# serycjon/WOFT

Hardware: AMD Instinct MI355X
Metric: tracked frames/sec at 1080p, 12 RAFT iters; flow EPE vs reference (higher is better)
Workload: dtype bf16x3 (split-bf16 MFMA operands emulating fp32, fp32 accumulate)

## Files before the change

### include/woft_hip.h

```cpp
#ifndef WOFT_HIP_H
#define WOFT_HIP_H

#include <stdint.h>

#ifdef __cplusplus
extern "C" {
#endif

#define WOFT_OK 0
#define WOFT_EINVAL (-1)
#define WOFT_ELAUNCH (-2)

int woft_abi_version(void);
int woft_sizeof(int which);
int woft_set_tuning(int key, int value);

enum woft_epilogue {
    WOFT_EPI_LINEAR = 0,
    WOFT_EPI_RELU = 1,
    WOFT_EPI_SIGMOID = 2,
    WOFT_EPI_TANH = 3,
    WOFT_EPI_RELU_RES_RELU = 4,
    WOFT_EPI_GRU_ZR = 5,
    WOFT_EPI_GRU_Q = 6,
    WOFT_EPI_CTX = 7,
    WOFT_EPI_WH_MEAN = 8,
    WOFT_EPI_FLOWHEAD = 9
};

typedef struct woft_conv_params {
    const float* in0;
    const float* in1;
    int32_t cs0, cs1;
    int32_t c_split;
    int32_t n_img, h, w;
    int32_t ho, wo;
    int32_t taps_y, taps_x;
    int32_t stride, pad_y, pad_x;
    int32_t cin_pad;
    int32_t flat;
    const float* wgt;
    const void* wgt_hi;
    const void* wgt_lo;
    int32_t precision;
    const float* bias;
    float alpha;
    int32_t cout;
    int32_t cout_pad;
    float* out;
    int64_t ldo;
    int32_t co_off;
    int32_t out_w, out_pitch;
    int32_t epi;
    int32_t split;
    const float* e0;
    const float* e1;
    int32_t lde0, lde1;
    float* out1;
    int32_t ldo1;
    float* stat_sum;
    float* stat_sq;
    int32_t tile_m, tile_n;
    int32_t halo;
    int32_t in_norm;
    const float* in_mean;
    const float* in_rstd;
    const float* bias_map;
    int32_t ld_bias_map;
    const int32_t* out_index;
    const float* wh0_lookup;
    int32_t wh0_ld;
    const float* wh0_mean;
    const void* wh0_w;
    const float* wh0_bias;
    const int32_t* wh0_index;
    const void* wgt_frag;
    const void* wgt_mx;
    int32_t roi_y0, roi_x0, roi_h, roi_w;
} woft_conv_params;

int woft_conv2d(const woft_conv_params* p, void* stream);
int woft_conv2d_pair(const woft_conv_params* a, const woft_conv_params* b, void* stream);
int woft_upload_u8(const void* src, void* pinned, void* dev, int64_t bytes, int32_t n_chunks, void* stream);
int woft_split_bf16(const float* x, int64_t n, void* hi, void* lo, void* stream);
int woft_conv3x3_narrow(const float* in, int32_t cs, int32_t n_img, int32_t h, int32_t w, int32_t cin_pad,
                        const float* wgt, const float* bias, int32_t cout, float* out, int64_t ldo, int32_t co_off,
                        void* stream);
int woft_flow_head_update(const float* in, int32_t cs, int32_t h, int32_t w, int32_t cin_pad, const float* wgt,
                          const float* bias, float* delta, int64_t ld_delta, float* coords1, float* flow4,
                          float* flow_cat, int32_t ld_cat, void* stream);
int woft_flow_head_gather(const float* part, int32_t n_planes, int32_t ld, int32_t h, int32_t w, const float* bias2,
                          float* delta, int64_t ld_delta, float* coords1, float* flow4, float* flow_cat, int32_t ld_cat,
                          void* stream);
int woft_split_bf16_lines(const float* x, int64_t n, void* out, void* stream);
int woft_corr_gemm_bf16(const void* a, const void* b, int64_t m, int64_t n, int64_t rows_a, int64_t rows_b, int32_t k,
                        float alpha, void* out, int64_t ldo, int32_t terms, int32_t out_bf16, void* stream);

int woft_inorm_finalize(const float* stat_sum, const float* stat_sq, int32_t n_part, int32_t ld,
                        int32_t channels, int32_t channels_pad, int64_t count, float eps,
                        float* mean, float* rstd, void* ws, void* stream);
int64_t woft_inorm_ws_bytes(void);
int woft_inorm_apply(const float* x, const float* mean, const float* rstd, const float* res,
                     const float* res_mean, const float* res_rstd, int32_t res_mode,
                     float* out, int64_t n_pix, int32_t channels, int32_t mode, void* stream);

int woft_preprocess_bgr_u8(const uint8_t* img, int32_t h, int32_t w, float* out,
                           int32_t hp, int32_t wp, int32_t pad_top, int32_t pad_left, void* stream);

int woft_avgpool2_nhwc(const float* in, int32_t h, int32_t w, int32_t c, float* out, void* stream);

int woft_feature_pyramid(const float* in, int32_t h, int32_t w, int32_t c, int32_t levels, float* const* pooled,
                         void* const* split, int32_t terms, void* stream);

typedef struct woft_lookup_params {
    const void* vol[4];
    int32_t ht[4], wt[4];
    int64_t plane[4];
    int32_t levels, radius;
    const float* coords;
    int64_t n_pix;
    float* out;
    int32_t ldo;
    int32_t vol_bf16;
    int32_t ablate;
} woft_lookup_params;
int woft_corr_lookup(const woft_lookup_params* p, void* stream);
typedef struct woft_lookup_otf_params {
    const void* f1;
    const void* f2[4];
    int32_t h[4], w[4];
    int32_t levels, radius, terms;
    int32_t hf, wf, k;
    float alpha;
    const float* coords;
    float* out;
    const int32_t* need;
    int32_t ldo;
    int32_t ablate;
    const float* fh_part;
    const float* fh_bias;
    float* fh_delta;
    float* fh_flow4;
    float* fh_flow_cat;
    int32_t fh_planes, fh_ld, fh_ld_delta, fh_ld_cat;
    int32_t roi_y0, roi_x0, roi_h, roi_w;
    int32_t smp_y0, smp_x0, smp_h, smp_w;
} woft_lookup_otf_params;
int woft_corr_lookup_otf(const woft_lookup_otf_params* p, void* stream);
#define WOFT_BAND_M0 3
#define WOFT_BAND_LD 16
#define WOFT_BAND_M(l) ((WOFT_BAND_M0 + (1 << (l)) - 1) >> (l))
#define WOFT_BAND_W(radius, l) (2 * ((radius) + 1 + WOFT_BAND_M(l)))
int woft_corr_band_geometry(int32_t radius, int32_t levels, int32_t* m, int32_t* w, int32_t* row_off);
typedef struct woft_lookup_band_params {
    woft_lookup_otf_params otf;
    float* band;
    int32_t* miss;
    int32_t* miss_count;
} woft_lookup_band_params;
int woft_corr_band_build(const woft_lookup_band_params* p, void* stream);
int woft_corr_lookup_band(const woft_lookup_band_params* p, void* stream);
int woft_tile_rows(const float* in, int32_t h, int32_t w, int32_t c, float* out, void* stream);

int woft_coords_update(float* coords1, const float* delta, int32_t ld_delta, int32_t wf, int64_t n_pix,
                       float* flow4, float* flow_cat, int32_t ld_cat, void* stream);
int woft_coords_init(float* coords1, int32_t hf, int32_t wf, float* flow4, float* flow_cat,
                     int32_t ld_cat, void* stream);
int woft_coords_init_flow(float* coords1, const float* flow_init, int32_t hf, int32_t wf, float* flow4, float* flow_cat,
                          int32_t ld_cat, void* stream);
int woft_forward_interpolate(const float* flow, int32_t hf, int32_t wf, float* out, void* stream);

int woft_sample_bilinear(const float* data, int32_t c, int32_t h, int32_t w, const float* x, const float* y, int64_t n,
                         float* out, void* stream);
int woft_flow_chain(const float* fab, const float* fbc, int32_t h, int32_t w, float* fac, void* stream);
int woft_flow_fb(const float* fab, const float* fba, int32_t h, int32_t w, float alpha, float beta, float* err, float* ok,
                 void* stream);

int woft_flow_chain_fold(const float* prev_flow, const float* prev_cost, const float* prev_vis, const float* step_flow,
                         const float* step_wlogit, const float* step_mlogit, int32_t h, int32_t w, float unit_cost,
                         float vis_thr, int32_t k, int32_t first, float* best_flow, float* best_cost, float* best_vis,
                         int32_t* best_sel, void* stream);

#define WOFT_CHAIN_HIST 130
int woft_chain_tc(const float* flow, const float* cost, const float* vis, const int32_t* sel, const uint8_t* tmask, int32_t gh,
                  int32_t gw, int32_t mh, int32_t mw, float vis_thr, float* dst, float* w, float* ok, int32_t* hist, void* stream);

int woft_features_pack(const float* f1, int64_t ld_f1, const float* net, int64_t ld_net, const float* inp, int64_t ld_inp,
                       int64_t P, int32_t fdim, int32_t hdim, int32_t cdim, float* record, void* stream);
int woft_features_unpack(const float* record, int64_t P, int32_t fdim, int32_t hdim, int32_t cdim, float* fmap, int64_t ld_fmap,
                         void* fmap_split, float* net, int64_t ld_net, float* xbuf, int64_t ld_xbuf, float* inp_c,
                         int64_t ld_inp_c, void* stream);

int woft_colsum(const float* f, int64_t n_pix, int32_t c, double* ws, int32_t n_part, double* total, void* stream);
int woft_wh_conv0(const float* lookup, int32_t ld_lookup, const float* mean, int64_t n_pix, int32_t nwin,
                  const float* wt, const float* bias, float* out, const int32_t* index, void* stream);
int woft_wh_pack(const float* lookup, int32_t ld_lookup, const float* f1, int32_t c, const double* f2_total,
                 float alpha, int64_t n_pix, int32_t nwin, float* mean, float* x8, void* stream);
int woft_wh_reduce(const float* act, int32_t c, int32_t nwin2, const float* w, float bias,
                   int64_t n_pix, float* out, void* stream);
int woft_warp_features(const float* f, int32_t h, int32_t w, int32_t c, int32_t cs, const float* coords, int64_t n_pix,
                       float* out, int32_t ld_out, void* stream);
int woft_wh_needed(const float* pts, const int32_t* count, int32_t n_max, int32_t top, int32_t left, int32_t hf, int32_t wf,
                   const int32_t* index, int32_t n_win, int32_t* bitmap, int32_t* dyn_index, int32_t* n_needed, void* stream);

int woft_convex_upsample(const float* coords1, const float* wlow, const float* mask, int32_t ld_mask,
                         int32_t hf, int32_t wf, int32_t crop_top, int32_t crop_left, int32_t h, int32_t w,
                         float* flow_up, float* dst, float* wout, int32_t do_sigmoid, void* stream);
int woft_convex_weights_at(const float* pts, const int32_t* count, int32_t n_max, const float* wlow, const float* mask,
                           int32_t ld_mask, int32_t hf, int32_t wf, int32_t crop_top, int32_t crop_left,
                           int32_t do_sigmoid, float* wsel, void* stream);
#define WOFT_WH_TRAIN_CHUNK 16
#define WOFT_WH_TRAIN_MAX_WIN (9 * 2048)
int woft_convex_weights_at_bwd(const float* pts, const int32_t* count, int32_t n_max, const float* g_wsel, const float* wlow,
                               const float* mask, int32_t ld_mask, int32_t hf, int32_t wf, int32_t crop_top,
                               int32_t crop_left, int32_t do_sigmoid, const int32_t* index, int32_t n_win, float* g_wlow,
                               void* stream);
int woft_wh_reduce_bwd(const float* act, const float* w6, const float* g_wlow, const int32_t* index, int32_t n_win,
                       float* g_act, double* ws, float* g_w6, float* g_b6, void* stream);
int woft_wh_train_conv(const float* x, int32_t cin, const float* wt, const float* bias, const float* gate, int32_t n_win,
                       float* y, void* stream);
int64_t woft_wh_wgrad_ws_bytes(int32_t n_win, int32_t cin);
int woft_wh_wgrad(const float* gy, const float* x, int32_t cin, int32_t cin_out, int32_t n_win, float* ws, float* gw,
                  float* gb, void* stream);
int woft_flow_to_tc(const float* flow, const float* weights, int32_t h, int32_t w, float* dst, float* wout,
                    int32_t do_sigmoid, void* stream);
int woft_upflow8(const float* coords1, const float* wlow, int32_t hf, int32_t wf,
                 int32_t crop_top, int32_t crop_left, int32_t h, int32_t w,
                 float* flow_up, float* dst, float* wout, int32_t do_sigmoid, void* stream);

int woft_warp_perspective_u8(const uint8_t* img, int32_t h, int32_t w, int32_t c, const double* hinv,
                             uint8_t* out, uint8_t* valid, int32_t nearest, void* stream);

int woft_warp_perspective_window_u8(const uint8_t* img, int32_t h, int32_t w, int32_t c, const double* hinv, int32_t y0,
                                    int32_t x0, int32_t hw, int32_t ww, uint8_t* out, uint8_t* valid, int32_t nearest,
                                    void* stream);
int woft_crop_u8(const uint8_t* img, int32_t h, int32_t w, int32_t c, int32_t y0, int32_t x0, int32_t hw, int32_t ww,
                 uint8_t* out, void* stream);
int64_t woft_mask_bbox_ws_bytes(void);
int woft_mask_bbox(const uint8_t* mask, int32_t h, int32_t w, const double* hinv, uint8_t* warped, void* ws, int32_t* bbox,
                   void* stream);

int woft_resize_linear_u8(const uint8_t* img, int32_t h, int32_t w, int32_t c, uint8_t* out, int32_t ho, int32_t wo,
                          float scale_y, float scale_x, void* stream);

int64_t woft_tc_select_ws_bytes(int64_t n);
int woft_tc_select(const float* dst, const float* w, const uint8_t* tmask, const uint8_t* pwmask, int32_t gh,
                   int32_t gw, int32_t mh, int32_t mw, int32_t check_dst, const float* sobol_u, int32_t n_draw,
                   void* ws, float* pa, float* pb, float* wout, int32_t cap, int32_t* count, void* stream);
int woft_tc_flags(const float* dst, const uint8_t* tmask, const uint8_t* pwmask, int32_t gh, int32_t gw, int32_t mh,
                  int32_t mw, int32_t check_dst, uint8_t* flags, void* stream);
int woft_tc_select_vis(const float* dst, const float* w, const uint8_t* tmask, const uint8_t* pwmask, int32_t gh,
                       int32_t gw, int32_t mh, int32_t mw, int32_t check_dst, const float* sobol_u, int32_t n_draw,
                       const float* vis, int32_t vis_mode, float vis_thr, void* ws, float* pa, float* pb, float* wout,
                       int32_t cap, int32_t* count, void* stream);
int woft_tc_flags_vis(const float* dst, const uint8_t* tmask, const uint8_t* pwmask, int32_t gh, int32_t gw, int32_t mh,
                      int32_t mw, int32_t check_dst, const float* vis, int32_t vis_mode, float vis_thr, uint8_t* flags,
                      void* stream);

#define WOFT_HFIT_SINGLE_MAX 2048
int64_t woft_hfit_ws_bytes(void);
int woft_hfit(const float* pa, const float* pb, const float* w, int32_t n_max, const int32_t* count,
              int32_t reweight, float huber_k, int32_t n_irls, void* ws, float* Hout, int32_t* status, void* stream);
#define WOFT_HFIT_BATCH_MAX 65535
int woft_hfit_batched(const float* pa, const float* pb, const float* w, int32_t batch, int32_t n_max,
                      const int32_t* counts, int32_t reweight, float huber_k, int32_t n_irls, float* Hout,
                      int32_t* status, void* stream);
int woft_hfit_batched_bwd(const float* pa, const float* pb, const float* w, int32_t batch, int32_t n_max,
                          const int32_t* counts, const float* gH, float* gpa, float* gpb, float* gw, int32_t* status,
                          void* stream);
int woft_hfit_step(const float* pa, const float* pb, const float* w, int32_t n, const float* rew, int32_t first,
                   void* ws, float* res, float* Hout, int32_t* status, void* stream);
int woft_inlier_frac(const float* pa, const float* pb, int32_t n_max, const int32_t* count, const float* H,
                     float thr, float* frac, void* stream);

int64_t woft_ransac_ws_bytes(int32_t n_max, int32_t max_iters);
int woft_ransac(const float* pa, const float* pb, int32_t n_max, const int32_t* count, int32_t max_iters, double thr,
                double conf, uint64_t seed, int32_t refine, void* ws, float* Hout, int32_t* status, int32_t* info,
                uint8_t* inlier_mask, void* stream);

int64_t woft_trs_ws_bytes(int32_t n_max, int32_t max_iters);
int woft_trs(const float* pa, const float* pb, int32_t n_max, const int32_t* count, int32_t max_iters, double thr,
             double conf, uint64_t seed, int32_t refine, void* ws, float* Hout, int32_t* status, int32_t* info,
             uint8_t* inlier_mask, void* stream);

#ifdef __cplusplus
}
#endif
#endif
```

### woft_amd/_lib.py

```python
import ctypes as C
import os
from pathlib import Path

import torch

LIB_PATH = Path(os.environ.get("WOFT_HIP_LIB") or Path(__file__).resolve().parent / "lib" / "libwoft_hip.so")

EPI_LINEAR, EPI_RELU, EPI_SIGMOID, EPI_TANH, EPI_RELU_RES_RELU, EPI_GRU_ZR, EPI_GRU_Q, EPI_CTX, EPI_WH_MEAN, EPI_FLOWHEAD = range(10)

vp, i32, i64, f32 = C.c_void_p, C.c_int32, C.c_int64, C.c_float


class ConvParams(C.Structure):
    _fields_ = [
        ("in0", vp), ("in1", vp), ("cs0", i32), ("cs1", i32), ("c_split", i32),
        ("n_img", i32), ("h", i32), ("w", i32), ("ho", i32), ("wo", i32),
        ("taps_y", i32), ("taps_x", i32), ("stride", i32), ("pad_y", i32), ("pad_x", i32),
        ("cin_pad", i32), ("flat", i32), ("wgt", vp), ("wgt_hi", vp), ("wgt_lo", vp), ("precision", i32),
        ("bias", vp), ("alpha", f32),
        ("cout", i32), ("cout_pad", i32), ("out", vp), ("ldo", i64), ("co_off", i32),
        ("out_w", i32), ("out_pitch", i32), ("epi", i32), ("split", i32),
        ("e0", vp), ("e1", vp), ("lde0", i32), ("lde1", i32), ("out1", vp), ("ldo1", i32),
        ("stat_sum", vp), ("stat_sq", vp), ("tile_m", i32), ("tile_n", i32), ("halo", i32),
        ("in_norm", i32), ("in_mean", vp), ("in_rstd", vp), ("bias_map", vp), ("ld_bias_map", i32),
        ("out_index", vp),
        ("wh0_lookup", vp), ("wh0_ld", i32), ("wh0_mean", vp), ("wh0_w", vp), ("wh0_bias", vp), ("wh0_index", vp),
        ("wgt_frag", vp), ("wgt_mx", vp),
        ("roi_y0", i32), ("roi_x0", i32), ("roi_h", i32), ("roi_w", i32),
    ]


class LookupParams(C.Structure):
    _fields_ = [
        ("vol", vp * 4), ("ht", i32 * 4), ("wt", i32 * 4), ("plane", i64 * 4),
        ("levels", i32), ("radius", i32), ("coords", vp), ("n_pix", i64), ("out", vp), ("ldo", i32),
        ("vol_bf16", i32), ("ablate", i32),
    ]


class LookupOtfParams(C.Structure):
    _fields_ = [
        ("f1", vp), ("f2", vp * 4), ("h", i32 * 4), ("w", i32 * 4),
        ("levels", i32), ("radius", i32), ("terms", i32), ("hf", i32), ("wf", i32), ("k", i32),
        ("alpha", f32), ("coords", vp), ("out", vp), ("need", vp), ("ldo", i32), ("ablate", i32),
        ("fh_part", vp), ("fh_bias", vp), ("fh_delta", vp), ("fh_flow4", vp), ("fh_flow_cat", vp),
        ("fh_planes", i32), ("fh_ld", i32), ("fh_ld_delta", i32), ("fh_ld_cat", i32),
        ("roi_y0", i32), ("roi_x0", i32), ("roi_h", i32), ("roi_w", i32),
        ("smp_y0", i32), ("smp_x0", i32), ("smp_h", i32), ("smp_w", i32),
    ]


class LookupBandParams(C.Structure):
    _fields_ = LookupOtfParams._fields_ + [("band", vp), ("miss", vp), ("miss_count", vp)]


_SIGS = {
    "woft_abi_version": (i32, []),
    "woft_sizeof": (i32, [i32]),
    "woft_set_tuning": (i32, [i32, i32]),
    "woft_conv2d": (i32, [C.POINTER(ConvParams), vp]),
    "woft_conv2d_pair": (i32, [C.POINTER(ConvParams), C.POINTER(ConvParams), vp]),
    "woft_upload_u8": (i32, [vp, vp, vp, i64, i32, vp]),
    "woft_split_bf16": (i32, [vp, i64, vp, vp, vp]),
    "woft_split_bf16_lines": (i32, [vp, i64, vp, vp]),
    "woft_flow_to_tc": (i32, [vp, vp, i32, i32, vp, vp, i32, vp]),
    "woft_corr_lookup_otf": (i32, [C.POINTER(LookupOtfParams), vp]),
    "woft_corr_band_geometry": (i32, [i32, i32, C.POINTER(i32), C.POINTER(i32), C.POINTER(i32)]),
    "woft_corr_band_build": (i32, [C.POINTER(LookupBandParams), vp]),
    "woft_corr_lookup_band": (i32, [C.POINTER(LookupBandParams), vp]),
    "woft_conv3x3_narrow": (i32, [vp, i32, i32, i32, i32, i32, vp, vp, i32, vp, i64, i32, vp]),
    "woft_flow_head_update": (i32, [vp, i32, i32, i32, i32, vp, vp, vp, i64, vp, vp, vp, i32, vp]),
    "woft_flow_head_gather": (i32, [vp, i32, i32, i32, i32, vp, vp, i64, vp, vp, vp, i32, vp]),
    "woft_corr_gemm_bf16": (i32, [vp, vp, i64, i64, i64, i64, i32, f32, vp, i64, i32, i32, vp]),
    "woft_inorm_finalize": (i32, [vp, vp, i32, i32, i32, i32, i64, f32, vp, vp, vp, vp]),
    "woft_inorm_ws_bytes": (i64, []),
    "woft_inorm_apply": (i32, [vp, vp, vp, vp, vp, vp, i32, vp, i64, i32, i32, vp]),
    "woft_preprocess_bgr_u8": (i32, [vp, i32, i32, vp, i32, i32, i32, i32, vp]),
    "woft_avgpool2_nhwc": (i32, [vp, i32, i32, i32, vp, vp]),
    "woft_feature_pyramid": (i32, [vp, i32, i32, i32, i32, vp, vp, i32, vp]),
    "woft_corr_lookup": (i32, [C.POINTER(LookupParams), vp]),
    "woft_tile_rows": (i32, [vp, i32, i32, i32, vp, vp]),
    "woft_coords_update": (i32, [vp, vp, i32, i32, i64, vp, vp, i32, vp]),
    "woft_coords_init": (i32, [vp, i32, i32, vp, vp, i32, vp]),
    "woft_coords_init_flow": (i32, [vp, vp, i32, i32, vp, vp, i32, vp]),
    "woft_forward_interpolate": (i32, [vp, i32, i32, vp, vp]),
    "woft_sample_bilinear": (i32, [vp, i32, i32, i32, vp, vp, i64, vp, vp]),
    "woft_flow_chain": (i32, [vp, vp, i32, i32, vp, vp]),
    "woft_flow_fb": (i32, [vp, vp, i32, i32, f32, f32, vp, vp, vp]),
    "woft_flow_chain_fold": (i32, [vp, vp, vp, vp, vp, vp, i32, i32, f32, f32, i32, i32, vp, vp, vp, vp, vp]),
    "woft_chain_tc": (i32, [vp, vp, vp, vp, vp, i32, i32, i32, i32, f32, vp, vp, vp, vp, vp]),
    "woft_features_pack": (i32, [vp, i64, vp, i64, vp, i64, i64, i32, i32, i32, vp, vp]),
    "woft_features_unpack": (i32, [vp, i64, i32, i32, i32, vp, i64, vp, vp, i64, vp, i64, vp, i64, vp]),
    "woft_colsum":(i32, [vp, i64, i32, vp, i32, vp, vp]),
    "woft_wh_pack": (i32, [vp, i32, vp, i32, vp, f32, i64, i32, vp, vp, vp]),
    "woft_wh_conv0": (i32, [vp, i32, vp, i64, i32, vp, vp, vp, vp, vp]),
    "woft_wh_reduce": (i32, [vp, i32, i32, vp, f32, i64, vp, vp]),
    "woft_warp_features": (i32, [vp, i32, i32, i32, i32, vp, i64, vp, i32, vp]),
    "woft_wh_needed": (i32, [vp, vp, i32, i32, i32, i32, i32, vp, i32, vp, vp, vp, vp]),
    "woft_convex_upsample": (i32, [vp, vp, vp, i32, i32, i32, i32, i32, i32, i32, vp, vp, vp, i32, vp]),
    "woft_convex_weights_at": (i32, [vp, vp, i32, vp, vp, i32, i32, i32, i32, i32, i32, vp, vp]),
    "woft_convex_weights_at_bwd": (i32, [vp, vp, i32, vp, vp, vp, i32, i32, i32, i32, i32, i32, vp, i32, vp, vp]),
    "woft_wh_reduce_bwd": (i32, [vp, vp, vp, vp, i32, vp, vp, vp, vp, vp]),
    "woft_wh_train_conv": (i32, [vp, i32, vp, vp, vp, i32, vp, vp]),
    "woft_wh_wgrad_ws_bytes": (i64, [i32, i32]),
    "woft_wh_wgrad": (i32, [vp, vp, i32, i32, i32, vp, vp, vp, vp]),
    "woft_upflow8": (i32, [vp, vp, i32, i32, i32, i32, i32, i32, vp, vp, vp, i32, vp]),
    "woft_warp_perspective_u8": (i32, [vp, i32, i32, i32, C.POINTER(C.c_double), vp, vp, i32, vp]),
    "woft_resize_linear_u8": (i32, [vp, i32, i32, i32, vp, i32, i32, f32, f32, vp]),
    "woft_warp_perspective_window_u8": (i32, [vp, i32, i32, i32, C.POINTER(C.c_double), i32, i32, i32, i32, vp, vp, i32, vp]),
    "woft_crop_u8": (i32, [vp, i32, i32, i32, i32, i32, i32, i32, vp, vp]),
    "woft_mask_bbox_ws_bytes": (i64, []),
    "woft_mask_bbox": (i32, [vp, i32, i32, C.POINTER(C.c_double), vp, vp, vp, vp]),
    "woft_tc_select_ws_bytes": (i64, [i64]),
    "woft_tc_select": (i32, [vp, vp, vp, vp, i32, i32, i32, i32, i32, vp, i32, vp, vp, vp, vp, i32, vp, vp]),
    "woft_tc_flags": (i32, [vp, vp, vp, i32, i32, i32, i32, i32, vp, vp]),
    "woft_tc_select_vis": (i32, [vp, vp, vp, vp, i32, i32, i32, i32, i32, vp, i32, vp, i32, f32, vp, vp, vp, vp, i32, vp, vp]),
    "woft_tc_flags_vis": (i32, [vp, vp, vp, i32, i32, i32, i32, i32, vp, i32, f32, vp, vp]),
    "woft_hfit_ws_bytes": (i64, []),
    "woft_hfit": (i32, [vp, vp, vp, i32, vp, i32, f32, i32, vp, vp, vp, vp]),
    "woft_hfit_batched": (i32, [vp, vp, vp, i32, i32, vp, i32, f32, i32, vp, vp, vp]),
    "woft_hfit_batched_bwd": (i32, [vp, vp, vp, i32, i32, vp, vp, vp, vp, vp, vp, vp]),
    "woft_hfit_step": (i32, [vp, vp, vp, i32, vp, i32, vp, vp, vp, vp, vp]),
    "woft_inlier_frac": (i32, [vp, vp, i32, vp, vp, f32, vp, vp]),
    "woft_ransac_ws_bytes": (i64, [i32, i32]),
    "woft_ransac": (i32, [vp, vp, i32, vp, i32, C.c_double, C.c_double, C.c_uint64, i32, vp, vp, vp, vp, vp, vp]),
    "woft_trs_ws_bytes": (i64, [i32, i32]),
    "woft_trs": (i32, [vp, vp, i32, vp, i32, C.c_double, C.c_double, C.c_uint64, i32, vp, vp, vp, vp, vp, vp]),
}

EXPORTS = tuple(_SIGS)
_lib = None


class WoftHipError(RuntimeError):
    pass


def load():
    global _lib
    if _lib is not None:
        return _lib
    if not LIB_PATH.exists():
        raise WoftHipError(f"{LIB_PATH} is missing: build it with `python -m woft_amd.build` "
                           "(hipcc --offload-arch=gfx950); woft_amd has no CPU fallback")
    lib = C.CDLL(str(LIB_PATH))
    for name, (res, args) in _SIGS.items():
        fn = getattr(lib, name)
        fn.restype, fn.argtypes = res, args
    if lib.woft_sizeof(0) != C.sizeof(ConvParams) or lib.woft_sizeof(1) != C.sizeof(LookupParams) \
            or lib.woft_sizeof(2) != C.sizeof(LookupOtfParams) or lib.woft_sizeof(3) != C.sizeof(LookupBandParams):
        raise WoftHipError("ctypes mirror of woft_conv_params / woft_lookup_params is out of sync with the library")
    _lib = lib
    return lib


def check(rc, what):
    if rc != 0:
        raise WoftHipError(f"{what} failed with code {rc}")


def ptr(t):
    return None if t is None else t.data_ptr()


_RAW_STREAM = getattr(torch._C, "_cuda_getCurrentRawStream", None) if os.environ.get("WOFT_RAW_STREAM", "1") != "0" else None
_CUR_DEV = torch.cuda.current_device


def stream_ptr():
    if _RAW_STREAM is None:
        return torch.cuda.current_stream().cuda_stream
    return _RAW_STREAM(_CUR_DEV())
```

### woft_amd/build.py

```python
import hashlib
import os
import subprocess
import sys
import time
from pathlib import Path

HERE = Path(__file__).resolve().parent
CSRC = HERE / "csrc"
LIBDIR = HERE / "lib"
LIB = LIBDIR / "libwoft_hip.so"
STAMP = LIBDIR / "libwoft_hip.stamp"
HIPCC = os.environ.get("HIPCC", "/opt/rocm/bin/hipcc")
FLAGS = ["--offload-arch=gfx950", "-O3", "-std=c++17", "-fPIC", "-fno-fast-math", "-ffp-contract=off",
         "-Wno-c++20-extensions"]


PARTS = {"conv.hip": [("p1", ["-DWOFT_ONLY_PREC=1"]), ("p2", ["-DWOFT_ONLY_PREC=2"]), ("p3", ["-DWOFT_ONLY_PREC=3"])],
         "conv_regb.hip": [(f"p{k}", [f"-DWOFT_ONLY_PREC={k}"]) for k in (1, 2, 3, 4)]}


def _sources():
    return sorted(CSRC.glob("*.hip"))


def _units():
    out = []
    for src in _sources():
        for tag, flags in PARTS.get(src.name, [("", [])]):
            out.append((src, LIBDIR / (src.stem + ("." + tag if tag else "") + ".o"), flags))
    return out


def _digest():
    h = hashlib.sha256()
    for p in sorted(list(CSRC.glob("*.hip")) + list(CSRC.glob("*.h")) + [HERE.parent / "include" / "woft_hip.h"]):
        h.update(p.name.encode())
        h.update(p.read_bytes())
    h.update(" ".join(FLAGS).encode())
    h.update(repr(sorted(PARTS.items())).encode())
    return h.hexdigest()


def build(force=False, verbose=True):
    LIBDIR.mkdir(exist_ok=True)
    dig = _digest()
    if not force and LIB.exists() and STAMP.exists() and STAMP.read_text().strip() == dig:
        return LIB
    objs = []
    units = _units()
    wanted = {u[1] for u in units}
    for old in LIBDIR.glob("*.o"):
        if old not in wanted:
            old.unlink()
    hdr = hashlib.sha256()
    for h in sorted(list(CSRC.glob("*.h")) + [HERE.parent / "include" / "woft_hip.h"]):
        hdr.update(h.name.encode())
        hdr.update(h.read_bytes())

    def unit_hash(src, extra):
        u = hashlib.sha256(hdr.digest())
        u.update(src.read_bytes())
        u.update(" ".join(FLAGS + extra).encode())
        return u.hexdigest()
    jobs = int(os.environ.get("WOFT_BUILD_JOBS", os.cpu_count() or 4))
    weight = {"conv.hip": 8, "conv_regb.hip": 6, "conv_1x1.hip": 20}
    units.sort(key=lambda u: -(u[0].stat().st_size * weight.get(u[0].name, 1)))
    pending, running = [], []
    for src, obj, extra in units:
        objs.append(obj)
        uh = unit_hash(src, extra)
        tag = Path(str(obj) + ".hash")
        if not force and obj.exists() and tag.exists() and tag.read_text().strip() == uh:
            continue
        pending.append((src, obj, extra, uh))
    while pending or running:
        while pending and len(running) < jobs:
            src, obj, extra, uh = pending.pop(0)
            tag = Path(str(obj) + ".hash")
            if tag.exists():
                tag.unlink()
            cmd = [HIPCC, *FLAGS, *extra, "-c", str(src), "-o", str(obj)]
            if verbose:
                print(" ".join(cmd), flush=True)
            running.append((src, subprocess.Popen(cmd), tag, uh))
        time.sleep(0.2)
        for ent in list(running):
            rc = ent[1].poll()
            if rc is None:
                continue
            running.remove(ent)
            if rc != 0:
                for other in running:
                    other[1].kill()
                raise RuntimeError(f"hipcc failed on {ent[0]}")
            ent[2].write_text(ent[3])
    cmd = [HIPCC, "--offload-arch=gfx950", "-shared", "-fPIC", "-o", str(LIB), *map(str, objs)]
    if verbose:
        print(" ".join(cmd), flush=True)
    subprocess.check_call(cmd)
    STAMP.write_text(dig)
    return LIB


if __name__ == "__main__":
    build(force="--force" in sys.argv)
    print(LIB)
```

### woft_amd/csrc/conv.hip

```cpp
#include <type_traits>

#include "conv_common.h"
#include "dma.h"
#include "halo_map.h"
#include "split_lines.h"

#if !defined(WOFT_ONLY_PREC)
#error "conv.hip is compiled in parts: -DWOFT_ONLY_PREC=1|2|3 (woft_amd/build.py)"
#endif
#define WOFT_CAT2_(a, b) a##b
#define WOFT_CAT2(a, b) WOFT_CAT2_(a, b)
#define WOFT_CAT4_(a, b, c, d) a##b##c##d
#define WOFT_CAT4(a, b, c, d) WOFT_CAT4_(a, b, c, d)
#if WOFT_ONLY_PREC == 1
constexpr int PART_TERMS = 3;
#elif WOFT_ONLY_PREC == 3
constexpr int PART_TERMS = 16;
#else
constexpr int PART_TERMS = 1;
#endif

#if WOFT_ONLY_PREC == 1
int g_tuning[4] = {0, 0, 0, 0};
#else
// ... 763 lines not shown
                            acc[i][j] = __builtin_amdgcn_mfma_f32_32x32x16_bf16(ah[i], bh[j], acc[i][j], 0, 0, 0);
                }
            }
        }
        if (STAGES == 2) dma_wait<0>();
        __syncthreads();
    }
    if (abl & 2) {
        float t = 0.f;
#pragma unroll
        for (int i = 0; i < TM; ++i)
#pragma unroll
            for (int j = 0; j < TN; ++j)
#pragma unroll
                for (int r = 0; r < 16; ++r) t += acc[i][j][r];
        if (t == 12345.678f) p.out[0] = t;
        return;
    }
    float* stage = (float*)smem + wave * woft::STAGE_FLOATS;
    constexpr int LD = woft::STAGE_LD;
    const int rr = lane >> 3, c4 = (lane & 7) * 4;
#pragma unroll
    for (int i = 0; i < TM; ++i)
#pragma unroll
        for (int j = 0; j < TN; ++j) {
#pragma unroll
            for (int r = 0; r < 16; ++r) stage[((r & 3) + 8 * (r >> 2) + 4 * hh) * LD + r32] = acc[i][j][r];
            __builtin_amdgcn_wave_barrier();
            const int n = n0 + wn * 64 + j * 32 + c4;
#pragma unroll
            for (int pass = 0; pass < 4; ++pass) {
                const int row = rr + 8 * pass;
                const int64_t m = m0 + wm * 64 + i * 32 + row;
                f32x4 v = *(const f32x4*)(stage + row * LD + c4);
                if (m >= M || n >= p.cout || (abl & 1)) continue;
#pragma unroll
                for (int e = 0; e < 4; ++e) v[e] *= p.alpha;
                if (OUT16) *(bf16x4*)((__bf16*)p.out + m * p.ldo + n) = __builtin_convertvector(v, bf16x4);
                else if (abl & 16) __builtin_nontemporal_store(v, (f32x4*)(p.out + m * p.ldo + n));
                else *(f32x4*)(p.out + m * p.ldo + n) = v;
            }
            __builtin_amdgcn_wave_barrier();
        }
}

#endif

#if WOFT_ONLY_PREC == 1
__global__ void split_bf16_kernel(const float* __restrict__ x, int64_t n4, __bf16* __restrict__ hi,
                                  __bf16* __restrict__ lo) {
    const int64_t i = (int64_t)blockIdx.x * blockDim.x + threadIdx.x;
    if (i >= n4) return;
    const f32x4 vv = *(const f32x4*)(x + i * 4);
    const bf16x4 h = __builtin_convertvector(vv, bf16x4);
    *(bf16x4*)(hi + i * 4) = h;
    if (lo != nullptr) *(bf16x4*)(lo + i * 4) = __builtin_convertvector(vv - __builtin_convertvector(h, f32x4), bf16x4);
}

#endif

template <int BM, int BN>
int launch_conv(const woft_conv_params& p, const woft_conv_params* second, hipStream_t s) {
    auto blocks = [](const woft_conv_params& q) { return ceil_div64((int64_t)q.n_img * q.ho * q.wo, BM) * (q.cout_pad / BN); };
    const woft_conv_params& pb = second ? *second : p;
    const int split = (int)blocks(p);
    dim3 grid((unsigned)(blocks(p) + (second ? blocks(pb) : 0)));
    if (p.precision == 0) {
#if WOFT_ONLY_PREC == 2
        if (second) return WOFT_EINVAL;
        woft_launch(0, conv_mfma_f32_kernel<BM, BN>, grid, dim3(256), 0, s, p);
        return woft_launch_status();
#else
        return WOFT_EINVAL;
#endif
    }
    if (p.precision != WOFT_ONLY_PREC) return WOFT_EINVAL;
    for (const woft_conv_params* q : {&p, &pb}) {
        const int64_t cs_max = (q->in1 != nullptr && q->cs1 > q->cs0) ? q->cs1 : q->cs0;
        if ((int64_t)q->n_img * q->h * q->w * cs_max >= (1ll << 31)) return WOFT_EINVAL;
        if ((int64_t)q->taps_y * q->taps_x * q->cin_pad >= (1 << 20)) return WOFT_EINVAL;
    }
    woft_launch(0, conv_mfma_bf16_kernel<BM, BN, PART_TERMS>, grid, dim3(256), 0, s, p, pb, split);
    return woft_launch_status();
}

}

int WOFT_CAT2(woft_conv_regb_launch_p, WOFT_ONLY_PREC)(const woft_conv_params& p, const woft_conv_params* second, void* stream);
int woft_conv_stem_launch(const woft_conv_params& p, void* stream);
int woft_conv_1x1_launch(const woft_conv_params& p, const woft_conv_params* second, void* stream);
int woft_conv_dispatch_p1(const woft_conv_params& p, const woft_conv_params* second, void* stream);
int woft_conv_dispatch_p2(const woft_conv_params& p, const woft_conv_params* second, void* stream);
int woft_conv_dispatch_p3(const woft_conv_params& p, const woft_conv_params* second, void* stream);

#if WOFT_ONLY_PREC == 1
static int conv_check(const woft_conv_params& p) {
    if (p.in0 == nullptr || p.out == nullptr) return WOFT_EINVAL;
    if (p.precision < 0 || p.precision > 4) return WOFT_EINVAL;
    if (p.precision == 4 && ((p.halo != 8 && p.halo != 12) || p.wgt_frag == nullptr || p.wgt_mx == nullptr ||
                             p.in_norm != 0 || p.taps_y * p.taps_x == 1))
        return WOFT_EINVAL;
    if (p.precision == 0 && p.wgt == nullptr) return WOFT_EINVAL;
    if (p.precision >= 1 && p.wgt_hi == nullptr) return WOFT_EINVAL;
    if (p.precision == 1 && p.wgt_lo == nullptr) return WOFT_EINVAL;
    if (p.cin_pad <= 0 || p.cin_pad % BK != 0) return WOFT_EINVAL;
    if (p.in1 != nullptr && (p.c_split % BK != 0 || p.c_split <= 0 || p.c_split >= p.cin_pad)) return WOFT_EINVAL;
    if (p.cs0 % 4 != 0 || (p.in1 != nullptr && p.cs1 % 4 != 0)) return WOFT_EINVAL;
    if (p.flat && (p.taps_x != 1 || p.in1 != nullptr || (p.cs0 != 4 && p.cs0 != 8 && p.cs0 != 16 && p.cs0 != 32)))
        return WOFT_EINVAL;
    if (!p.flat && (p.cs0 < (p.in1 != nullptr ? p.c_split : p.cin_pad) || (p.in1 != nullptr && p.cs1 < p.cin_pad - p.c_split)))
        return WOFT_EINVAL;
    if (p.n_img <= 0 || p.h <= 0 || p.w <= 0 || p.ho <= 0 || p.wo <= 0 || p.taps_y <= 0 || p.taps_x <= 0 ||
        p.stride <= 0 || p.cout <= 0)
        return WOFT_EINVAL;
    if ((p.tile_m != 64 && p.tile_m != 128) || (p.tile_n != 64 && p.tile_n != 128 && !(p.halo == 16 && p.tile_n == 256)))
        return WOFT_EINVAL;
    if (p.cout_pad % p.tile_n != 0 || p.cout > p.cout_pad) return WOFT_EINVAL;
    if (p.epi < 0 || p.epi > WOFT_EPI_FLOWHEAD) return WOFT_EINVAL;
    if (p.epi == WOFT_EPI_FLOWHEAD && (p.halo != 8 || p.precision == 0 || p.stat_sum != nullptr || p.bias_map != nullptr ||
                                       p.e0 == nullptr))
        return WOFT_EINVAL;
    if (p.epi == WOFT_EPI_WH_MEAN && (p.halo != 2 || p.cout_pad != p.tile_n || p.e0 == nullptr || p.e1 == nullptr ||
                                      p.stat_sum != nullptr))
        return WOFT_EINVAL;
    if ((p.epi == WOFT_EPI_RELU_RES_RELU || p.epi == WOFT_EPI_GRU_ZR || p.epi == WOFT_EPI_GRU_Q) && p.e0 == nullptr)
        return WOFT_EINVAL;
    if (p.epi == WOFT_EPI_GRU_Q && p.e1 == nullptr) return WOFT_EINVAL;
    if (p.epi == WOFT_EPI_GRU_ZR && p.out1 == nullptr) return WOFT_EINVAL;
    if (p.e0 != nullptr && p.lde0 % 4 != 0) return WOFT_EINVAL;
    if (p.e1 != nullptr && p.lde1 % 4 != 0) return WOFT_EINVAL;
    if (p.out1 != nullptr && (p.ldo1 % 4 != 0 || p.split % 4 != 0)) return WOFT_EINVAL;
    if ((p.stat_sum == nullptr) != (p.stat_sq == nullptr)) return WOFT_EINVAL;
    if (p.epi != WOFT_EPI_WH_MEAN) {
        if (p.out_pitch != 0 || p.ldo % 4 != 0 || p.co_off % 4 != 0 || p.epi == WOFT_EPI_CTX) return WOFT_EINVAL;
        const bool simple = p.epi == WOFT_EPI_LINEAR || p.epi == WOFT_EPI_RELU || p.epi == WOFT_EPI_SIGMOID || p.epi == WOFT_EPI_TANH;
        if (p.cout % 4 != 0 && (!simple || p.stat_sum != nullptr || p.bias_map != nullptr)) return WOFT_EINVAL;
    }
    if (p.in_norm < 0 || p.in_norm > 2) return WOFT_EINVAL;
    if ((p.roi_y0 | p.roi_x0 | p.roi_h | p.roi_w) != 0 &&
        ((p.halo != 8 && p.halo != 12 && p.halo != 16) || p.roi_h <= 0 || p.roi_w <= 0 || p.roi_y0 < 0 || p.roi_x0 < 0 ||
         p.roi_y0 > p.ho - p.roi_h || p.roi_x0 > p.wo - p.roi_w || p.stat_sum != nullptr || p.precision == 0))
        return WOFT_EINVAL;
    if (p.bias_map != nullptr && (p.cout % 4 != 0 || p.ld_bias_map < p.cout || p.ld_bias_map % 4 != 0 ||
                                  p.epi == WOFT_EPI_CTX || p.epi == WOFT_EPI_WH_MEAN || p.out_pitch != 0))
        return WOFT_EINVAL;
    if (p.in_norm != 0 && (p.halo == 0 || p.in1 != nullptr || p.in_mean == nullptr || p.in_rstd == nullptr)) return WOFT_EINVAL;
    if (p.wh0_lookup != nullptr &&
        (p.halo != 2 || p.precision == 0 || p.taps_y != 3 || p.taps_x != 3 || p.cin_pad != 128 || p.in1 != nullptr ||
         p.in_norm != 0 || p.ho != 9 || p.wo != 9 || p.wh0_ld < 324 || p.wh0_ld % 4 != 0 || p.wh0_mean == nullptr ||
         p.wh0_w == nullptr || p.wh0_bias == nullptr))
        return WOFT_EINVAL;
    return WOFT_OK;
}
#endif

int WOFT_CAT2(woft_conv_dispatch_p, WOFT_ONLY_PREC)(const woft_conv_params& p, const woft_conv_params* second, void* stream) {
    hipStream_t s = (hipStream_t)stream;
    if (second != nullptr && (second->precision != p.precision || second->halo != p.halo ||
                              (p.halo == 0 && second->tile_m != p.tile_m) ||
                              (second->tile_n != p.tile_n && p.halo != 16) || p.precision == 0 ||
                              (p.halo != 0 && p.halo != 8 && p.halo != 12 && p.halo != 16)))
        return WOFT_EINVAL;
    if (p.halo == 7)
        return second != nullptr ? WOFT_EINVAL : woft_conv_stem_launch(p, stream);
    if (p.halo == 16)
        return p.precision == 0 ? WOFT_EINVAL : woft_conv_1x1_launch(p, second, stream);
    for (const woft_conv_params* q : {&p, second}) {
        if (q == nullptr || q->halo == 0) continue;
        if (q->precision == 0 || q->flat || q->stride != 1) return WOFT_EINVAL;
        if (q->ho != q->h + 2 * q->pad_y - q->taps_y + 1 || q->wo != q->w + 2 * q->pad_x - q->taps_x + 1) return WOFT_EINVAL;
        const int64_t cs_max = (q->in1 != nullptr && q->cs1 > q->cs0) ? q->cs1 : q->cs0;
        if ((int64_t)q->n_img * q->h * q->w * cs_max >= (1ll << 31)) return WOFT_EINVAL;
        if ((int64_t)q->taps_y * q->taps_x * q->cin_pad >= (1 << 20)) return WOFT_EINVAL;
    }
    if (p.halo != 0) {
        if (p.halo == 8 || p.halo == 12)
            return WOFT_CAT2(woft_conv_regb_launch_p, WOFT_ONLY_PREC)(p, second, stream);
        if (p.halo == 1 && p.tile_n == 128) return launch_halo<8, 16, 128, 2, 2>(p, s);
        if (p.halo == 1 && p.tile_n == 64) return launch_halo<8, 16, 64, 2, 2>(p, s);
        if (p.halo == 2 && p.tile_n == 128 && p.ho == 9 && p.wo == 9) return launch_halo<9, 9, 128, 1, 2>(p, s);
        if (p.halo == 4 && p.tile_n == 128) return launch_halo<4, 16, 128, 2, 2>(p, s);
        if (p.halo == 4 && p.tile_n == 64) return launch_halo<4, 16, 64, 2, 2>(p, s);
        return WOFT_EINVAL;
    }
    if (p.tile_m == 128 && p.tile_n == 128) return launch_conv<128, 128>(p, second, s);
    if (p.tile_m == 128 && p.tile_n == 64) return launch_conv<128, 64>(p, second, s);
    if (p.tile_m == 64 && p.tile_n == 128) return launch_conv<64, 128>(p, second, s);
    return launch_conv<64, 64>(p, second, s);
}

#if WOFT_ONLY_PREC == 1
int woft_conv_regb_launch_p4(const woft_conv_params& p, const woft_conv_params* second, void* stream);

static int conv_dispatch_f16mx8(const woft_conv_params& p, const woft_conv_params* second, void* stream) {
    for (const woft_conv_params* q : {&p, second}) {
        if (q == nullptr) continue;
        if (q->precision != 4 || q->halo != p.halo || q->tile_n != p.tile_n || q->flat || q->stride != 1) return WOFT_EINVAL;
        if (q->ho != q->h + 2 * q->pad_y - q->taps_y + 1 || q->wo != q->w + 2 * q->pad_x - q->taps_x + 1) return WOFT_EINVAL;
        const int64_t cs_max = (q->in1 != nullptr && q->cs1 > q->cs0) ? q->cs1 : q->cs0;
        if ((int64_t)q->n_img * q->h * q->w * cs_max >= (1ll << 31)) return WOFT_EINVAL;
    }
    return woft_conv_regb_launch_p4(p, second, stream);
}

static int conv_dispatch(const woft_conv_params& p, const woft_conv_params* second, void* stream) {
    switch (p.precision) {
        case 4: return conv_dispatch_f16mx8(p, second, stream);
        case 1: return woft_conv_dispatch_p1(p, second, stream);
        case 3: return woft_conv_dispatch_p3(p, second, stream);
        default: return woft_conv_dispatch_p2(p, second, stream);
    }
}

extern "C" int woft_conv2d(const woft_conv_params* pp, void* stream) {
    if (pp == nullptr) return WOFT_EINVAL;
    const int rc = conv_check(*pp);
    return rc != WOFT_OK ? rc : conv_dispatch(*pp, nullptr, stream);
}

extern "C" int woft_conv2d_pair(const woft_conv_params* a, const woft_conv_params* b, void* stream) {
    if (a == nullptr || b == nullptr) return WOFT_EINVAL;
    int rc = conv_check(*a);
    if (rc == WOFT_OK) rc = conv_check(*b);
    if (rc != WOFT_OK) return rc;
    if (a->stat_sum != nullptr || b->stat_sum != nullptr) return WOFT_EINVAL;
    return conv_dispatch(*a, b, stream);
}
#endif

#if WOFT_ONLY_PREC == 3
extern "C" int woft_corr_gemm_bf16(const void* a, const void* b, int64_t m, int64_t n, int64_t rows_a, int64_t rows_b,
                                   int32_t k, float alpha, void* out, int64_t ldo, int32_t terms, int32_t out_bf16,
                                   void* stream) {
    if (!a || !b || !out || m <= 0 || n <= 0 || k <= 0 || ldo < n || n % 4 != 0 || ldo % 4 != 0) return WOFT_EINVAL;
    if (terms != 1 && terms != 3) return WOFT_EINVAL;
    if (k % (terms == 3 ? 32 : 64) != 0) return WOFT_EINVAL;
    if (rows_a % 128 != 0 || rows_b % 128 != 0 || rows_a < m || rows_b < n || m >= (1ll << 31)) return WOFT_EINVAL;
    woft_conv_params p = {};
    p.n_img = 1; p.ho = 1; p.wo = (int32_t)m;
    p.alpha = alpha;
    p.cout = (int32_t)n; p.cout_pad = (int32_t)rows_b;
    p.out = (float*)out; p.ldo = ldo;
    p.epi = WOFT_EPI_LINEAR;
    const int abl = g_tuning[2];
    hipStream_t s = (hipStream_t)stream;
    if (rows_a % 128 != 0 || rows_b % 128 != 0) return WOFT_EINVAL;
    dim3 grid((unsigned)(ceil_div64(m, 128) * (rows_b / 128)));
    if (terms == 3 && !out_bf16)
        hipLaunchKernelGGL((corr_gemm_bf16_kernel<3, 2, 2, 1>), grid, dim3(256), 0, s, (const __bf16*)a, (const __bf16*)b,
                           2 * k, p, abl);
    else if (terms == 3)
        hipLaunchKernelGGL((corr_gemm_bf16_kernel<3, 2, 2, 1, true>), grid, dim3(256), 0, s, (const __bf16*)a,
                           (const __bf16*)b, 2 * k, p, abl);
    else if (!out_bf16)
        hipLaunchKernelGGL((corr_gemm_bf16_kernel<1, 2, 2, 1>), grid, dim3(256), 0, s, (const __bf16*)a, (const __bf16*)b,
                           k, p, abl);
    else
        hipLaunchKernelGGL((corr_gemm_bf16_kernel<1, 2, 2, 1, true>), grid, dim3(256), 0, s, (const __bf16*)a,
                           (const __bf16*)b, k, p, abl);
    return woft_launch_status();
}

#endif

#if WOFT_ONLY_PREC == 1
int g_regb_dyn_lds = 0;

extern "C" int woft_set_tuning(int key, int value) {
    if (key < 0 || key >= 4) return WOFT_EINVAL;
    g_tuning[key] = value;
    if (key == 3) g_regb_dyn_lds = value;
    return WOFT_OK;
}

__global__ void split_bf16_lines_kernel(const float* __restrict__ x, int64_t n4, __bf16* __restrict__ out) {
    const int64_t i = (int64_t)blockIdx.x * blockDim.x + threadIdx.x;
    if (i >= n4) return;
    split_bf16_lines_store(out, i, *(const f32x4*)(x + i * 4));
}

extern "C" int woft_split_bf16_lines(const float* x, int64_t n, void* out, void* stream) {
    if (!x || !out || n <= 0 || n % 32 != 0) return WOFT_EINVAL;
    hipLaunchKernelGGL(split_bf16_lines_kernel, dim3((unsigned)ceil_div64(n / 4, 256)), dim3(256), 0, (hipStream_t)stream,
                       x, n / 4, (__bf16*)out);
    return woft_launch_status();
}

extern "C" int woft_split_bf16(const float* x, int64_t n, void* hi, void* lo, void* stream) {
    if (!x || !hi || n <= 0 || n % 4 != 0) return WOFT_EINVAL;
    hipLaunchKernelGGL(split_bf16_kernel, dim3((unsigned)ceil_div64(n / 4, 256)), dim3(256), 0, (hipStream_t)stream, x,
                       n / 4, (__bf16*)hi, (__bf16*)lo);
    return woft_launch_status();
}
#endif
```

### woft_amd/csrc/conv_1x1.hip

```cpp
#include "conv_common.h"

namespace {

using woft::BK;

template <int TERMS, int TN>
struct Geom1x1 {
    static constexpr int NP = (TERMS == 3) ? 2 : 1;
    static constexpr int BM = 64, TM = 2;
    static constexpr int WCOLS = 32 * TN, BN = 4 * WCOLS;
    static constexpr int A_PLANE = BM * LDB, A_ELEMS = NP * A_PLANE;
    static constexpr int ST = 2;
    static constexpr int STAGE_ELEMS = 2 * 4 * ST * woft::STAGE_FLOATS;
    static constexpr int SMEM_ELEMS = (2 * A_ELEMS > STAGE_ELEMS) ? 2 * A_ELEMS : STAGE_ELEMS;
};

template <int TERMS, int TN, bool FLAT, int DEPTH, int NB>
__device__ __forceinline__ void tile_1x1(const woft_conv_params& p, const int m_tile, const int n_tile, __bf16* smem) {
    using G = Geom1x1<TERMS, TN>;
    constexpr int NP = G::NP, TM = G::TM, A_PLANE = G::A_PLANE, A_ELEMS = G::A_ELEMS, WCOLS = G::WCOLS, BN = G::BN;
    static_assert(DEPTH % 2 == 0 && (2 * DEPTH) % NB == 0 && NB >= 2, "static ring slots");
    constexpr int STEP_ELEMS = NP * 2 * 64 * 8;

    const int tid = threadIdx.x;
    const int lane = tid & 63;
    const int wave = __builtin_amdgcn_readfirstlane(tid >> 6);
    const int r32 = lane & 31, hh = lane >> 5;
    const int row = tid >> 2, v = tid & 3;

    int64_t M = (int64_t)p.n_img * p.ho * p.wo;
    int64_t m0 = (int64_t)m_tile * G::BM;
    if ((p.roi_y0 | p.roi_x0 | p.roi_h | p.roi_w) != 0) {
        const int runs = (p.roi_w + G::BM - 1) / G::BM;
        const int line = m_tile / runs, run = m_tile - line * runs;
        const int img = line / p.roi_h, ry = line - img * p.roi_h;
        m0 = ((int64_t)img * p.ho + p.roi_y0 + ry) * p.wo + p.roi_x0 + run * G::BM;
        const int left = p.roi_w - run * G::BM;
        M = m0 + (left < G::BM ? left : G::BM);
    }
    const int n0 = n_tile * BN;
    const int nchunk = FLAT ? p.taps_y : p.cin_pad / BK;

    const int abl = (p.out_w <= -12350 && p.out_w > -12358) ? -12350 - p.out_w : 0;
    const bool rok = m0 + row < M;
    const uint32_t pix = rok ? (uint32_t)(m0 + row) : 0u;
    int oy = 0, img_row0 = 0;
    uint32_t run0 = 0;
    bool okx[2] = {true, true};
    if constexpr (FLAT) {
        const int hw = p.ho * p.wo;
        const int img = (int)(pix / (uint32_t)hw), rem = (int)(pix - (uint32_t)img * (uint32_t)hw);
        oy = rem / p.wo;
        const int ox = rem - oy * p.wo;
        img_row0 = img * p.h;
#pragma unroll
        for (int e = 0; e < 2; ++e) {
            const int ixp = ox - p.pad_x + (8 * v + 4 * e) / p.cs0;
            okx[e] = rok && ixp >= 0 && ixp < p.w;
        }
        run0 = (uint32_t)((ox - p.pad_x) * p.cs0 + 8 * v);
    }
    f32x4 rh[DEPTH][2];
    auto load_a = [&](int chunk, auto slot_tag) {
        constexpr int slot = decltype(slot_tag)::value;
        if ((abl & 1) && chunk >= DEPTH) return;
        const int ck = chunk < nchunk ? chunk : nchunk - 1;
        if constexpr (FLAT) {
            int iy = oy + ck - p.pad_y;
            iy = iy < 0 ? 0 : (iy >= p.h ? p.h - 1 : iy);
            const uint32_t rowoff = (uint32_t)(img_row0 + iy) * (uint32_t)(p.w * p.cs0);
#pragma unroll
            for (int e = 0; e < 2; ++e) rh[slot][e] = *(const f32x4*)(p.in0 + (okx[e] ? rowoff + run0 + 4 * e : 0u));
        } else {
            const int c0 = ck * BK;
            const bool second = (p.in1 != nullptr) && (c0 >= p.c_split);
            const float* base = second ? p.in1 : p.in0;
            const uint32_t cs = (uint32_t)(second ? p.cs1 : p.cs0);
            const uint32_t coff = (uint32_t)(second ? c0 - p.c_split : c0);
            rh[slot][0] = *(const f32x4*)(base + (pix * cs + coff + 8 * v));
            rh[slot][1] = *(const f32x4*)(base + (pix * cs + coff + 8 * v + 4));
        }
    };
    auto store_a = [&](int chunk, __bf16* As, auto slot_tag) {
        constexpr int slot = decltype(slot_tag)::value;
        const f32x4 zero = {0.f, 0.f, 0.f, 0.f};
        bool oky = true;
        if constexpr (FLAT) {
            const int iy = oy + chunk - p.pad_y;
            oky = iy >= 0 && iy < p.h;
        }
        bf16x4 hi[2], lo[2];
#pragma unroll
        for (int e = 0; e < 2; ++e) {
            const f32x4 val = (FLAT ? (okx[e] && oky) : rok) ? rh[slot][e] : zero;
            hi[e] = cvt16<TERMS>(val);
            if (NP == 2) lo[e] = __builtin_convertvector(val - widen_bf16x4(hi[e]), bf16x4);
        }
        *(bf16x8*)(As + row * LDB + 8 * v) = __builtin_shufflevector(hi[0], hi[1], 0, 1, 2, 3, 4, 5, 6, 7);
        if (NP == 2) *(bf16x8*)(As + A_PLANE + row * LDB + 8 * v) = __builtin_shufflevector(lo[0], lo[1], 0, 1, 2, 3, 4, 5, 6, 7);
    };

    const __bf16* wstream[TN];
#pragma unroll
    for (int j = 0; j < TN; ++j) wstream[j] = (const __bf16*)p.wgt_frag + (int64_t)(n0 / 32 + wave * TN + j) * nchunk * STEP_ELEMS + lane * 8;
    bf16x8 bq[NB][TN][NP];
    auto fetch_b = [&](int step, auto slot_tag) {
        constexpr int slot = decltype(slot_tag)::value;
        if ((abl & 2) && step >= NB - 1) return;
        const int s = step < 2 * nchunk ? step : 2 * nchunk - 1;
        const int off = (s >> 1) * STEP_ELEMS + (s & 1) * 512;
#pragma unroll
        for (int j = 0; j < TN; ++j)
#pragma unroll
            for (int pl = 0; pl < NP; ++pl) bq[slot][j][pl] = *(const bf16x8*)(wstream[j] + off + pl * 1024);
    };

    f32x16 acc[TM][TN];
#pragma unroll
    for (int i = 0; i < TM; ++i)
#pragma unroll
        for (int j = 0; j < TN; ++j)
#pragma unroll
            for (int r = 0; r < 16; ++r) acc[i][j][r] = 0.f;
    const int a_off = r32 * LDB + hh * 8;

    [&]<int... D>(std::integer_sequence<int, D...>) {
        (load_a(D, std::integral_constant<int, D>{}), ...);
    }(std::make_integer_sequence<int, DEPTH>{});
    [&]<int... S>(std::integer_sequence<int, S...>) {
        (fetch_b(S, std::integral_constant<int, S>{}), ...);
    }(std::make_integer_sequence<int, NB - 1>{});
    store_a(0, smem, std::integral_constant<int, 0>{});
    __syncthreads();

    auto run_chunk = [&](int c, auto d_tag) {
        constexpr int D = decltype(d_tag)::value;
        const __bf16* As = smem + (D & 1) * A_ELEMS;
        bf16x8 aq[2][TM][NP];
        auto read_a = [&](auto s2_tag) {
            constexpr int s2 = decltype(s2_tag)::value;
#pragma unroll
            for (int i = 0; i < TM; ++i)
#pragma unroll
                for (int pl = 0; pl < NP; ++pl) aq[s2][i][pl] = *(const bf16x8*)(As + a_off + i * 32 * LDB + pl * A_PLANE + s2 * 16);
        };
        read_a(std::integral_constant<int, 0>{});
        read_a(std::integral_constant<int, 1>{});
        [&]<int... S2>(std::integer_sequence<int, S2...>) {
            ([&] {
                constexpr int s2 = S2, slot = (2 * D + s2) % NB;
                fetch_b(2 * c + s2 + NB - 1, std::integral_constant<int, (2 * D + s2 + NB - 1) % NB>{});
                __builtin_amdgcn_sched_barrier(0);
                if (NP == 2) {
#pragma unroll
                    for (int j = 0; j < TN; ++j)
#pragma unroll
                        for (int i = 0; i < TM; ++i) acc[i][j] = mma16<TERMS>(aq[s2][i][NP - 1], bq[slot][j][0], acc[i][j]);
#pragma unroll
                    for (int j = 0; j < TN; ++j)
#pragma unroll
                        for (int i = 0; i < TM; ++i) acc[i][j] = mma16<TERMS>(aq[s2][i][0], bq[slot][j][NP - 1], acc[i][j]);
                }
#pragma unroll
                for (int j = 0; j < TN; ++j)
#pragma unroll
                    for (int i = 0; i < TM; ++i) acc[i][j] = mma16<TERMS>(aq[s2][i][0], bq[slot][j][0], acc[i][j]);
                if constexpr (s2 == 0) {
                    store_a(c + 1, smem + ((D + 1) & 1) * A_ELEMS, std::integral_constant<int, (D + 1) % DEPTH>{});
                    load_a(c + DEPTH, std::integral_constant<int, D>{});
                }
                __builtin_amdgcn_sched_barrier(0);
            }(), ...);
        }(std::make_integer_sequence<int, 2>{});
        __syncthreads();
    };
    for (int c0 = 0; c0 < nchunk; c0 += DEPTH) {
        [&]<int... D>(std::integer_sequence<int, D...>) {
            ((c0 + D < nchunk ? run_chunk(c0 + D, std::integral_constant<int, D>{}) : (void)0), ...);
        }(std::make_integer_sequence<int, DEPTH>{});
    }
    if (abl & 4) {
        float t = 0.f;
#pragma unroll
        for (int i = 0; i < TM; ++i)
#pragma unroll
            for (int j = 0; j < TN; ++j)
#pragma unroll
                for (int r = 0; r < 16; ++r) t += acc[i][j][r];
        if (t == 12345.678f) p.out[0] = t;
        return;
    }
    woft::conv_epilogue_t<TM, TN, G::BM, WCOLS, G::ST>(p, acc, (float*)smem + wave * G::ST * woft::STAGE_FLOATS,
                                                        woft::LinearRows{m0, M}, n0, 0, wave, lane, m_tile);
}

__host__ __device__ __forceinline__ int m_tiles_1x1(const woft_conv_params& p) {
    if ((p.roi_y0 | p.roi_x0 | p.roi_h | p.roi_w) != 0) return p.n_img * p.roi_h * ((p.roi_w + 63) / 64);
    return (int)(((int64_t)p.n_img * p.ho * p.wo + 63) / 64);
}


template <int TERMS>
__global__ __launch_bounds__(256, 2) void conv1x1_kernel(const woft_conv_params pa, const woft_conv_params pb, const int split) {
    __shared__ __attribute__((aligned(16))) __bf16 smem[Geom1x1<TERMS, 2>::SMEM_ELEMS];
    static_assert(Geom1x1<TERMS, 2>::SMEM_ELEMS >= Geom1x1<TERMS, 1>::SMEM_ELEMS, "one LDS array for every mode");
    const bool second_layer = (int)blockIdx.x >= split;
    const woft_conv_params p = second_layer ? pb : pa;
    const int bid = second_layer ? (int)blockIdx.x - split : (int)blockIdx.x;
    int m_tile, n_tile;
    woft::tile_of_block(bid, m_tiles_1x1(p), p.cout_pad / (p.flat ? 128 : 256), m_tile, n_tile);
    if (!p.flat) tile_1x1<TERMS, 2, false, 4, 4>(p, m_tile, n_tile, smem);
    else tile_1x1<TERMS, 1, true, 4, 4>(p, m_tile, n_tile, smem);
}

}

int woft_conv_1x1_launch(const woft_conv_params& a, const woft_conv_params* second, void* stream) {
    for (const woft_conv_params* q : {&a, second}) {
        if (q == nullptr) continue;
        const woft_conv_params& p = *q;
        if (p.precision < 1 || p.precision > 3 || p.precision != a.precision) return WOFT_EINVAL;
        if (p.stride != 1 || p.ho != p.h || p.wo != p.w || p.taps_x != 1) return WOFT_EINVAL;
        if (p.flat) {
            if (p.cin_pad != 32 || p.tile_n != 128 || 2 * p.pad_y + 1 != p.taps_y) return WOFT_EINVAL;
        } else if (p.taps_y != 1 || p.pad_y != 0 || p.pad_x != 0 || p.tile_n != 256) {
            return WOFT_EINVAL;
        }
        if (p.wgt_frag == nullptr || p.stat_sum != nullptr || p.in_norm != 0 || p.wh0_lookup != nullptr) return WOFT_EINVAL;
        if (p.epi == WOFT_EPI_FLOWHEAD || p.epi == WOFT_EPI_WH_MEAN || p.epi == WOFT_EPI_CTX) return WOFT_EINVAL;
        if (p.cout_pad % p.tile_n != 0) return WOFT_EINVAL;
        const int64_t cs_max = (p.in1 != nullptr && p.cs1 > p.cs0) ? p.cs1 : p.cs0;
        if ((int64_t)p.n_img * p.h * p.w * cs_max >= (1ll << 31)) return WOFT_EINVAL;
    }
    auto blocks = [](const woft_conv_params& q) {
        return (int64_t)m_tiles_1x1(q) * (q.cout_pad / (q.flat ? 128 : 256));
    };
    const woft_conv_params& pb = second ? *second : a;
    const int split = (int)blocks(a);
    dim3 grid((unsigned)(blocks(a) + (second ? blocks(pb) : 0)));
    hipStream_t s = (hipStream_t)stream;
    switch (a.precision) {
        case 1: woft_launch(0, conv1x1_kernel<3>, grid, dim3(256), 0, s, a, pb, split); break;
        case 2: woft_launch(0, conv1x1_kernel<1>, grid, dim3(256), 0, s, a, pb, split); break;
        default: woft_launch(0, conv1x1_kernel<16>, grid, dim3(256), 0, s, a, pb, split); break;
    }
    return woft_launch_status();
}
```

### woft_amd/csrc/lookup_band.hip

```cpp
#include "common.h"
#include "lookup_blocks.h"

namespace {

template <int R>
__global__ __launch_bounds__(256) void corr_lookup_band_kernel(const woft_lookup_band_params bp) {
    const woft_lookup_otf_params& p = bp.otf;
    constexpr int NPX = 64, NT = 256, MAXL = 4;
    constexpr int NW = 2 * R + 1, N2 = NW * NW, WS = NW + 1;
    constexpr int RS = WOFT_BAND_LD + 4;
    constexpr int PLD = WS * RS;
    constexpr int NLD = NPX * WS * 4 / NT;
    static_assert(NLD * NT == NPX * WS * 4, "pieces divide among the threads");
    __shared__ __attribute__((aligned(16))) float Wl[NPX * PLD];
    __shared__ int s_ox[MAXL][NPX], s_oy[MAXL][NPX];
    __shared__ float s_fx[MAXL][NPX], s_fy[MAXL][NPX];

    const int tid = threadIdx.x;
    const BlockRect br = block_rect(p);
    const int tiles_x = br.nx, ntiles = br.nx * br.ny;
    int tile;
    {
        const int q = ntiles / 8, rr = ntiles % 8, xcd = blockIdx.x % 8, idx = blockIdx.x / 8;
        tile = (xcd < rr ? xcd * (q + 1) : rr * (q + 1) + (xcd - rr) * q) + idx;
    }
    const int px0 = (br.bx0 + tile % tiles_x) * 8, py0 = (br.by0 + tile / tiles_x) * 8;
    const bool sampled = (p.smp_y0 | p.smp_x0 | p.smp_h | p.smp_w) == 0 ||
                         (py0 < p.smp_y0 + p.smp_h && py0 + 8 > p.smp_y0 && px0 < p.smp_x0 + p.smp_w && px0 + 8 > p.smp_x0);
    const int y = py0 + ((tid & 63) >> 3), x = px0 + (tid & 7);
    const bool cvalid = tid < NPX && y < p.hf && x < p.wf;
    const int64_t i = (int64_t)y * p.wf + x;
    if (p.need != nullptr) {
        const int any = cvalid ? p.need[i] : 0;
        if (!__syncthreads_or(any)) {
            if (cvalid) bp.miss[i] = 0;
            return;
        }
    }
    float cx = 0.f, cy = 0.f;
    if (cvalid) {
        cx = p.coords[i * 2];
        cy = p.coords[i * 2 + 1];
        if (p.fh_part != nullptr) {
            typedef float f32x2 __attribute__((ext_vector_type(2)));
            float dx = p.fh_bias ? p.fh_bias[0] : 0.f, dy = p.fh_bias ? p.fh_bias[1] : 0.f;
            const int64_t plane = (int64_t)p.hf * p.wf * p.fh_ld;
#pragma unroll
            for (int ky = 0; ky < 3; ++ky)
#pragma unroll
                for (int kx = 0; kx < 3; ++kx) {
                    const int yy = y + ky - 1, xx = x + kx - 1;
                    f32x2 v = {0.f, 0.f};
                    if (yy >= 0 && yy < p.hf && xx >= 0 && xx < p.wf) {
                        const float* src = p.fh_part + ((int64_t)yy * p.wf + xx) * p.fh_ld + (ky * 3 + kx) * 2;
                        v = *(const f32x2*)src;
                        for (int t = 1; t < p.fh_planes; ++t) v += *(const f32x2*)(src + t * plane);
                    }
                    dx += v[0];
                    dy += v[1];
                }
            p.fh_delta[i * p.fh_ld_delta] = dx;
            p.fh_delta[i * p.fh_ld_delta + 1] = dy;
            cx += dx;
            cy += dy;
            ((float*)p.coords)[i * 2] = cx;
            ((float*)p.coords)[i * 2 + 1] = cy;
            const float fx = cx - (float)x, fy = cy - (float)y;
            if (p.fh_flow4 != nullptr) *(f32x4*)(p.fh_flow4 + i * 4) = f32x4{fx, fy, 0.f, 0.f};
            if (p.fh_flow_cat != nullptr) {
                p.fh_flow_cat[i * p.fh_ld_cat] = fx;
                p.fh_flow_cat[i * p.fh_ld_cat + 1] = fy;
            }
        }
    }
    if (!sampled) {
        if (cvalid) bp.miss[i] = 0;
        return;
    }
    int ok = 1;
    if (cvalid) {
#pragma unroll
        for (int l = 0; l < MAXL; ++l) {
            if (l < p.levels) {
                const float sc = 1.0f / (float)(1 << l);
                const float xs = cx * sc, ys = cy * sc;
                float flx = floorf(xs), fly = floorf(ys);
                s_fx[l][tid] = xs - flx;
                s_fy[l][tid] = ys - fly;
                flx = fminf(fmaxf(flx, -1.0e6f), 1.0e6f);
                fly = fminf(fmaxf(fly, -1.0e6f), 1.0e6f);
                const int m = WOFT_BAND_M(l);
                const int ox = (int)flx - (x >> l) + m, oy = (int)fly - (y >> l) + m;
                ok &= (ox >= 0 && ox <= 2 * m && oy >= 0 && oy <= 2 * m) ? 1 : 0;
                s_ox[l][tid] = ox;
                s_oy[l][tid] = oy;
            }
        }
    }
    const int hit = __syncthreads_and(ok);
    if (cvalid) bp.miss[i] = hit ? 0 : 1;
    if (!hit) {
        if (tid == 0) atomicAdd(bp.miss_count, 1);
        return;
    }
    const int rows = band_row_off(R, p.levels);
    f32x4 pc[NLD];
    auto load_level = [&](int l) __attribute__((always_inline)) {
        const int roff = band_row_off(R, l);
#pragma unroll
        for (int k = 0; k < NLD; ++k) {
            const int it = tid + k * NT;
            const int pix = it / (4 * WS), rem = it - pix * (4 * WS);
            const int gy = py0 + (pix >> 3), gx = px0 + (pix & 7);
            pc[k] = f32x4{0.f, 0.f, 0.f, 0.f};
            if (gy < p.hf && gx < p.wf)
                pc[k] = *(const f32x4*)(bp.band + (((int64_t)gy * p.wf + gx) * rows + roff + s_ox[l][pix]) * WOFT_BAND_LD + rem * 4);
        }
    };
    load_level(0);
    for (int l = 0; l < p.levels; ++l) {
#pragma unroll
        for (int k = 0; k < NLD; ++k) {
            const int it = tid + k * NT;
            const int pix = it / (4 * WS), rem = it - pix * (4 * WS);
            *(f32x4*)(Wl + pix * PLD + (rem >> 2) * RS + (rem & 3) * 4) = pc[k];
        }
        __syncthreads();
        if (l + 1 < p.levels) load_level(l + 1);
        for (int it = tid; it < NPX * NW; it += NT) {
            const int pix = it / NW, c = it - pix * NW;
            const int gy = py0 + (pix >> 3), gx = px0 + (pix & 7);
            if (gy >= p.hf || gx >= p.wf) continue;
            const float fx = s_fx[l][pix], fy = s_fy[l][pix];
            const float* cq = Wl + pix * PLD + c * RS + s_oy[l][pix];
            float h[WS];
#pragma unroll
            for (int j = 0; j < WS; ++j) h[j] = cq[j] * (1.f - fx) + cq[RS + j] * fx;
            float* o = p.out + ((int64_t)gy * p.wf + gx) * p.ldo + l * N2 + c * NW;
#pragma unroll
            for (int j = 0; j < NW; ++j) o[j] = h[j] * (1.f - fy) + h[j + 1] * fy;
        }
        __syncthreads();
    }
}

}

extern "C" int woft_corr_lookup_band(const woft_lookup_band_params* bp, void* stream) {
    if (!bp || !bp->band || !bp->miss || !bp->miss_count) return WOFT_EINVAL;
    const woft_lookup_otf_params& p = bp->otf;
    if (p.levels < 1 || p.levels > 4 || !p.f1 || !p.coords || !p.out || p.hf <= 0 || p.wf <= 0 || p.ablate != 0) return WOFT_EINVAL;
    if (p.terms != 1 && p.terms != 3) return WOFT_EINVAL;
    if (!((p.k == 256 && p.radius == 4) || (p.k == 128 && p.radius == 3))) return WOFT_EINVAL;
    for (int l = 0; l < p.levels; ++l)
        if (p.h[l] <= 0 || p.w[l] <= 0) return WOFT_EINVAL;
    const int nout = p.levels * (2 * p.radius + 1) * (2 * p.radius + 1);
    if (p.ldo < nout) return WOFT_EINVAL;
    if (p.fh_part != nullptr && (p.fh_delta == nullptr || p.fh_planes < 1 || p.fh_ld < 20 || p.fh_ld % 4 != 0 || p.fh_ld_delta < 2 ||
                                 (p.fh_flow_cat != nullptr && p.fh_ld_cat < 2) || p.need != nullptr))
        return WOFT_EINVAL;
    auto rect_bad = [&](int y0, int x0, int h, int w) {
        return (y0 | x0 | h | w) != 0 && (h <= 0 || w <= 0 || y0 < 0 || x0 < 0 || y0 > p.hf - h || x0 > p.wf - w);
    };
    if (rect_bad(p.roi_y0, p.roi_x0, p.roi_h, p.roi_w) || rect_bad(p.smp_y0, p.smp_x0, p.smp_h, p.smp_w)) return WOFT_EINVAL;
    const BlockRect br = block_rect(p);
    dim3 grid((unsigned)(br.nx * br.ny));
    hipStream_t s = (hipStream_t)stream;
    if (p.radius == 4) woft_launch(0, corr_lookup_band_kernel<4>, grid, dim3(256), 0, s, *bp);
    else woft_launch(0, corr_lookup_band_kernel<3>, grid, dim3(256), 0, s, *bp);
    return woft_launch_status();
}
```

### woft_amd/engine.py

```python
import math
import os
from typing import NamedTuple

import torch

from . import _lib, conv_select, flow_region, ops, wh_train
from .conv_select import KERNELS, Kernel
from .ops import Act, new_act

EPI = _lib
DEFER_NORM = os.environ.get("WOFT_DEFER_NORM", "1") != "0"
FUSE_FLOWHEAD = os.environ.get("WOFT_FUSE_FLOWHEAD", "1") != "0"
PAIR_BRANCHES = os.environ.get("WOFT_PAIR", "1") != "0"
PYRAMID_ONE_LAUNCH = os.environ.get("WOFT_PYRAMID", "1") != "0"
FOLD_GATHER = os.environ.get("WOFT_FOLD_GATHER", "1") != "0"
CORR_BAND = os.environ.get("WOFT_CORR_BAND", "1") != "0"
BAND_MIN_LOOKUPS = 6


def _ru(x, m):
    return (x + m - 1) // m * m


class Step(NamedTuple):
    kind: str
    arg: object
    tag: str = None


class _Folded(NamedTuple):
    prog_iter_first: list
    prog_iter: list
    prog_iter_last: list
    gather: list
    lookup: object


class FlowKey(NamedTuple):
    iters: int
    crop: tuple
    h: int
    w: int
    flow_up: int
    dst: int
    wout: int
    mout: int
    do_sigmoid: bool
    mask_sigmoid: bool
    defer_wh: bool
    skip_wh: bool
    has_init: bool
    target_restored: bool
    wh_region: int
    flow_region: tuple


class _FlowGraph(torch.cuda.CUDAGraph):
    post = None


def _timed(sink, launch, *args, extra=None):
    if sink is None:
        return launch(*args)
    s, e = torch.cuda.Event(enable_timing=True), torch.cuda.Event(enable_timing=True)
    s.record()
    launch(*args)
    e.record()
    sink.append((s, e) if extra is None else (s, e, extra()))


def _head_layers(sd, prefix, cin):
    idx = sorted(int(k.split(".")[2]) for k in sd if k.startswith(prefix) and k.endswith(".weight"))
    shapes = [tuple(sd[f"{prefix}{i}.weight"].shape) for i in idx]
    ok = not (len(idx) < 2 or shapes[-1][0] != 1 or shapes[-1][2:] != (1, 1) or shapes[0][1] != cin
              or any(a[0] != b[1] for a, b in zip(shapes, shapes[1:])) or any(sh[2] != sh[3] or sh[2] % 2 == 0 for sh in shapes))
    return idx, shapes, ok


class _Spec:

    def __init__(self, small):
        self.small = small
        if small:
            self.fdim, self.hdim, self.cdim, self.radius = 128, 96, 64, 3
            self.fnorm, self.cnorm = "instance", "none"
        else:
            self.fdim, self.hdim, self.cdim, self.radius = 256, 128, 128, 4
            self.fnorm, self.cnorm = "instance", "batch"
        self.levels = 4
        self.nwin = 2 * self.radius + 1
        self.corr_c = self.levels * self.nwin ** 2
        self.corr_cs = _ru(self.corr_c, 32)
        self.xdim = _ru(self.cdim + (82 if small else 128), 32)
        self.flow_off = self.cdim + (80 if small else 126)


class _Enc:

    def __init__(self, sd, p, norm, spec, out_split=None):
        self.norm = norm

        def get(name, stride=1, flat_cs=0, bn=None):
            w, b = sd[name + ".weight"], sd[name + ".bias"]
            if norm == "batch" and bn is not None:
                w, b = ops.fold_bn(w, b, sd[bn + ".weight"], sd[bn + ".bias"], sd[bn + ".running_mean"],
                                   sd[bn + ".running_var"])
            return ops.pack_conv(w, b, stride=stride, flat_cs=flat_cs)

        self.conv1 = get(p + ".conv1", 2, 4, p + ".norm1")
        self.blocks = []
        for li, stride in ((1, 1), (2, 2), (3, 2)):
            for bi in range(2):
                q = f"{p}.layer{li}.{bi}"
                s = stride if bi == 0 else 1
                if spec.small:
                    convs = [get(q + ".conv1", 1, bn=q + ".norm1"), get(q + ".conv2", s, bn=q + ".norm2"),
                             get(q + ".conv3", 1, bn=q + ".norm3")]
                else:
                    convs = [get(q + ".conv1", s, bn=q + ".norm1"), get(q + ".conv2", 1, bn=q + ".norm2")]
                blk = dict(stride=s, convs=convs)
                if s != 1:
                    blk["down"] = get(q + ".downsample.0", s, bn=q + ".downsample.1")
                self.blocks.append(blk)
        w2, b2 = sd[p + ".conv2.weight"], sd[p + ".conv2.bias"]
        if out_split:
            self.conv2_net = ops.pack_conv(w2[:out_split], b2[:out_split])
            self.conv2_inp = ops.pack_conv(w2[out_split:], b2[out_split:])
        else:
            self.conv2 = ops.pack_conv(w2, b2)


class RaftEngine:
    def __init__(self, state_dict, small=False, weighted=True, precision="fp32", corr="volume", volume_storage=None,
                 mask_head=False, corr_band="auto"):
        if precision not in ops.PRECISION:
            raise ValueError(f"precision must be one of {sorted(ops.PRECISION)}")
        if corr not in ("volume", "otf"):
            raise ValueError("corr must be 'volume' or 'otf'")
        self.precision = precision
        self.prec_corr = self.prec_wh = "bf16x3" if precision in ("fp16", "f16mx8") else precision
        self.corr = corr
        if corr_band not in ("auto", True, False):
            raise ValueError("corr_band must be 'auto', True or False")
        self.corr_band = corr_band
        self.volume_storage = volume_storage or ("bf16" if precision == "bf16" else "fp32")
        if self.volume_storage not in ("fp32", "bf16") or (self.volume_storage == "bf16" and precision == "fp32"):
            raise ValueError("volume_storage: 'fp32', or 'bf16' with the split-bf16 precisions (their GEMM packs it)")
        _lib.load()
        if not torch.cuda.is_available():
            raise _lib.WoftHipError("woft_amd needs a HIP device: there is no CPU fallback")
        sd = {k: v.detach().float().cpu() for k, v in state_dict.items()}
        self.weighted, self.small, self.mask_head = weighted, small, bool(mask_head)
        self.spec = sp = _Spec(small)
        self.radius, self.levels = sp.radius, sp.levels
        if self.mask_head and not weighted:
            raise ValueError("mask_head: the MaskHead belongs to WeightedRAFT (weighted_raft.py:75-76), not to plain RAFT")
        self.convc2 = self.mk1 = self.mk2 = None
        self.wh_std = self.wh_flat0 = False
        self.wh0 = self.wh2 = self.wh4 = self.wh0_frag = self.wh_layers = self.wh6_c = self.wh6_w = self.wh6_b = None
        self.mh_shapes = self.mh_layers = self.mh_c = self.mh_wlast = self.mh_b = None
        self._pack_encoders(sd)
        self._pack_update_block(sd)
        if weighted:
            self._pack_weight_head(sd)
        if self.mask_head:
            self._pack_mask_head(sd)
        self._plans = {}

    def _pack_encoders(self, sd):
        self.fnet = _Enc(sd, "fnet", self.spec.fnorm, self.spec)
        self.cnet = _Enc(sd, "cnet", self.spec.cnorm, self.spec, out_split=self.spec.hdim)

    def _pack_update_block(self, sd):
        sp, small, precision = self.spec, self.small, self.precision
        u = "update_block."
        g = lambda n, **kw: ops.pack_conv(sd[u + n + ".weight"], sd[u + n + ".bias"], **kw)
        self.convc1 = g("encoder.convc1")
        self.convf1 = g("encoder.convf1", flat_cs=4)
        self.convf2 = g("encoder.convf2")
        self.convm = g("encoder.conv")
        self.fh1 = g("flow_head.conv1")
        self.fh2 = g("flow_head.conv2")
        self.fh2_frag = (ops.pack_flowhead_frags(sd[u + "flow_head.conv2.weight"], 2 if precision in ("bf16x3", "f16mx8") else 1,
                                                 f16=precision == "fp16")
                         if precision != "fp32" and FUSE_FLOWHEAD else None)
        if not small:
            self.convc2 = g("encoder.convc2")
            self.mk1 = g("mask.0")
            self.mk2 = g("mask.2", scale=0.25)
        hd_, cd_, mot = sp.hdim, sp.cdim, (82 if small else 128)
        dyn = [(0, hd_, 0), (hd_ + cd_, hd_ + cd_ + mot, hd_)]
        ctx = [(hd_, hd_ + cd_, 0)]
        self.zr_dyn, self.zr_inp, self.q_dyn, self.q_inp = [], [], [], []
        for sfx, pd in (("", None),) if small else (("1", (0, 2)), ("2", (2, 0))):
            zr_w, zr_b = (torch.cat([sd[f"{u}gru.convz{sfx}{s}"], sd[f"{u}gru.convr{sfx}{s}"]], 0) for s in (".weight", ".bias"))
            q_w, q_b = sd[f"{u}gru.convq{sfx}.weight"], sd[f"{u}gru.convq{sfx}.bias"]
            self.zr_dyn.append(ops.pack_conv(zr_w, None, padding=pd, cin_layout=dyn))
            self.zr_inp.append(ops.pack_conv(zr_w, zr_b, padding=pd, cin_layout=ctx))
            self.q_dyn.append(ops.pack_conv(q_w, None, padding=pd, cin_layout=dyn))
            self.q_inp.append(ops.pack_conv(q_w, q_b, padding=pd, cin_layout=ctx))

    def _pack_weight_head(self, sd):
        sp, precision = self.spec, self.precision
        w = "weight_head.net."
        idx, shapes, ok = _head_layers(sd, w, sp.levels + 1)
        if not ok:
            raise ValueError(f"weight head layers {shapes}: not a WeightHead (weighted_raft.py:318-345)")
        self.wh_std = shapes == [(128, 5, 3, 3), (128, 128, 3, 3), (128, 128, 3, 3), (1, 128, 1, 1)]
        last = idx[-1]
        if self.wh_std:
            self.wh0, self.wh2, self.wh4, self.wh0_frag = self._wh_std_packed(sd)
        else:
            k0 = shapes[0][2]
            self.wh_flat0 = k0 * 8 <= 32
            self.wh_layers = [ops.pack_conv(sd[f"{w}{idx[0]}.weight"], sd[f"{w}{idx[0]}.bias"], flat_cs=8 if self.wh_flat0 else 0)]
            self.wh_layers += [ops.pack_conv(sd[f"{w}{i}.weight"], sd[f"{w}{i}.bias"]) for i in idx[1:-1]]
        self.wh6_c = shapes[-1][1]
        self.wh6_w = torch.zeros(_ru(self.wh6_c, 4))
        self.wh6_w[:self.wh6_c] = sd[f"{w}{last}.weight"].reshape(-1)
        self.wh6_w = self.wh6_w.contiguous().cuda()
        self.wh6_b = float(sd[f"{w}{last}.bias"].item())

    def _wh_std_packed(self, sd):
        w = "weight_head.net."
        wh0 = ops.pack_conv(sd[w + "0.weight"], sd[w + "0.bias"], flat_cs=8)
        wh2 = ops.pack_conv(sd[w + "2.weight"], sd[w + "2.bias"])
        wh4 = ops.pack_conv(sd[w + "4.weight"], sd[w + "4.bias"])
        wh0_frag = (ops.pack_wh0_frags(sd[w + "0.weight"], 2 if self.prec_wh == "bf16x3" else 1)
                    if self.precision != "fp32" and self.spec.nwin == 9 else None)
        return wh0, wh2, wh4, wh0_frag

    def repack_weight_head(self, sd):
        assert self.weighted and self.wh_std
        sd = {k: v.detach().float().cpu() for k, v in sd.items() if k.startswith("weight_head.net.")}
        wh0, wh2, wh4, frag = self._wh_std_packed(sd)
        for old, new in ((self.wh0, wh0), (self.wh2, wh2), (self.wh4, wh4)):
            ops.repack_conv_(old, new)
        if self.wh0_frag is not None:
            self.wh0_frag.copy_(frag)
        self.wh6_w[:self.wh6_c].copy_(sd["weight_head.net.6.weight"].reshape(-1))
        self.wh6_b = float(sd["weight_head.net.6.bias"].item())
        for plan in self._plans.values():
            plan.refresh_weight_head()

    def _pack_mask_head(self, sd):
        sp = self.spec
        m = "mask_head.net."
        idx, shapes, ok = _head_layers(sd, m, 2 * sp.fdim)
        if not ok:
            raise ValueError(f"mask head layers {shapes}: not a MaskHead on {2 * sp.fdim} channels (weighted_raft.py:387-409)")
        self.mh_shapes = shapes
        self.mh_layers = [ops.pack_conv(sd[f"{m}{i}.weight"], sd[f"{m}{i}.bias"]) for i in idx[:-1]]
        self.mh_c = shapes[-1][1]
        self.mh_wlast = sd[f"{m}{idx[-1]}.weight"].reshape(-1).clone()
        self.mh_b = float(sd[f"{m}{idx[-1]}.bias"].item())

    def plan(self, hp, wp, slot=0):
        key = (hp, wp) if slot == 0 else (hp, wp, slot)
        if key not in self._plans:
            self._plans[key] = _Plan(self, hp, wp)
        return self._plans[key]

    def drop_plan(self, key):
        return self._plans.pop(key, None)


class _Plan:

    def __init__(self, eng, hp, wp):
        assert hp % 8 == 0 and wp % 8 == 0
        self.eng, self.hp, self.wp = eng, hp, wp
        self.prec, self.prec_corr, self.prec_wh = eng.precision, eng.prec_corr, eng.prec_wh
        self.otf = eng.corr == "otf"
        self.hf, self.wf, self.P = hp // 8, wp // 8, (hp // 8) * (wp // 8)
        self._source_changed()
        self._target_changed()
        self.lookup_events = None
        self.wh_events = None
        self.conv_events = None
        self._graphs = {}
        self._band = None
        self._band_params = {}
        self.mk = self.mask = self.prog_iter_last = self.folded = self.fh_part = None
        self.x8 = self.x32 = self.wmean = self.wlow = self.cs_ws = self.cs_tot = self.wh6_b = self._wh6_pad = None
        self.a1 = self.a2 = self.wh0_t = self.wh_last = None
        self.wh0_direct = self.wh0_fused = self.wh_fused = False
        self.prog_mask, self.prog_wh, self.prog_mh = [], [], []
        self.mh_warped = self.mh_last = self.mh_w = self.mh_low = None
        self.flow_region, self._flow_regions = None, {}
        self.wh_region, self._wh_regions = None, {}
        self._wh_dyn = {}
        self._wh_train = None
        self._plan_features()
        self._plan_update_block()
        if eng.weighted:
            self._plan_weight_head()
        if eng.mask_head:
            self._plan_mask_head()

    @staticmethod
    def _z(*s, dtype=torch.float32):
        return torch.zeros(*s, dtype=dtype, device="cuda")

    def _plan_features(self):
        eng, sp, hp, wp, hf, wf, P, z = self.eng, self.eng.spec, self.hp, self.wp, self.hf, self.wf, self.P, self._z
        self.img = [new_act(1, hp, wp, 3, cs=4), new_act(1, hp, wp, 3, cs=4)]
        self.f1rows = z(_ru(P, 128), sp.fdim)
        self.f1 = Act(self.f1rows[:P], 1, hf, wf, sp.fdim)
        x3 = self.prec_corr == "bf16x3"
        bf = lambda rows: (z(rows.shape[0], rows.shape[1] * (2 if x3 else 1), dtype=torch.bfloat16)
                           if self.prec != "fp32" else None)
        self.f1s = bf(self.f1rows)
        if self.otf and self.prec == "fp32":
            self.f1s = self.f1rows
        self.dims, self.f2rows, self.f2act, self.vol, self.f2s = [], [], [], [], []
        h, w = hf, wf
        for _ in range(sp.levels):
            self.dims.append((h, w))
            self.f2act.append(new_act(1, h, w, sp.fdim, zero=True))
            if self.otf:
                self.f2s.append(bf(self.f2act[-1].t) if self.prec != "fp32" else self.f2act[-1].t)
            else:
                n = ops.tiled_dims(h, w)[2]
                rows = z(_ru(n, 128), sp.fdim)
                self.f2rows.append(rows)
                self.f2s.append(bf(rows))
                self.vol.append(z(P, n, dtype=torch.bfloat16 if eng.volume_storage == "bf16" else torch.float32))
            h, w = h // 2, w // 2
        self.net0 = new_act(1, hf, wf, sp.hdim, zero=True)
        self.xbuf = new_act(1, hf, wf, sp.xdim, zero=True)
        self.flow_cat = self.xbuf.t[:, sp.flow_off:]
        self._enc_scratch = {}
        n_stat = 2 * math.ceil((hp // 2) * (wp // 2) / 64) * 128
        self.stats = (z(n_stat), z(n_stat))
        self.fin_ws = ops.inorm_ws("cuda")
        self._norm_slots = {}
        self.prog_f_src = self._encoder_program(eng.fnet, self.img[0], [(eng.fnet.conv2, self.f1, 0, EPI.EPI_LINEAR)])
        self.prog_f_dst = self._encoder_program(eng.fnet, self.img[1],
                                                [(eng.fnet.conv2, self.f2act[0], 0, EPI.EPI_LINEAR)])
        self.prog_c_src = self._encoder_program(eng.cnet, self.img[0],
                                                [(eng.cnet.conv2_net, self.net0, 0, EPI.EPI_TANH),
                                                 (eng.cnet.conv2_inp, self.xbuf, 0, EPI.EPI_RELU)])
        self.prog_volume = self._volume_program()

    def _plan_update_block(self):
        eng, sp, hf, wf, P, z, cp = self.eng, self.eng.spec, self.hf, self.wf, self.P, self._z, self._cp
        self.coords = z(P, 2)
        self.corr = new_act(1, hf, wf, sp.corr_c, cs=sp.corr_cs, zero=True)
        self.c1 = new_act(1, hf, wf, 96 if sp.small else 256, zero=True)
        self.cf = new_act(1, hf, wf, 128 if sp.small else 256, zero=True)
        self.fl1 = new_act(1, hf, wf, 64 if sp.small else 128, zero=True)
        self.flow4 = new_act(1, hf, wf, 2, cs=4, zero=True)
        self.inp_c = new_act(1, hf, wf, sp.cdim, zero=True)
        self.gate_bias = [(new_act(1, hf, wf, 2 * sp.hdim, zero=True), new_act(1, hf, wf, sp.hdim, zero=True))
                          for _ in eng.zr_inp]
        self.prog_gate_bias = []
        for k in range(len(eng.zr_inp)):
            self.prog_gate_bias += [Step("conv", cp(self.inp_c, eng.zr_inp[k], self.gate_bias[k][0])),
                                    Step("conv", cp(self.inp_c, eng.q_inp[k], self.gate_bias[k][1]))]
        self.zbuf = new_act(1, hf, wf, sp.hdim, zero=True)
        self.rh = new_act(1, hf, wf, sp.hdim, zero=True)
        self.hA = new_act(1, hf, wf, sp.hdim, zero=True)
        self.hB = new_act(1, hf, wf, sp.hdim, zero=True)
        self.fh = new_act(1, hf, wf, 128 if sp.small else 256, zero=True)
        self.delta = new_act(1, hf, wf, 2, cs=4, zero=True)
        self.flow_init = z(2, hf, wf)
        if self.otf:
            terms = 3 if self.prec_corr == "bf16x3" else (0 if self.prec == "fp32" else 1)
            self.lookup = ops.make_lookup_otf_params(self.f1s, self.f2s, self.dims, hf, wf, sp.fdim, self.coords,
                                                     self.corr.t, sp.radius, terms)
        else:
            self.lookup = ops.make_lookup_params(self.vol, self.dims, self.coords, self.corr.t, sp.radius)
        self.prog_iter_first = self._iter_program(first=True)
        self.prog_iter = self._iter_program(first=False)
        if not sp.small:
            self.mk = new_act(1, hf, wf, 256, zero=True)
            self.mask = new_act(1, hf, wf, 576, zero=True)
            self.prog_mask = [cp(self.hB, eng.mk1, self.mk, epi=EPI.EPI_RELU),
                              cp(self.mk, eng.mk2, self.mask)]
            k = next((i for i, st in enumerate(self.prog_iter) if st.tag == "fh1"), None)
            if PAIR_BRANCHES and k is not None and ops.pair_ok(self.prog_iter[k].arg, self.prog_mask[0]):
                self.prog_iter_last = (self.prog_iter[:k] + [Step("conv2", (self.prog_iter[k].arg, self.prog_mask[0]), "fh1+mk1")]
                                       + self.prog_iter[k + 1:])
        self.folded = self._fold_gather_programs()

    def _plan_weight_head(self):
        eng, sp, P, z, n = self.eng, self.eng.spec, self.P, self._z, self.eng.spec.nwin
        self.x8 = new_act(P, n, n, 5, cs=8, zero=True)
        self.wmean = z(P)
        self.wlow = z(P)
        self.cs_ws = z(256, sp.fdim, dtype=torch.float64)
        self.cs_tot = z(sp.fdim, dtype=torch.float64)
        self.wh6_b = torch.tensor([eng.wh6_b], dtype=torch.float32, device="cuda")
        cpw = lambda *a, **kw: self._cp(*a, precision=self.prec_wh, **kw)
        if eng.wh_std:
            self.a2 = new_act(P, n, n, 128)
            self.wh0_direct = n in (7, 9)
            self.wh0_fused = (eng.wh0_frag is not None and os.environ.get("WOFT_WH0_FUSED", "1") != "0"
                              and ops.select_conv(self.a2, eng.wh2, precision=self.prec_wh).kernel is Kernel.WINDOW_9X9)
            self.a1 = self.a2 if self.wh0_fused else new_act(P, n, n, 128)
            self.wh0_t = eng.wh0.wgt[:128].t().contiguous()
            self.prog_wh, self.wh_fused = self._wh_program(P, None)
            return
        x = self.x8
        if not eng.wh_flat0:
            self.x32 = x = new_act(P, n, n, 5, cs=32, zero=True)
        for pc in eng.wh_layers:
            out = new_act(P, n, n, pc.cout, cs=_ru(_ru(pc.cout, 4), 32), zero=True)
            self.prog_wh.append(cpw(x, pc, out, epi=EPI.EPI_RELU))
            x = out
        self.wh_last = x

    def _plan_mask_head(self):
        eng, sp, hf, wf = self.eng, self.eng.spec, self.hf, self.wf
        self.mh_warped = new_act(1, hf, wf, sp.fdim, zero=True)
        x = None
        for k, pc in enumerate(eng.mh_layers):
            out = new_act(1, hf, wf, pc.cout, cs=_ru(_ru(pc.cout, 4), 32), zero=True)
            src = dict(x2=self.mh_warped, c_split=sp.fdim) if k == 0 else {}
            self.prog_mh.append(self._cp(self.f1 if k == 0 else x, pc, out, epi=EPI.EPI_RELU, precision=self.prec_wh, **src))
            x = out
        self.mh_last = x
        self.mh_w = torch.zeros(x.cs, dtype=torch.float32)
        self.mh_w[:eng.mh_c] = eng.mh_wlast
        self.mh_w = self.mh_w.to("cuda")
        self.mh_low = self._z(self.P)

    def _fold_gather_programs(self):
        progs = [p for p in (self.prog_iter_first, self.prog_iter, self.prog_iter_last) if p is not None]
        if not (FOLD_GATHER and self.otf and all(p and p[-1].kind == "fh_gather" and p[0].kind == "lookup" for p in progs)):
            return None
        n_planes, bias2 = self.prog_iter[-1].arg
        lk = ops.copy_params(self.lookup)
        lk.fh_part, lk.fh_bias, lk.fh_delta = _lib.ptr(self.fh_part), _lib.ptr(bias2), _lib.ptr(self.delta.t)
        lk.fh_flow4, lk.fh_flow_cat = _lib.ptr(self.flow4.t), self.flow_cat.data_ptr()
# ... 121 lines not shown

    def _cp(self, *a, **kw):
        kw.setdefault("precision", self.prec)
        return ops.conv_params(*a, **kw)

    def _scratch(self, name, n, h, w, c):
        cs = _ru(c, 32)
        key = (name, h, w, cs)
        if key not in self._enc_scratch:
            self._enc_scratch[key] = new_act(n, h, w, c, cs=cs, zero=True)
        return self._enc_scratch[key]

    def _encoder_program(self, e, img, outputs):
        prog = []
        inorm = e.norm == "instance"
        tag = "i" if inorm else "c"

        def slot(name):
            key = f"{tag}_{name}"
            if key not in self._norm_slots:
                self._norm_slots[key] = (torch.zeros(256, device="cuda"), torch.zeros(256, device="cuda"))
            return self._norm_slots[key]

        def materialise(x):
            if not isinstance(x, list):
                return x
            if x[4] is None:
                _, raw_x, mode, ms, _ = x
                x[4] = self._scratch(f"{tag}_mat_{len(prog)}", 1, raw_x.h, raw_x.w, raw_x.c)
                prog.append(Step("apply", (raw_x, x[4], mode - 1, None, ms, None, 0)))
            return x[4]

        def layer(x, pc, name, relu, res=None, defer=False):
            xin, in_norm, in_stats = x, 0, None
            if isinstance(x, list):
                _, raw_x, mode, ms, mat = x
                if mat is None and ops.select_conv(raw_x, pc, in_norm=mode, precision=self.prec).in_norm:
                    xin, in_norm, in_stats = raw_x, mode, ms
                else:
                    xin = materialise(x)
            ho, wo = pc.out_hw(xin.h, xin.w)
            out = self._scratch(f"{tag}_{name}", 1, ho, wo, pc.cout)
            kw = dict(in_norm=in_norm, in_stats=in_stats) if in_norm else {}
            if not inorm:
                epi = EPI.EPI_RELU_RES_RELU if res is not None else (EPI.EPI_RELU if relu else EPI.EPI_LINEAR)
                prog.append(Step("conv", self._cp(xin, pc, out, epi=epi, e0=materialise(res) if res is not None else None, **kw)))
                return out
            raw = self._scratch(f"{tag}_raw_{name}", 1, ho, wo, pc.cout)
            p = self._cp(xin, pc, raw, stats=self.stats, **kw)
            rows = 2 * p._m_tiles
            ms = slot(name)
            prog.append(Step("conv", p))
            prog.append(Step("fin", (rows, pc.cout_pad, pc.cout, raw.cs, p._m, ms)))
            if defer and res is None:
                return ["raw", raw, 2 if relu else 1, ms, None]
            if res is None:
                prog.append(Step("apply", (raw, out, 1 if relu else 0, None, ms, None, 0)))
            elif isinstance(res, list) and res[4] is None:
                prog.append(Step("apply", (raw, out, 2, res[1], ms, res[3], res[2])))
            else:
                prog.append(Step("apply", (raw, out, 2, materialise(res), ms, None, 0)))
            return out

        x = layer(img, e.conv1, "c1", True, defer=inorm and DEFER_NORM)
        for i, blk in enumerate(e.blocks):
            res = x if blk["stride"] == 1 else layer(x, blk["down"], f"b{i}_d", False, defer=inorm and DEFER_NORM)
            y = x
            for k, pc in enumerate(blk["convs"][:-1]):
                y = layer(y, pc, f"b{i}_{k}", True, defer=inorm)
            x = layer(y, blk["convs"][-1], f"b{i}_o", True, res=res)
        x = materialise(x)
        for pc, out, co_off, epi in outputs:
            prog.append(Step("conv", self._cp(x, pc, out, co_off=co_off, epi=epi)))
        return prog

    def _volume_program(self):
        sp = self.eng.spec
        prog = []
        alpha = 1.0 / math.sqrt(float(sp.fdim))
        x3 = self.prec_corr == "bf16x3"
        if self.otf and self.prec != "fp32" and PYRAMID_ONE_LAUNCH and sp.fdim % 32 == 0 and self.f2act[0].cs == sp.fdim and sp.levels <= 4:
            return [Step("pyramid", ops.PyramidArgs(self.f2act[:sp.levels], self.f2s[:sp.levels], 3 if x3 else 1))]
        for l in range(sp.levels):
            if l > 0:
                prog.append(Step("pool", (self.f2act[l - 1], self.f2act[l])))
            if self.otf:
                if self.prec != "fp32":
                    prog.append(Step("split", (self.f2act[l].t, self.f2s[l])))
                continue
            prog.append(Step("tile", (self.f2act[l], self.f2rows[l])))
            if self.prec == "fp32":
                prog.append(Step("conv", ops.corr_volume(self.f1, self.f2rows[l], self.vol[l].shape[1], self.vol[l], alpha)))
            else:
                prog.append(Step("split", (self.f2rows[l], self.f2s[l])))
                prog.append(Step("cgemm", (self.f1s, self.f2s[l], self.P, self.vol[l].shape[1], alpha, self.vol[l],
                                       3 if x3 else 1)))
        return prog

    def _iter_program(self, first):
        e, cp, sp = self.eng, self._cp, self.eng.spec
        hd = sp.hdim
        h_in = self.net0 if first else self.hB
        prog = [Step("lookup", self.lookup)]
        if sp.small:
            prog += [Step("conv", cp(self.corr, e.convc1, self.cf, co_off=0, epi=EPI.EPI_RELU)),
                     Step("conv", cp(self.flow4, e.convf1, self.fl1, epi=EPI.EPI_RELU)),
                     Step("conv", cp(self.fl1, e.convf2, self.cf, co_off=96, epi=EPI.EPI_RELU)),
                     Step("conv", cp(self.cf, e.convm, self.xbuf, co_off=sp.cdim, epi=EPI.EPI_RELU))]
        else:
            flo = [Step("conv", cp(self.flow4, e.convf1, self.fl1, epi=EPI.EPI_RELU), "convf1"),
                   Step("conv", cp(self.fl1, e.convf2, self.cf, co_off=192, epi=EPI.EPI_RELU), "convf2")]
            cor = [Step("conv", cp(self.corr, e.convc1, self.c1, epi=EPI.EPI_RELU), "convc1"),
                   Step("conv", cp(self.c1, e.convc2, self.cf, co_off=0, epi=EPI.EPI_RELU), "convc2")]
            if PAIR_BRANCHES:
                for c_, f_ in zip(cor, flo):
                    if ops.pair_ok(c_.arg, f_.arg):
                        prog.append(Step("conv2", (c_.arg, f_.arg), c_.tag + "+" + f_.tag))
                    else:
                        prog += [c_, f_]
            else:
                prog += cor + flo
            prog.append(Step("conv", cp(self.cf, e.convm, self.xbuf, co_off=sp.cdim, epi=EPI.EPI_RELU), "convm"))
        steps = len(e.zr_dyn)
        states = [h_in, self.hA, self.hB] if steps == 2 else [h_in, self.hB]
        if steps == 1 and not first:
            states = [self.hB, self.hA]
        for k in range(steps):
            hi, ho = states[k], states[k + 1]
            gz, gq = self.gate_bias[k]
            pzr = cp(hi, e.zr_dyn[k], self.zbuf, x2=self.xbuf, x2_off=sp.cdim, c_split=hd,
                     epi=EPI.EPI_GRU_ZR, split=hd, e0=hi, out1=self.rh, bias_map=gz)
            pq = cp(self.rh, e.q_dyn[k], ho, x2=self.xbuf, x2_off=sp.cdim, c_split=hd,
                    epi=EPI.EPI_GRU_Q, e0=hi, e1=self.zbuf, bias_map=gq)
            prog += [Step("conv", pzr, f"gru_zr{k}"), Step("conv", pq, f"gru_q{k}")]
        if steps == 1 and not first:
            prog.append(Step("copy", (self.hA.t, self.hB.t)))
        fused = None
        if e.fh2_frag is not None and e.fh2.cout == 2:
            if self.fh_part is None:
                self.fh_part = torch.zeros(4 * self.P, 20, dtype=torch.float32, device="cuda")
            fused = ops.flowhead_params(self.hB, e.fh1, self.fh_part, e.fh2_frag, precision=self.prec)
        if fused is not None:
            prog += [Step("conv", fused, "fh1"), Step("fh_gather", (fused._n_planes, e.fh2.bias[:2].contiguous()))]
            return prog
        prog.append(Step("conv", cp(self.hB, e.fh1, self.fh, epi=EPI.EPI_RELU), "fh1"))
        if ops.narrow_ok(self.fh, e.fh2):
            prog.append(Step("fh_update", (self.fh, e.fh2, self.delta)))
        else:
            prog += [Step("conv", cp(self.fh, e.fh2, self.delta)), Step("coords", None)]
        return prog

    def run(self, prog):
        ev = self.conv_events
        for kind, a, tag in prog:
            if kind == "conv":
                ops.run_conv(a) if ev is None else _timed(ev.get(tag), ops.run_conv, a)
            elif kind == "conv2":
                ops.run_conv_pair(*a) if ev is None else _timed(ev.get(tag), ops.run_conv_pair, *a)
            elif kind == "fin":
                rows, ld, c, c_pad, count, ms = a
                ops.inorm_finalize(self.stats, rows, ld, c, count, ms[0], ms[1], channels_pad=c_pad, ws=self.fin_ws)
            elif kind == "apply":
                raw, out, mode, res, ms, res_ms, res_mode = a
                ops.inorm_apply(raw, ms[0], ms[1], out, mode, res=res, res_stats=res_ms, res_mode=res_mode)
            elif kind == "pyramid":
                ops.feature_pyramid(a)
            elif kind == "pool":
                ops.avgpool2(a[0], a[1])
            elif kind == "split":
                self._split(a[0], a[1])
            elif kind == "tile":
                ops.tile_rows(a[0], a[1])
            elif kind == "cgemm":
                ops.corr_gemm_bf16(*a)
            elif kind == "lookup":
                self._lookup(a)
            elif kind == "copy":
                a[1].copy_(a[0])
            elif kind == "fh_gather":
                ops.flow_head_gather(self.fh_part, a[0], self.hf, self.wf, a[1], self.delta, self.coords, self.flow4.t,
                                     self.flow_cat, self.xbuf.cs)
            elif kind == "fh_update":
                ops.flow_head_update(a[0], a[1], a[2], self.coords, self.flow4.t, self.flow_cat, self.xbuf.cs)
            elif kind == "coords":
                ops.coords_update(self.coords, self.delta.t, self.delta.cs, self.wf, self.flow4.t, self.flow_cat, self.xbuf.cs)
            else:
                raise ValueError(kind)

    def _lookup(self, params):
        if self.band_valid:
            _timed(self.lookup_events, self._lookup_band, params)
            return
        _timed(self.lookup_events, ops.run_lookup_otf if self.otf else ops.run_lookup, params)

    def band_applies(self, lookups, has_init=False):
        e, sp = self.eng, self.eng.spec
        if not CORR_BAND or e.corr_band is False or not self.otf or self.prec == "fp32" or has_init:
            return False
        if (sp.radius, sp.fdim) not in ops.BAND_INSTANCES or sp.levels > 4:
            return False
        return e.corr_band is True or lookups >= BAND_MIN_LOOKUPS

    def _band_buffers(self):
        if self._band is None:
            sp = self.eng.spec
            rows = ops.band_geometry(sp.radius, sp.levels)[3]
            i32 = lambda n: torch.zeros(n, dtype=torch.int32, device="cuda")
            self._band = (torch.zeros(self.P * rows * ops.BAND_LD, dtype=torch.float32, device="cuda"), i32(self.P), i32(1))
        return self._band

    def _band_build(self):
        band, miss, count = self._band_buffers()
        count.zero_()
        ops.run_band_build(self._band_variant(self.lookup))
        self.band_valid = True

    def _band_variant(self, params):
        key = id(params)
        if key not in self._band_params:
            band, miss, count = self._band_buffers()
            fb = ops.copy_params(params)
            fb.fh_part, fb.need = None, _lib.ptr(miss)
            fb._keep = (getattr(params, "_keep", None), miss)
            self._band_params[key] = (params, ops.make_lookup_band_params(params, band, miss, count), fb)
        _, bp, fb = self._band_params[key]
        bp.need = params.need
        bp._fallback = fb
        return bp

    def _lookup_band(self, params):
        bp = self._band_variant(params)
        ops.run_lookup_band(bp)
        ops.run_lookup_otf(bp._fallback)

    @property
    def band_miss_blocks(self):
        return 0 if self._band is None else int(self._band[2].item())

    def _split(self, rows, out):
        if self.prec_corr == "bf16x3":
            ops.split_bf16_lines(rows, out)
        else:
            ops.split_bf16(rows, out, None)

    def _source_changed(self, owner=None):
        self.source_owner = owner
        self._operands_changed()

    def _target_changed(self, owner=None):
        self.target_owner, self.target_valid = owner, False
        self._operands_changed()

    def _operands_changed(self):
        self.band_valid = False

    @property
    def source_tag(self):
        return None if self.source_owner is None else self.source_owner[0]

    def load_image(self, slot, img_u8, pad_top, pad_left, owner=None):
        if slot == 0:
            self._source_changed()
        else:
            self._target_changed(owner)
        ops.preprocess(img_u8, self.img[slot], self.hp, self.wp, pad_top, pad_left)

    def encode_source(self, reuse_target=False, owner=None):
        reused = bool(reuse_target) and self.otf and self.target_valid
        self._source_changed(owner)
        if reused:
            self.f1rows[:self.P].copy_(self.f2act[0].t.view(self.P, -1))
            if self.prec != "fp32":
                self.f1s[:self.P].copy_(self.f2s[0])
        else:
            self.run(self.prog_f_src)
        self.run(self.prog_c_src)
        if self.prec != "fp32" and not reused:
            self._split(self.f1rows, self.f1s)
        self.inp_c.t.copy_(self.xbuf.t[:, :self.eng.spec.cdim])
        self.run(self.prog_gate_bias)
        return reused

    @property
    def record_dims(self):
        sp = self.eng.spec
        return sp.fdim, sp.hdim, sp.cdim

    def new_record(self):
        return torch.empty(ops.features_record_floats(self.P, *self.record_dims), dtype=torch.float32, device="cuda")

    def encode_record(self, record):
        self._source_changed()
        self._target_changed()
        self.run(self.prog_f_src)
        self.run(self.prog_c_src)
        ops.features_pack(self.f1rows, self.net0.t, self.xbuf.t, self.P, self.record_dims, record)

    def restore_source(self, record):
        x3 = self.prec != "fp32" and self.prec_corr == "bf16x3"
        self._source_changed()
        ops.features_unpack(record, self.P, self.record_dims, self.f1rows, self.f1s if x3 else None, self.net0.t, self.xbuf.t,
                            self.inp_c.t)
        if self.prec != "fp32" and not x3:
            self._split(self.f1rows, self.f1s)
        self.run(self.prog_gate_bias)

    def restore_target(self, record):
        self._target_changed()
        ops.features_unpack(record, self.P, self.record_dims, self.f2act[0].t)

    def set_flow_init(self, flow_init):
        if tuple(flow_init.shape) != (2, self.hf, self.wf):
            raise ValueError(f"flow_init must have shape (2, {self.hf}, {self.wf}) for a {self.hp} x {self.wp} padded input, "
                             f"got {tuple(flow_init.shape)}")
        self.flow_init.copy_(flow_init, non_blocking=True)

    def flow_low(self):
        return self.flow4.t[:, :2].t().reshape(2, self.hf, self.wf).contiguous()

    def flow(self, iters, crop, h, w, flow_up=None, dst=None, wout=None, do_sigmoid=False, trace=None, defer_wh=False,
             mout=None, mask_sigmoid=False, flow_init=None, skip_wh=False, target_restored=False, graph=False):
        if iters < 1:
            raise ValueError("iters must be >= 1")
        if self._wh_train is not None:
            self._wh_train["gen"] += 1
        if flow_init is not None and flow_init is not True:
            self.set_flow_init(flow_init)
        region = self.flow_region if (trace is None and flow_init is None) else None
        if region is not None and region["key"][1] != iters:
            region = None
        launch = lambda: self._flow(iters, crop, h, w, flow_up, dst, wout, do_sigmoid, trace, defer_wh, mout, mask_sigmoid,
                                    flow_init is not None, skip_wh, target_restored, region)
        if not graph or trace is not None or any(ev is not None for ev in (self.lookup_events, self.wh_events, self.conv_events)):
            return launch()
        key = FlowKey(iters, crop, h, w, _lib.ptr(flow_up), _lib.ptr(dst), _lib.ptr(wout), _lib.ptr(mout), bool(do_sigmoid),
                      bool(mask_sigmoid), bool(defer_wh), bool(skip_wh), flow_init is not None, bool(target_restored),
                      _lib.ptr(self.wh_region[0]) if self.wh_region is not None else None, region["key"] if region is not None else None)
        g = self._graphs.get(key)
        if g is not None:
            g.replay()
            self.band_valid, self.target_valid = g.post
            return
        launch()
        if key in self._graphs:
            g = _FlowGraph()
            with torch.cuda.graph(g):
                launch()
            g.post = (self.band_valid, self.target_valid)
        self._graphs[key] = g

    def _flow(self, iters, crop, h, w, flow_up, dst, wout, do_sigmoid, trace, defer_wh, mout, mask_sigmoid, has_init, skip_wh,
              target_restored, region):
        e, sp = self.eng, self.eng.spec
        self._target_changed(self.target_owner)
        if not target_restored:
            self.run(self.prog_f_dst)
        self.run(self.prog_volume)
        self.target_valid = True
        if self.band_applies(iters + (1 if e.weighted and not skip_wh else 0), has_init):
            self._band_build()
        if not has_init:
            ops.coords_init(self.coords, self.hf, self.wf, self.flow4.t, self.flow_cat, self.xbuf.cs)
        else:
            ops.coords_init_flow(self.coords, self.flow_init, self.hf, self.wf, self.flow4.t, self.flow_cat, self.xbuf.cs)
            if trace is not None:
                trace(self, -1)
        folded = self.folded is not None and trace is None
        for it in range(iters):
            prog = self._iteration(it, iters, folded)
            self.run(prog if region is None else region["iters"].get(it, prog))
            if trace is not None:
                trace(self, it)
        if folded:
            self.run(self.folded.gather)
        for p in self.prog_mask[1 if iters > 1 and self.prog_iter_last is not None else 0:]:
            ops.run_conv(p)
        if defer_wh or skip_wh:
            assert not defer_wh or (e.weighted and not sp.small and self.wh_region is not None and not e.mask_head)
            self._upsample(None, crop, h, w, flow_up=flow_up, dst=dst, wout=None, do_sigmoid=do_sigmoid)
            return
        if e.weighted:
            index, prog = self.wh_region if self.wh_region is not None else (None, self.prog_wh)
            self._weight_head(prog, index)
        wout = wout if e.weighted else None
        self._upsample(self.wlow, crop, h, w, flow_up=flow_up, dst=dst, wout=wout, do_sigmoid=do_sigmoid)
        if e.mask_head:
            self._mask_head()
            if mout is not None:
                self._upsample(self.mh_low, crop, h, w, wout=mout, do_sigmoid=mask_sigmoid)

    def _upsample(self, wlow, crop, h, w, **outputs):
        if self.eng.spec.small:
            ops.upflow8(self.coords, wlow, self.hf, self.wf, crop, h, w, **outputs)
        else:
            ops.convex_upsample(self.coords, wlow, self.mask.t, self.hf, self.wf, crop, h, w, **outputs)

    def _mask_head(self):
        e = self.eng
        ops.warp_features(self.f2act[0], self.coords, self.mh_warped)
        for p in self.prog_mh:
            ops.run_conv(p)
        ops.wh_reduce(self.mh_last, 1, self.mh_w, e.mh_b, self.P, self.mh_low)

    def finish_weights(self, pts, count, n_max, pad, crop, h, w, flow_up=None, dst=None, wout=None, do_sigmoid=False,
                       w_points=None):
        index, _ = self.wh_region[:2]
        key = index.data_ptr()
        if key not in self._wh_dyn:
            dyn = torch.full_like(index, -1)
            prog, fused = self._wh_program(int(index.numel()), dyn)
            assert fused
            self._wh_dyn[key] = (dyn, prog, torch.zeros(self.P, dtype=torch.int32, device=index.device),
                                 torch.zeros(1, dtype=torch.int32, device=index.device))
        dyn, prog, bitmap, n_needed = self._wh_dyn[key]
        ops.wh_needed(pts, count, n_max, pad[0], pad[1], self.hf, self.wf, index, bitmap, dyn, n_needed)
        self._weight_head(prog, dyn, n_needed, need=bitmap)
        if w_points is not None:
            ops.convex_weights_at(pts, count, n_max, self.wlow, self.mask.t, self.hf, self.wf, crop, w_points,
                                  do_sigmoid=do_sigmoid)
            return
        self._upsample(self.wlow, crop, h, w, flow_up=flow_up, dst=dst, wout=wout, do_sigmoid=do_sigmoid)

    def refresh_weight_head(self):
        e = self.eng
        self.wh0_t.copy_(e.wh0.wgt[:128].t())
        self.wh6_b.fill_(e.wh6_b)
        if self._wh6_pad is not None:
            self._wh6_pad[:e.wh6_c].copy_(e.wh6_w[:e.wh6_c])
        self._graphs.clear()

    def _wh6_padded(self, cs):
        if self._wh6_pad is None or self._wh6_pad.numel() != cs:
            self._wh6_pad = torch.zeros(cs, dtype=torch.float32, device="cuda")
            self._wh6_pad[:self.eng.wh6_c] = self.eng.wh6_w[:self.eng.wh6_c]
        return self._wh6_pad

    def _head_input(self, need, x8):
        sp = self.eng.spec
        if self.otf:
            self.lookup.need = _lib.ptr(need)
        self._lookup(self.lookup)
        if self.otf:
            self.lookup.need = None
        ops.colsum(self.f2act[0].t, self.P, sp.fdim, self.cs_ws, self.cs_tot)
        ops.wh_pack(self.corr, self.f1, self.cs_tot, 1.0 / (math.sqrt(float(sp.fdim)) * self.P), sp.nwin, self.wmean, x8)

    def _weight_head(self, prog_wh, index, n_needed=None, need=None):
        e, n = self.eng, self.eng.spec.nwin
        self._head_input(need, None if self.wh0_direct else self.x8)
        if self.x32 is not None:
            self.x32.t[:, :8].copy_(self.x8.t)
        n_win = int(index.numel()) if index is not None else self.P
        if index is not None:
            self.wlow.zero_()
        if self.wh0_direct and not self.wh0_fused:
            ops.wh_conv0(self.corr, self.wmean, n_win, n, self.wh0_t, e.wh0.bias, self.a1, index)
        _timed(self.wh_events, ops.run_conv, prog_wh[0], extra=lambda: n_win if n_needed is None else n_needed.clone())
        for p in prog_wh[1:]:
            ops.run_conv(p)
        if not self.wh_fused:
            last = self.a1 if e.wh_std else self.wh_last
            ops.wh_reduce(last, n * n, self._wh6_padded(last.cs), e.wh6_b, self.P, self.wlow)

    def _wh_train_buffers(self, n_max):
        cap = 9 * n_max
        t = self._wh_train
        if t is None or t["cap"] < cap:
            z, P = self._z, self.P
            i32 = lambda *s: torch.zeros(*s, dtype=torch.int32, device="cuda")
            t = dict(cap=cap, x8=z(cap, 81, 8), act=[z(cap, 81, 128) for _ in range(3)], g=[z(cap, 81, 128) for _ in range(2)],
                     out=z(cap), wlow=z(P), g_wlow=z(P), bitmap=i32(P), dyn=i32(P),
                     all=torch.arange(P, dtype=torch.int32, device="cuda"),
                     ws=z(ops.wh_wgrad_ws_floats(cap, 128)), ws64=z(-(-cap // ops.WH_TRAIN_CHUNK) * 129, dtype=torch.float64),
                     gen=0 if t is None else t["gen"])
            self._wh_train = t
        return t

    def wh_train_forward(self, params, pts, count, n_max, pad, crop, do_sigmoid=False):
        sp, n = self.eng.spec, self.eng.spec.nwin
        assert self.eng.weighted and self.eng.wh_std and not sp.small and n == 9 and 0 < n_max <= ops.HFIT_SINGLE_MAX
        t = self._wh_train_buffers(n_max)
        t["gen"] += 1
        w0, b0, w2, b2, w4, b4, w6, b6 = (p.detach() for p in params)
        wsel = torch.zeros(n_max, dtype=torch.float32, device="cuda")
        ops.wh_needed(pts, count, n_max, pad[0], pad[1], self.hf, self.wf, t["all"], t["bitmap"], t["dyn"])
        index = t["dyn"][t["dyn"] >= 0].contiguous()
        n_win = int(index.numel())
        if n_win == 0:
            return wsel, None
        self._head_input(t["bitmap"], None)
        li = index.long()
        x8 = t["x8"][:n_win]
        x8[:, :, :4] = self.corr.t[li, :4 * n * n].view(n_win, n * n, 4)
        x8[:, :, 4] = self.wmean[li][:, None]
        wh_train.head_forward(x8, n_win, (w0, b0, w2, b2, w4, b4, w6), t["act"], t["out"])
        t["wlow"].zero_()
        t["wlow"][li] = t["out"][:n_win] + b6.reshape(())
        ops.convex_weights_at(pts, count, n_max, t["wlow"], self.mask.t, self.hf, self.wf, crop, wsel, do_sigmoid=do_sigmoid)
        return wsel, dict(gen=t["gen"], index=index, n_win=n_win, pts=pts, count=count, n_max=n_max, crop=crop,
                          do_sigmoid=bool(do_sigmoid), w2=w2.clone(), w4=w4.clone(), w6=w6.reshape(-1).clone())

    def wh_train_backward(self, state, g_wsel):
        z = lambda *s: torch.zeros(*s, dtype=torch.float32, device="cuda")
        gw0, gb0, gw2, gb2, gw4, gb4, gw6, gb6 = z(128, 5, 3, 3), z(128), z(128, 128, 3, 3), z(128), z(128, 128, 3, 3), z(128), \
            z(1, 128, 1, 1), z(1)
        grads = (gw0, gb0, gw2, gb2, gw4, gb4, gw6, gb6)
# ... 13 lines not shown
```

### woft_amd/flow_provider.py

```python
import logging
import os
from collections import OrderedDict
from pathlib import Path
from timeit import default_timer as timer

import numpy as np
import torch

from . import _lib, ops, wh_train
from .engine import RaftEngine

logger = logging.getLogger(__name__)


def _pad_geometry(h, w, mode):
    if mode == "nopad":
        assert h % 8 == 0
        assert w % 8 == 0
        return h, w, 0, 0, h, w, h, w
    if mode == "crop":
        ch, cw = (h // 8) * 8, (w // 8) * 8
        return ch, cw, 0, 0, ch, cw, ch, cw
    if mode == "RAFT":
        ph = (((h // 8) + 1) * 8 - h) % 8
        pw = (((w // 8) + 1) * 8 - w) % 8
        return h + ph, w + pw, ph // 2, pw // 2, h, w, h, w
    if mode == "Michal":
        raise NotImplementedError("padding_mode 'Michal' (raft.py:250-271) fails in the reference itself for "
                                  "raft_type 'orig'/'weighted'; it is not provided on the HIP path")
    raise ValueError(f"invalid padding_mode '{mode}'")


def _mask_head_shapes(structure, fdim):
    try:
        layers = [tuple(d) if isinstance(d, (list, tuple)) else (d, 3) for d in structure]
        shapes, cur = [], 2 * fdim
        for c, k in layers:
            c, k = int(c), int(k)
            if c < 1 or k < 1 or k % 2 == 0:
                raise ValueError
            shapes.append((c, cur, k, k))
            cur = c
    except (TypeError, ValueError):
        raise ValueError(f"class_params.mask_head_structure {structure!r}: not a list of (channels, odd kernel) tuples "
                         "or channel counts (weighted_raft.py:387-409)") from None
    return shapes + [(1, cur, 1, 1)]


class FrameFeatures:

    def __init__(self, provider, record, geometry, size):
        self.provider, self.record = provider, record
        self.geometry, self.size = tuple(int(v) for v in geometry), tuple(int(v) for v in size)

    @property
    def shape(self):
        return self.size + (3,)

    @property
    def nbytes(self):
        return self.record.numel() * self.record.element_size()

    def __repr__(self):
        return f"FrameFeatures({self.size[0]} x {self.size[1]}, padded geometry {self.geometry}, {self.nbytes} bytes)"


class _Recent:

    def __init__(self):
        self.order, self.protected = OrderedDict(), None

    def touch(self, key, keep, protect=False):
        if protect:
            self.protected = key
        self.order[key] = None
        self.order.move_to_end(key)
        others = [k for k in self.order if k != self.protected]
        dropped = others[:max(0, len(others) - keep)]
        for k in dropped:
            del self.order[k]
        return dropped


class _LastFlow:

    def __init__(self, low_plan=None):
        self.low_plan = low_plan
        self.wh = None
        self.flow_map = None
        self.deferred = None


class RAFTWrapper:
    def __init__(self, config):
        self.C = config
        cp = config.class_params
        if self.C.raft_type not in ("orig", "weighted", "weighted_masked"):
            raise ValueError(f"Unknown RAFT type {self.C.raft_type}")
        self.masked = self.C.raft_type == "weighted_masked"
        if self.masked and not cp.mask_estimation:
            raise ValueError("raft_type 'weighted_masked' needs class_params.mask_estimation = True (and mask_head_structure): "
                             "without the MaskHead the network has no mask output")
        if self.C.raft_type == "weighted" and cp.mask_estimation:
            raise ValueError("class_params.mask_estimation is set with raft_type 'weighted', which returns no mask: use raft_type "
                             "'weighted_masked'")
        self._cache_mask_warned = False
        logger.info(f"Loading weights from: {self.C.model}")

        def read(src):
            sd = src if isinstance(src, dict) else torch.load(src, map_location="cpu")
            return {(k[len("module."):] if k.startswith("module.") else k): v for k, v in sd.items()}
        state_dict = read(self.C.model)
        if self.C.backbone_model:
            in_backbone = lambda k: ("fnet" in k) or ("cnet" in k) or ("update_block" in k)
            state_dict = {k: v for k, v in state_dict.items() if not in_backbone(k)}
            state_dict.update({k: v for k, v in read(self.C.backbone_model).items() if in_backbone(k)})
        weighted = self.C.raft_type in ("weighted", "weighted_masked")
        small = bool(cp.small)
        if self.masked:
            if not cp.mask_head_structure:
                raise ValueError("raft_type 'weighted_masked' needs class_params.mask_head_structure (weighted_raft.py:387-409)")
            want = _mask_head_shapes(cp.mask_head_structure, 128 if small else 256)
            idx = sorted(int(k.split(".")[2]) for k in state_dict if k.startswith("mask_head.net.") and k.endswith(".weight"))
            got = [tuple(state_dict[f"mask_head.net.{i}.weight"].shape) for i in idx]
            if got != want or idx != list(range(0, 2 * len(want), 2)):
                raise ValueError(f"class_params.mask_head_structure {cp.mask_head_structure!r} expects mask_head.net layers {want}; "
                                 f"the checkpoint has {got} (at net.{idx})")
        for src, val in (("env WOFT_PRECISION", os.environ.get("WOFT_PRECISION")),
                         ("flow config key 'precision'", self.C.precision),
                         ("class_params.mixed_precision", "fp16" if cp.mixed_precision else None),
                         ("built-in default (no key in the flow config): fp32-emulating bf16x3 -- finer than the TF32 convolutions "
                          "the reference's torch 1.8.1 runs by default on Ampere; 'fp32' = exact products", "bf16x3")):
            if val:
                self.precision, self.precision_source = str(val), src
                break
        note = (f"RAFT arithmetic: precision = '{self.precision}' (from: {self.precision_source}). "
                + ("This is the reference's arithmetic (exact IEEE fp32 products)." if self.precision == "fp32" else
                   "NOT the reference's IEEE-fp32 products: set precision = 'fp32' in the flow config (or WOFT_PRECISION=fp32) "
                   "for the reference's arithmetic (about 4x slower)."))
        logger.log(logging.WARNING if self.precision_source.startswith("built-in default") else logging.INFO, note)
        self.precision_note = note
        self.corr = os.environ.get("WOFT_CORR") or getattr(self.C, "corr", None) or "otf"
        v = getattr(self.C, "corr_band", None)
        self.corr_band = "auto" if (v is None or isinstance(v, type(self.C))) else (v if v == "auto" else bool(v))
        self.engine = RaftEngine(state_dict, small=small, weighted=weighted, precision=self.precision, corr=self.corr,
                                 volume_storage=getattr(self.C, "volume_storage", None), mask_head=self.masked,
                                 corr_band=self.corr_band)
        self._wh_loaded = {k: v for k, v in state_dict.items() if k.startswith("weight_head.net.")}
        self._wh_params = None
        v = getattr(self.C, "flow_region", None)
        self.flow_region_on = (os.environ.get("WOFT_FLOW_REGION", "1") != "0") if (v is None or isinstance(v, type(self.C))) else bool(v)
        self.use_graph = (os.environ.get("WOFT_GRAPH") or str(int(bool(getattr(self.C, "graph", False))))) == "1"
        self._pinned, self._pins = None, 0
        self._wmask, self._wregion, self._all_pixels = None, {}, {}
        self._fmask, self._fregion = None, {}
        self.weights_deferred, self._last = False, _LastFlow()
        self.defer_min_ratio = 6
        self._out = {}
        self._cache_errors = set()
        self.source_features_reused = False
        self._plan_bound = None
        self._recent_plans, self._recent_outs, self._recent_pixels = _Recent(), _Recent(), _Recent()

    def bound_plans(self, n_other):
        self._plan_bound = None if n_other is None else max(1, int(n_other))

    def _touch_plan(self, plan_key, out_key, n_pix, pinned_here):
        n = self._plan_bound
        if n is None:
            return
        for key in self._recent_plans.touch(plan_key, n, protect=pinned_here):
            self.engine.drop_plan(key)
        for key in self._recent_outs.touch(out_key, n, protect=pinned_here):
            self._out.pop(key, None)
        for key in self._recent_pixels.touch(n_pix, n, protect=pinned_here):
            self._all_pixels.pop(key, None)

    def finish_weights(self, pts, count, n_max, out=None):
        plan, crop, oh, ow, o, do_sigmoid = self._last.deferred
        self._last.deferred = None
        plan.finish_weights(pts, count, n_max, crop, crop, oh, ow, flow_up=o["flow"], dst=o["dst"], wout=o["w"],
                            do_sigmoid=do_sigmoid, w_points=out)
        return o["w"] if out is None else out

    @property
    def _wh_flow(self):
        return self._last.wh

    def _wh_trainable(self):
        eng = self.engine
        why = (f"raft_type '{self.C.raft_type}' (only 'weighted' is covered)" if self.C.raft_type != "weighted" else
               "the small model (its head reads 7x7 windows of another lookup)" if eng.small else
               "a weight_head_structure other than [(128, 3), (128, 3), (128, 3)]" if not eng.wh_std else
               "a weights_postprocessing_fn between the head and the weights" if self.C.weights_postprocessing_fn else None)
        if why:
            raise NotImplementedError(f"training of the weight head is not provided for {why}")

    def weight_head_parameters(self):
        self._wh_trainable()
        if self._wh_params is None:
            self._wh_params = wh_train.make_parameters(self._wh_loaded)
        return self._wh_params

    def weights_at(self, pts, count=None, do_sigmoid=False):
        self._wh_trainable()
        if self._last.wh is None:
            raise RuntimeError("weights_at(): no computed flow to evaluate the head on (none yet, or the last one came from the "
                               "flow cache)")
        if not (isinstance(pts, torch.Tensor) and pts.is_cuda and pts.dtype == torch.float32 and pts.dim() == 2
                and pts.shape[1] == 2 and pts.shape[0] >= 1):
            raise TypeError("weights_at(): pts must be a (n_max, 2) float32 device tensor of (x, y) pixels")
        if pts.shape[0] > ops.HFIT_SINGLE_MAX:
            raise ValueError(f"weights_at(): at most {ops.HFIT_SINGLE_MAX} points per call, got {pts.shape[0]}")
        if count is not None and not (isinstance(count, torch.Tensor) and count.is_cuda and count.dtype == torch.int32
                                      and count.numel() == 1):
            raise TypeError("weights_at(): count must be a device int32 scalar")
        plan, crop = self._last.wh
        params = self.weight_head_parameters().values()
        return wh_train.weights_at(plan, params, pts.detach().contiguous(), count, int(pts.shape[0]), crop, do_sigmoid)

    def sync_weight_head(self):
        self.engine.repack_weight_head({k: v.detach() for k, v in self.weight_head_parameters().items()})

    def pin_source(self, src_img):
        self._pinned = src_img
        self._pins += 1
        self._wmask, self._wregion = None, {}
        self._fmask, self._fregion = None, {}

    def pin_flow_region(self, mask):
        self._fmask = None if mask is None else np.ascontiguousarray(np.asarray(mask) > 0)
        self._fregion = {}

    def _flow_region(self, key, hp, wp, top, left, oh, ow):
        if self._fmask is None:
            return None
        if key not in self._fregion:
            ys, xs = np.nonzero(self._fmask[:oh, :ow])
            rect = None
            if ys.size:
                y0, y1, x0, x1 = (ys.min() + top) >> 3, (ys.max() + top) >> 3, (xs.min() + left) >> 3, (xs.max() + left) >> 3
                rect = (int(y0), int(x0), int(y1 - y0 + 1), int(x1 - x0 + 1))
            self._fregion[key] = rect
        return self._fregion[key]

    def pin_weight_region(self, mask):
        self._wmask = None if mask is None else np.ascontiguousarray(np.asarray(mask) > 0)
        self._wregion = {}

    def _weight_region(self, key, hp, wp, top, left, oh, ow):
        if self._wmask is None:
            return None
        if key not in self._wregion:
            m = self._wmask[:oh, :ow]
            coarse = np.zeros((hp // 8, wp // 8), bool)
            ys, xs = np.nonzero(m)
            coarse[(ys + top) >> 3, (xs + left) >> 3] = True
            pad = np.pad(coarse, 1)
            dil = np.zeros_like(coarse)
            for dy in range(3):
                for dx in range(3):
                    dil |= pad[dy:dy + coarse.shape[0], dx:dx + coarse.shape[1]]
            idx = np.flatnonzero(dil).astype(np.int32)
            self._wregion[key] = torch.from_numpy(idx).cuda() if idx.size and idx.size < dil.size else None
        return self._wregion[key]

    def postprocess_weights(self, flat_weights, fn):
        s = self.last_flow_shape
        weights = fn(flat_weights.reshape(s["batch"], 1, s["H"], s["W"]))
        return weights.reshape(s["batch"], s["H"] * s["W"])

    def _outputs(self, h, w):
        key = (h, w)
        if key not in self._out:
            z = lambda *s: torch.empty(*s, dtype=torch.float32, device="cuda")
            self._out[key] = dict(flow=z(2, h, w), dst=z(2, h * w), w=z(1, h * w),
                                  src=torch.stack([torch.arange(h * w, device="cuda") % w,
                                                   torch.div(torch.arange(h * w, device="cuda"), w, rounding_mode="floor")]))
            if self.masked:
                self._out[key]["m"] = z(1, h * w)
        return self._out[key]

    def _cached_flow(self, src_img, identifier, mode, numpy_out, do_sigmoid, borrow=False):
        dataset_name, seq_name, frame_i = identifier
        self._last = _LastFlow(self._last.low_plan)
        path = Path(self.C.flow_cache_dir) / dataset_name / seq_name / f"{frame_i}-{frame_i + 1}.npz"
        data = np.load(path, allow_pickle=False)
        flow = np.ascontiguousarray(data["half_flow"].astype(np.float32))
        wts = data["half_weights"].astype(np.float32)
        wts = np.ascontiguousarray(wts) if wts.size > 1 else None
        h, w = flow.shape[1:]
        post = self.C.weights_postprocessing_fn if wts is not None else None
        o = self._outputs(h, w)
        o["flow"].copy_(torch.from_numpy(flow), non_blocking=True)
        wl = None
        if wts is not None:
            wl = torch.from_numpy(wts).cuda(non_blocking=True)
        lib = _lib.load()
        _lib.check(lib.woft_flow_to_tc(_lib.ptr(o["flow"]), _lib.ptr(wl), h, w, _lib.ptr(o["dst"]),
                                       _lib.ptr(o["w"]) if wl is not None else None, int(bool(do_sigmoid) and not post),
# ... 194 lines not shown
```

### woft_amd/ops.py

```python
import ctypes as C
import math
import os
from dataclasses import dataclass

import numpy as np
import torch

from . import _lib, conv_select
from ._lib import ConvParams, LookupBandParams, LookupOtfParams, LookupParams, check, ptr, stream_ptr
from .conv_select import KERNELS, PRECISION, Kernel, pair_ok

DEV = "cuda"


def _round_up(x, m):
    return (x + m - 1) // m * m


@dataclass
class Act:
    t: torch.Tensor
    n: int
    h: int
    w: int
# ... 274 lines not shown
    assert part.shape[0] >= n_planes * x.n_pix and part.shape[1] >= 20 and x.n == 1
    p.e0, p.lde0 = ptr(frags), 0
    p._keep = p._keep + (part, frags)
    p._n_planes = n_planes
    return p


def flow_head_gather(part, n_planes, h, w, bias2, delta, coords, flow4=None, flow_cat=None, ld_cat=0):
    check(_lib.load().woft_flow_head_gather(ptr(part), n_planes, part.shape[1], h, w, ptr(bias2), ptr(delta.t), delta.cs,
                                            ptr(coords), ptr(flow4), ptr(flow_cat), ld_cat, stream_ptr()),
          "woft_flow_head_gather")


def run_conv_pair(a, b):
    check(_lib.load().woft_conv2d_pair(C.byref(a), C.byref(b), stream_ptr()), "woft_conv2d_pair")


def run_conv(p):
    check(_lib.load().woft_conv2d(C.byref(p), stream_ptr()), "woft_conv2d")


def conv2d(x, pc, c_out_stride=None, **kw):
    ho, wo = pc.out_hw(x.h, x.w)
    out = kw.pop("out", None) or new_act(x.n, ho, wo, pc.cout, cs=c_out_stride or _round_up(pc.cout, 4), zero=True)
    p = conv_params(x, pc, out, ho=ho, wo=wo, **kw)
    run_conv(p)
    return out


def inorm_ws(device="cuda"):
    return torch.zeros(int(_lib.load().woft_inorm_ws_bytes()), dtype=torch.uint8, device=device)


def inorm_finalize(stats, n_part, ld, channels, count, mean, rstd, eps=1e-5, channels_pad=None, ws=None):
    check(_lib.load().woft_inorm_finalize(ptr(stats[0]), ptr(stats[1]), n_part, ld, channels, channels_pad or channels,
                                          count, eps, ptr(mean), ptr(rstd), ptr(ws), stream_ptr()), "woft_inorm_finalize")


def inorm_apply(x, mean, rstd, out, mode, res=None, res_stats=None, res_mode=0):
    assert out.cs == x.cs and (res is None or res.cs == x.cs)
    rm, rr = res_stats if res_stats is not None else (None, None)
    check(_lib.load().woft_inorm_apply(ptr(x.t), ptr(mean), ptr(rstd), ptr(res.t) if res is not None else None,
                                       ptr(rm), ptr(rr), res_mode, ptr(out.t), x.n_pix, x.cs, mode, stream_ptr()),
          "woft_inorm_apply")


class PyramidArgs:
    def __init__(self, maps, splits, terms):
        import ctypes
        self.maps, self.splits, self.terms = maps, splits, terms
        self.levels = len(maps)
        assert 1 <= self.levels <= 4 and len(splits) == self.levels and all(m.cs == maps[0].cs == m.c for m in maps)
        for l in range(1, self.levels):
            assert (maps[l].h, maps[l].w) == (maps[l - 1].h // 2, maps[l - 1].w // 2)
        self.pooled = (ctypes.c_void_p * 3)(*[maps[l].t.data_ptr() if l < self.levels else None for l in range(1, 4)])
        self.split = (ctypes.c_void_p * 4)(*[splits[l].data_ptr() if l < self.levels else None for l in range(4)])


def feature_pyramid(a):
    m = a.maps[0]
    check(_lib.load().woft_feature_pyramid(ptr(m.t), m.h, m.w, m.cs, a.levels, a.pooled, a.split, a.terms, stream_ptr()),
          "woft_feature_pyramid")


def preprocess(img_u8, out, hp, wp, pad_top, pad_left):
    h, w = img_u8.shape[:2]
    check(_lib.load().woft_preprocess_bgr_u8(ptr(img_u8), h, w, ptr(out.t), hp, wp, pad_top, pad_left, stream_ptr()),
          "woft_preprocess_bgr_u8")


def avgpool2(x, out):
    check(_lib.load().woft_avgpool2_nhwc(ptr(x.t), x.h, x.w, x.cs, ptr(out.t), stream_ptr()), "woft_avgpool2_nhwc")


def split_bf16(x, hi, lo=None):
    check(_lib.load().woft_split_bf16(ptr(x), x.numel(), ptr(hi), ptr(lo), stream_ptr()), "woft_split_bf16")


def conv3x3_narrow(x, pc, out, co_off=0):
    assert (pc.taps_y, pc.taps_x, pc.stride, pc.pad_y, pc.pad_x, pc.flat) == (3, 3, 1, 1, 1, 0) and pc.cout <= 2
    assert out.n == x.n and out.h == x.h and out.w == x.w
    check(_lib.load().woft_conv3x3_narrow(ptr(x.t), x.cs, x.n, x.h, x.w, pc.cin_pad, ptr(pc.wgt), ptr(pc.bias), pc.cout,
                                          ptr(out.t), out.cs, co_off, stream_ptr()), "woft_conv3x3_narrow")


def flow_head_update(x, pc, delta, coords, flow4=None, flow_cat=None, ld_cat=0):
    assert narrow_ok(x, pc) and pc.cout == 2 and x.n == 1 and coords.shape[0] == x.h * x.w
    check(_lib.load().woft_flow_head_update(ptr(x.t), x.cs, x.h, x.w, pc.cin_pad, ptr(pc.wgt), ptr(pc.bias), ptr(delta.t),
                                            delta.cs, ptr(coords), ptr(flow4), ptr(flow_cat), ld_cat, stream_ptr()),
          "woft_flow_head_update")


def narrow_ok(x, pc):
    return ((pc.taps_y, pc.taps_x, pc.stride, pc.pad_y, pc.pad_x, pc.flat) == (3, 3, 1, 1, 1, 0) and pc.cout <= 2
            and pc.cin_pad in (128, 256) and x.cs >= pc.cin_pad)


def make_lookup_otf_params(f1s, f2s, dims, hf, wf, k, coords, out, radius, terms):
    p = LookupOtfParams()
    p.f1 = ptr(f1s)
    for l, (t, (h, w)) in enumerate(zip(f2s, dims)):
        p.f2[l], p.h[l], p.w[l] = ptr(t), h, w
    p.levels, p.radius, p.terms = len(f2s), radius, terms
    p.hf, p.wf, p.k = hf, wf, k
    p.alpha = 1.0 / math.sqrt(float(k))
    p.coords, p.out, p.ldo = ptr(coords), ptr(out), out.shape[1]
    p._keep = (f1s, f2s, coords, out)
    return p


def run_lookup_otf(p):
    check(_lib.load().woft_corr_lookup_otf(C.byref(p), stream_ptr()), "woft_corr_lookup_otf")


BAND_M0, BAND_LD = 3, 16
BAND_INSTANCES = ((4, 256), (3, 128))


def band_m(l):
    return (BAND_M0 + (1 << l) - 1) >> l


def band_geometry(radius, levels):
    m = [band_m(l) for l in range(levels)]
    w = [2 * (radius + 1 + ml) for ml in m]
    off = [sum(w[:l]) for l in range(levels)]
    return m, w, off, sum(w)


def band_hit(cx, cy, x, y, levels):
    for l in range(levels):
        s = 1.0 / (1 << l)
        if abs(math.floor(cx * s) - (x >> l)) > band_m(l) or abs(math.floor(cy * s) - (y >> l)) > band_m(l):
            return False
    return True


def make_lookup_band_params(otf, band, miss, miss_count):
    p = LookupBandParams()
    C.memmove(C.byref(p), C.byref(otf), C.sizeof(LookupOtfParams))
    p.band, p.miss, p.miss_count = ptr(band), ptr(miss), ptr(miss_count)
    p._keep = (getattr(otf, "_keep", None), band, miss, miss_count)
    return p


def run_band_build(p):
    check(_lib.load().woft_corr_band_build(C.byref(p), stream_ptr()), "woft_corr_band_build")


def run_lookup_band(p):
    check(_lib.load().woft_corr_lookup_band(C.byref(p), stream_ptr()), "woft_corr_lookup_band")


def split_bf16_lines(x, out):
    check(_lib.load().woft_split_bf16_lines(ptr(x), x.numel(), ptr(out), stream_ptr()), "woft_split_bf16_lines")


def features_record_floats(n_pix, fdim, hdim, cdim):
    return n_pix * (fdim + hdim + cdim)


def features_pack(f1rows, net, xbuf, n_pix, dims, record):
    fdim, hdim, cdim = dims
    assert record.dtype == torch.float32 and record.is_contiguous() and record.numel() == features_record_floats(n_pix, *dims)
    assert f1rows.shape[0] >= n_pix and net.shape[0] >= n_pix and xbuf.shape[0] >= n_pix
    check(_lib.load().woft_features_pack(ptr(f1rows), f1rows.stride(0), ptr(net), net.stride(0), ptr(xbuf), xbuf.stride(0),
                                         n_pix, fdim, hdim, cdim, ptr(record), stream_ptr()), "woft_features_pack")


def features_unpack(record, n_pix, dims, fmap, fmap_split=None, net=None, xbuf=None, inp_c=None):
    fdim, hdim, cdim = dims
    assert record.dtype == torch.float32 and record.is_contiguous() and record.numel() == features_record_floats(n_pix, *dims)
    assert fmap.shape[0] >= n_pix and all(t is None or t.shape[0] >= n_pix for t in (fmap_split, net, xbuf, inp_c))
    ld = lambda t: 0 if t is None else t.stride(0)
    check(_lib.load().woft_features_unpack(ptr(record), n_pix, fdim, hdim, cdim, ptr(fmap), ld(fmap), ptr(fmap_split), ptr(net),
                                           ld(net), ptr(xbuf), ld(xbuf), ptr(inp_c), ld(inp_c), stream_ptr()),
          "woft_features_unpack")


def corr_gemm_bf16(a, b, m, n, alpha, out, terms):
    k = a.shape[1] // 2 if terms == 3 else a.shape[1]
    assert out.dtype in (torch.float32, torch.bfloat16)
    check(_lib.load().woft_corr_gemm_bf16(ptr(a), ptr(b), m, n, a.shape[0], b.shape[0], k, float(alpha), ptr(out),
                                          out.shape[1], terms, int(out.dtype == torch.bfloat16), stream_ptr()),
          "woft_corr_gemm_bf16")


def corr_volume(f1, f2_rows, n_q, out, alpha, precision=0, f2_hi=None, f2_lo=None):
    p = ConvParams()
    p.in0, p.cs0, p.in1, p.cs1, p.c_split = ptr(f1.t), f1.cs, None, 0, f1.cs
    p.n_img, p.h, p.w, p.ho, p.wo = 1, f1.h, f1.w, f1.h, f1.w
    p.taps_y = p.taps_x = p.stride = 1
    p.pad_y = p.pad_x = 0
    p.cin_pad, p.flat = f1.cs, 0
    p.wgt, p.bias, p.alpha = ptr(f2_rows), None, alpha
    p.wgt_hi, p.wgt_lo, p.precision = ptr(f2_hi), ptr(f2_lo), PRECISION.get(precision, precision)
    p.cout, p.cout_pad = n_q, f2_rows.shape[0]
    p.out, p.ldo, p.co_off = ptr(out), out.shape[1], 0
    p.out_w, p.out_pitch = 0, 0
    p.epi = _lib.EPI_LINEAR
    p.tile_m, p.tile_n = (128, 128) if f2_rows.shape[0] % 128 == 0 else (128, 64)
    p.halo = Kernel.GATHER
    p._keep = (f1, f2_rows, out, f2_hi, f2_lo)
    return p


def tiled_dims(h, w, tw=4):
    ht, wt = (h + 3) // 4, (w + tw - 1) // tw
    return ht, wt, ht * wt * 4 * tw


def tile_rows(x, out):
    check(_lib.load().woft_tile_rows(ptr(x.t), x.h, x.w, x.cs, ptr(out), stream_ptr()), "woft_tile_rows")


def tile_planes(planes, tw=4):
    P, h, w = planes.shape
    ht, wt, n = tiled_dims(h, w, tw)
    pad = torch.zeros(P, ht * 4, wt * tw, dtype=planes.dtype, device=planes.device)
    pad[:, :h, :w] = planes
    return pad.reshape(P, ht, 4, wt, tw).permute(0, 1, 3, 2, 4).reshape(P, n).contiguous()


def untile_planes(vol, h, w, tw=4):
    ht, wt, n = tiled_dims(h, w, tw)
    P = vol.shape[0]
    return vol[:, :n].reshape(P, ht, wt, 4, tw).permute(0, 1, 3, 2, 4).reshape(P, ht * 4, wt * tw)[:, :h, :w]


def make_lookup_params(vols, dims, coords, out, radius):
    p = LookupParams()
    assert len({v.dtype for v in vols}) == 1 and vols[0].dtype in (torch.float32, torch.bfloat16)
    p.vol_bf16 = int(vols[0].dtype == torch.bfloat16)
    for l, v in enumerate(vols):
        p.vol[l] = ptr(v)
        p.ht[l], p.wt[l], n = tiled_dims(*dims[l])
        assert v.shape[1] >= n
        p.plane[l] = v.shape[1]
    p.levels, p.radius = len(vols), radius
    p.coords, p.n_pix, p.out, p.ldo = ptr(coords), coords.shape[0], ptr(out), out.shape[1]
    p._keep = (vols, coords, out)
    return p


def run_lookup(p):
    check(_lib.load().woft_corr_lookup(C.byref(p), stream_ptr()), "woft_corr_lookup")


def coords_init(coords, hf, wf, flow4=None, flow_cat=None, ld_cat=0):
    check(_lib.load().woft_coords_init(ptr(coords), hf, wf, ptr(flow4), ptr(flow_cat), ld_cat, stream_ptr()),
          "woft_coords_init")


def coords_init_flow(coords, flow_init, hf, wf, flow4=None, flow_cat=None, ld_cat=0):
    assert flow_init.dtype == torch.float32 and flow_init.is_contiguous() and tuple(flow_init.shape) == (2, hf, wf)
    check(_lib.load().woft_coords_init_flow(ptr(coords), ptr(flow_init), hf, wf, ptr(flow4), ptr(flow_cat), ld_cat,
                                            stream_ptr()), "woft_coords_init_flow")


def forward_interpolate(flow, out=None):
    assert flow.dtype == torch.float32 and flow.is_contiguous() and flow.dim() == 3 and flow.shape[0] == 2
    if out is None:
        out = torch.empty_like(flow)
    assert out.dtype == torch.float32 and out.is_contiguous() and out.shape == flow.shape
    check(_lib.load().woft_forward_interpolate(ptr(flow), flow.shape[1], flow.shape[2], ptr(out), stream_ptr()),
          "woft_forward_interpolate")
    return out


def _f32c(t, *shape):
    return t.dtype == torch.float32 and t.is_contiguous() and t.is_cuda and (not shape or tuple(t.shape) == shape)


def sample_bilinear(data, x, y, out=None):
    assert data.dim() == 3 and _f32c(data) and x.dim() == 1 and _f32c(x) and _f32c(y, *x.shape)
    c, h, w = data.shape
    n = x.shape[0]
    if out is None:
        out = torch.empty((c, n), dtype=torch.float32, device=data.device)
    assert _f32c(out, c, n)
    check(_lib.load().woft_sample_bilinear(ptr(data), c, h, w, ptr(x), ptr(y), n, ptr(out), stream_ptr()), "woft_sample_bilinear")
    return out


def flow_chain(flow_ab, flow_bc, out=None):
    assert flow_ab.dim() == 3 and flow_ab.shape[0] == 2 and _f32c(flow_ab) and _f32c(flow_bc, *flow_ab.shape)
    if out is None:
        out = torch.empty_like(flow_ab)
    assert _f32c(out, *flow_ab.shape) and out.data_ptr() != flow_bc.data_ptr()
    check(_lib.load().woft_flow_chain(ptr(flow_ab), ptr(flow_bc), flow_ab.shape[1], flow_ab.shape[2], ptr(out), stream_ptr()),
          "woft_flow_chain")
    return out


def flow_fb(flow_ab, flow_ba, alpha=0.01, beta=0.5, err=None, ok=None, want_err=True, want_ok=True):
    assert flow_ab.dim() == 3 and flow_ab.shape[0] == 2 and _f32c(flow_ab) and _f32c(flow_ba, *flow_ab.shape)
    h, w = flow_ab.shape[1:]
    if err is None and want_err:
        err = torch.empty((h, w), dtype=torch.float32, device=flow_ab.device)
    if ok is None and want_ok:
        ok = torch.empty((h, w), dtype=torch.float32, device=flow_ab.device)
    assert (err is None or (_f32c(err) and err.numel() == h * w)) and (ok is None or (_f32c(ok) and ok.numel() == h * w))
    check(_lib.load().woft_flow_fb(ptr(flow_ab), ptr(flow_ba), h, w, float(alpha), float(beta), ptr(err), ptr(ok), stream_ptr()),
          "woft_flow_fb")
    return err, ok

# ... 368 lines not shown
```

Measured before the change: 122.8.

## Fuse band correlation sampling into the convc1 1x1 GEMM kernel

Adds a fused kernel that computes the band correlation samples for each 8x8 pixel tile straight into LDS and feeds them as the A operand of the convc1 1x1 GEMM. The separate write and re-read of the lookup output is skipped. The convf1 1x1 conv runs in the same launch as extra blocks. The band lookup kernel gains a defer_samples flag so it only does miss detection, and misses still go through the fallback path. This removes a global round trip and a launch per iteration, at the cost of a much more complex kernel that is specialized to radius 4, fdim 256, 4 levels and cin 352, with higher LDS pressure.

```diff
diff --git a/include/woft_hip.h b/include/woft_hip.h
--- a/include/woft_hip.h
+++ b/include/woft_hip.h
@@ -157,9 +157,11 @@
     float* band;
     int32_t* miss;
     int32_t* miss_count;
+    int32_t defer_samples;
 } woft_lookup_band_params;
 int woft_corr_band_build(const woft_lookup_band_params* p, void* stream);
 int woft_corr_lookup_band(const woft_lookup_band_params* p, void* stream);
+int woft_conv1x1_band(const woft_conv_params* c1, const woft_conv_params* f1, const woft_lookup_band_params* bp, void* stream);
 int woft_tile_rows(const float* in, int32_t h, int32_t w, int32_t c, float* out, void* stream);
 
 int woft_coords_update(float* coords1, const float* delta, int32_t ld_delta, int32_t wf, int64_t n_pix,
diff --git a/woft_amd/_lib.py b/woft_amd/_lib.py
--- a/woft_amd/_lib.py
+++ b/woft_amd/_lib.py
@@ -51,7 +51,7 @@
 
 
 class LookupBandParams(C.Structure):
-    _fields_ = LookupOtfParams._fields_ + [("band", vp), ("miss", vp), ("miss_count", vp)]
+    _fields_ = LookupOtfParams._fields_ + [("band", vp), ("miss", vp), ("miss_count", vp), ("defer_samples", i32)]
 
 
 _SIGS = {
@@ -68,6 +68,7 @@
     "woft_corr_band_geometry": (i32, [i32, i32, C.POINTER(i32), C.POINTER(i32), C.POINTER(i32)]),
     "woft_corr_band_build": (i32, [C.POINTER(LookupBandParams), vp]),
     "woft_corr_lookup_band": (i32, [C.POINTER(LookupBandParams), vp]),
+    "woft_conv1x1_band": (i32, [C.POINTER(ConvParams), C.POINTER(ConvParams), C.POINTER(LookupBandParams), vp]),
     "woft_conv3x3_narrow": (i32, [vp, i32, i32, i32, i32, i32, vp, vp, i32, vp, i64, i32, vp]),
     "woft_flow_head_update": (i32, [vp, i32, i32, i32, i32, vp, vp, vp, i64, vp, vp, vp, i32, vp]),
     "woft_flow_head_gather": (i32, [vp, i32, i32, i32, i32, vp, vp, i64, vp, vp, vp, i32, vp]),
diff --git a/woft_amd/build.py b/woft_amd/build.py
--- a/woft_amd/build.py
+++ b/woft_amd/build.py
@@ -63,7 +63,7 @@
         u.update(" ".join(FLAGS + extra).encode())
         return u.hexdigest()
     jobs = int(os.environ.get("WOFT_BUILD_JOBS", os.cpu_count() or 4))
-    weight = {"conv.hip": 8, "conv_regb.hip": 6, "conv_1x1.hip": 20}
+    weight = {"conv.hip": 8, "conv_regb.hip": 6, "conv_1x1.hip": 20, "conv_1x1_band.hip": 20}
     units.sort(key=lambda u: -(u[0].stat().st_size * weight.get(u[0].name, 1)))
     pending, running = [], []
     for src, obj, extra in units:
diff --git a/woft_amd/csrc/conv.hip b/woft_amd/csrc/conv.hip
--- a/woft_amd/csrc/conv.hip
+++ b/woft_amd/csrc/conv.hip
@@ -939,6 +939,7 @@
         return WOFT_EINVAL;
     return WOFT_OK;
 }
+int woft_conv_check(const woft_conv_params& p) { return conv_check(p); }
 #endif
 
 int WOFT_CAT2(woft_conv_dispatch_p, WOFT_ONLY_PREC)(const woft_conv_params& p, const woft_conv_params* second, void* stream) {
diff --git a/woft_amd/csrc/conv_1x1.hip b/woft_amd/csrc/conv_1x1.hip
--- a/woft_amd/csrc/conv_1x1.hip
+++ b/woft_amd/csrc/conv_1x1.hip
@@ -1,203 +1,6 @@
-#include "conv_common.h"
+#include "conv_1x1_tile.h"
 
 namespace {
-
-using woft::BK;
-
-template <int TERMS, int TN>
-struct Geom1x1 {
-    static constexpr int NP = (TERMS == 3) ? 2 : 1;
-    static constexpr int BM = 64, TM = 2;
-    static constexpr int WCOLS = 32 * TN, BN = 4 * WCOLS;
-    static constexpr int A_PLANE = BM * LDB, A_ELEMS = NP * A_PLANE;
-    static constexpr int ST = 2;
-    static constexpr int STAGE_ELEMS = 2 * 4 * ST * woft::STAGE_FLOATS;
-    static constexpr int SMEM_ELEMS = (2 * A_ELEMS > STAGE_ELEMS) ? 2 * A_ELEMS : STAGE_ELEMS;
-};
-
-template <int TERMS, int TN, bool FLAT, int DEPTH, int NB>
-__device__ __forceinline__ void tile_1x1(const woft_conv_params& p, const int m_tile, const int n_tile, __bf16* smem) {
-    using G = Geom1x1<TERMS, TN>;
-    constexpr int NP = G::NP, TM = G::TM, A_PLANE = G::A_PLANE, A_ELEMS = G::A_ELEMS, WCOLS = G::WCOLS, BN = G::BN;
-    static_assert(DEPTH % 2 == 0 && (2 * DEPTH) % NB == 0 && NB >= 2, "static ring slots");
-    constexpr int STEP_ELEMS = NP * 2 * 64 * 8;
-
-    const int tid = threadIdx.x;
-    const int lane = tid & 63;
-    const int wave = __builtin_amdgcn_readfirstlane(tid >> 6);
-    const int r32 = lane & 31, hh = lane >> 5;
-    const int row = tid >> 2, v = tid & 3;
-
-    int64_t M = (int64_t)p.n_img * p.ho * p.wo;
-    int64_t m0 = (int64_t)m_tile * G::BM;
-    if ((p.roi_y0 | p.roi_x0 | p.roi_h | p.roi_w) != 0) {
-        const int runs = (p.roi_w + G::BM - 1) / G::BM;
-        const int line = m_tile / runs, run = m_tile - line * runs;
-        const int img = line / p.roi_h, ry = line - img * p.roi_h;
-        m0 = ((int64_t)img * p.ho + p.roi_y0 + ry) * p.wo + p.roi_x0 + run * G::BM;
-        const int left = p.roi_w - run * G::BM;
-        M = m0 + (left < G::BM ? left : G::BM);
-    }
-    const int n0 = n_tile * BN;
-    const int nchunk = FLAT ? p.taps_y : p.cin_pad / BK;
-
-    const int abl = (p.out_w <= -12350 && p.out_w > -12358) ? -12350 - p.out_w : 0;
-    const bool rok = m0 + row < M;
-    const uint32_t pix = rok ? (uint32_t)(m0 + row) : 0u;
-    int oy = 0, img_row0 = 0;
-    uint32_t run0 = 0;
-    bool okx[2] = {true, true};
-    if constexpr (FLAT) {
-        const int hw = p.ho * p.wo;
-        const int img = (int)(pix / (uint32_t)hw), rem = (int)(pix - (uint32_t)img * (uint32_t)hw);
-        oy = rem / p.wo;
-        const int ox = rem - oy * p.wo;
-        img_row0 = img * p.h;
-#pragma unroll
-        for (int e = 0; e < 2; ++e) {
-            const int ixp = ox - p.pad_x + (8 * v + 4 * e) / p.cs0;
-            okx[e] = rok && ixp >= 0 && ixp < p.w;
-        }
-        run0 = (uint32_t)((ox - p.pad_x) * p.cs0 + 8 * v);
-    }
-    f32x4 rh[DEPTH][2];
-    auto load_a = [&](int chunk, auto slot_tag) {
-        constexpr int slot = decltype(slot_tag)::value;
-        if ((abl & 1) && chunk >= DEPTH) return;
-        const int ck = chunk < nchunk ? chunk : nchunk - 1;
-        if constexpr (FLAT) {
-            int iy = oy + ck - p.pad_y;
-            iy = iy < 0 ? 0 : (iy >= p.h ? p.h - 1 : iy);
-            const uint32_t rowoff = (uint32_t)(img_row0 + iy) * (uint32_t)(p.w * p.cs0);
-#pragma unroll
-            for (int e = 0; e < 2; ++e) rh[slot][e] = *(const f32x4*)(p.in0 + (okx[e] ? rowoff + run0 + 4 * e : 0u));
-        } else {
-            const int c0 = ck * BK;
-            const bool second = (p.in1 != nullptr) && (c0 >= p.c_split);
-            const float* base = second ? p.in1 : p.in0;
-            const uint32_t cs = (uint32_t)(second ? p.cs1 : p.cs0);
-            const uint32_t coff = (uint32_t)(second ? c0 - p.c_split : c0);
-            rh[slot][0] = *(const f32x4*)(base + (pix * cs + coff + 8 * v));
-            rh[slot][1] = *(const f32x4*)(base + (pix * cs + coff + 8 * v + 4));
-        }
-    };
-    auto store_a = [&](int chunk, __bf16* As, auto slot_tag) {
-        constexpr int slot = decltype(slot_tag)::value;
-        const f32x4 zero = {0.f, 0.f, 0.f, 0.f};
-        bool oky = true;
-        if constexpr (FLAT) {
-            const int iy = oy + chunk - p.pad_y;
-            oky = iy >= 0 && iy < p.h;
-        }
-        bf16x4 hi[2], lo[2];
-#pragma unroll
-        for (int e = 0; e < 2; ++e) {
-            const f32x4 val = (FLAT ? (okx[e] && oky) : rok) ? rh[slot][e] : zero;
-            hi[e] = cvt16<TERMS>(val);
-            if (NP == 2) lo[e] = __builtin_convertvector(val - widen_bf16x4(hi[e]), bf16x4);
-        }
-        *(bf16x8*)(As + row * LDB + 8 * v) = __builtin_shufflevector(hi[0], hi[1], 0, 1, 2, 3, 4, 5, 6, 7);
-        if (NP == 2) *(bf16x8*)(As + A_PLANE + row * LDB + 8 * v) = __builtin_shufflevector(lo[0], lo[1], 0, 1, 2, 3, 4, 5, 6, 7);
-    };
-
-    const __bf16* wstream[TN];
-#pragma unroll
-    for (int j = 0; j < TN; ++j) wstream[j] = (const __bf16*)p.wgt_frag + (int64_t)(n0 / 32 + wave * TN + j) * nchunk * STEP_ELEMS + lane * 8;
-    bf16x8 bq[NB][TN][NP];
-    auto fetch_b = [&](int step, auto slot_tag) {
-        constexpr int slot = decltype(slot_tag)::value;
-        if ((abl & 2) && step >= NB - 1) return;
-        const int s = step < 2 * nchunk ? step : 2 * nchunk - 1;
-        const int off = (s >> 1) * STEP_ELEMS + (s & 1) * 512;
-#pragma unroll
-        for (int j = 0; j < TN; ++j)
-#pragma unroll
-            for (int pl = 0; pl < NP; ++pl) bq[slot][j][pl] = *(const bf16x8*)(wstream[j] + off + pl * 1024);
-    };
-
-    f32x16 acc[TM][TN];
-#pragma unroll
-    for (int i = 0; i < TM; ++i)
-#pragma unroll
-        for (int j = 0; j < TN; ++j)
-#pragma unroll
-            for (int r = 0; r < 16; ++r) acc[i][j][r] = 0.f;
-    const int a_off = r32 * LDB + hh * 8;
-
-    [&]<int... D>(std::integer_sequence<int, D...>) {
-        (load_a(D, std::integral_constant<int, D>{}), ...);
-    }(std::make_integer_sequence<int, DEPTH>{});
-    [&]<int... S>(std::integer_sequence<int, S...>) {
-        (fetch_b(S, std::integral_constant<int, S>{}), ...);
-    }(std::make_integer_sequence<int, NB - 1>{});
-    store_a(0, smem, std::integral_constant<int, 0>{});
-    __syncthreads();
-
-    auto run_chunk = [&](int c, auto d_tag) {
-        constexpr int D = decltype(d_tag)::value;
-        const __bf16* As = smem + (D & 1) * A_ELEMS;
-        bf16x8 aq[2][TM][NP];
-        auto read_a = [&](auto s2_tag) {
-            constexpr int s2 = decltype(s2_tag)::value;
-#pragma unroll
-            for (int i = 0; i < TM; ++i)
-#pragma unroll
-                for (int pl = 0; pl < NP; ++pl) aq[s2][i][pl] = *(const bf16x8*)(As + a_off + i * 32 * LDB + pl * A_PLANE + s2 * 16);
-        };
-        read_a(std::integral_constant<int, 0>{});
-        read_a(std::integral_constant<int, 1>{});
-        [&]<int... S2>(std::integer_sequence<int, S2...>) {
-            ([&] {
-                constexpr int s2 = S2, slot = (2 * D + s2) % NB;
-                fetch_b(2 * c + s2 + NB - 1, std::integral_constant<int, (2 * D + s2 + NB - 1) % NB>{});
-                __builtin_amdgcn_sched_barrier(0);
-                if (NP == 2) {
-#pragma unroll
-                    for (int j = 0; j < TN; ++j)
-#pragma unroll
-                        for (int i = 0; i < TM; ++i) acc[i][j] = mma16<TERMS>(aq[s2][i][NP - 1], bq[slot][j][0], acc[i][j]);
-#pragma unroll
-                    for (int j = 0; j < TN; ++j)
-#pragma unroll
-                        for (int i = 0; i < TM; ++i) acc[i][j] = mma16<TERMS>(aq[s2][i][0], bq[slot][j][NP - 1], acc[i][j]);
-                }
-#pragma unroll
-                for (int j = 0; j < TN; ++j)
-#pragma unroll
-                    for (int i = 0; i < TM; ++i) acc[i][j] = mma16<TERMS>(aq[s2][i][0], bq[slot][j][0], acc[i][j]);
-                if constexpr (s2 == 0) {
-                    store_a(c + 1, smem + ((D + 1) & 1) * A_ELEMS, std::integral_constant<int, (D + 1) % DEPTH>{});
-                    load_a(c + DEPTH, std::integral_constant<int, D>{});
-                }
-                __builtin_amdgcn_sched_barrier(0);
-            }(), ...);
-        }(std::make_integer_sequence<int, 2>{});
-        __syncthreads();
-    };
-    for (int c0 = 0; c0 < nchunk; c0 += DEPTH) {
-        [&]<int... D>(std::integer_sequence<int, D...>) {
-            ((c0 + D < nchunk ? run_chunk(c0 + D, std::integral_constant<int, D>{}) : (void)0), ...);
-        }(std::make_integer_sequence<int, DEPTH>{});
-    }
-    if (abl & 4) {
-        float t = 0.f;
-#pragma unroll
-        for (int i = 0; i < TM; ++i)
-#pragma unroll
-            for (int j = 0; j < TN; ++j)
-#pragma unroll
-                for (int r = 0; r < 16; ++r) t += acc[i][j][r];
-        if (t == 12345.678f) p.out[0] = t;
-        return;
-    }
-    woft::conv_epilogue_t<TM, TN, G::BM, WCOLS, G::ST>(p, acc, (float*)smem + wave * G::ST * woft::STAGE_FLOATS,
-                                                        woft::LinearRows{m0, M}, n0, 0, wave, lane, m_tile);
-}
-
-__host__ __device__ __forceinline__ int m_tiles_1x1(const woft_conv_params& p) {
-    if ((p.roi_y0 | p.roi_x0 | p.roi_h | p.roi_w) != 0) return p.n_img * p.roi_h * ((p.roi_w + 63) / 64);
-    return (int)(((int64_t)p.n_img * p.ho * p.wo + 63) / 64);
-}
 
 
 template <int TERMS>
diff --git a/woft_amd/csrc/conv_1x1_band.hip b/woft_amd/csrc/conv_1x1_band.hip
--- /dev/null
+++ b/woft_amd/csrc/conv_1x1_band.hip
@@ -0,0 +1,322 @@
+#include "conv_1x1_tile.h"
+#include "lookup_blocks.h"
+
+int woft_conv_check(const woft_conv_params& p);
+
+namespace {
+
+struct BlockRows {
+    int py0, px0, hf, wf;
+    __device__ __forceinline__ int64_t operator()(int row) const {
+        const int y = py0 + (row >> 3), x = px0 + (row & 7);
+        return (y < hf && x < wf) ? (int64_t)y * wf + x : -1;
+    }
+};
+
+template <int TERMS>
+struct GeomBand {
+    using G = Geom1x1<TERMS, 2>;
+    static constexpr int R = 4, NW = 2 * R + 1, N2 = NW * NW, WS = NW + 1, LEVELS = 4;
+    static constexpr int RING = 4;
+    static constexpr int RS = WOFT_BAND_LD + 4;
+    static constexpr int HR = 6, PLD = HR * RS;
+    static constexpr int RING_ELEMS = RING * G::A_ELEMS;
+    static constexpr int WIN_ELEMS = 64 * PLD * 2;
+    static constexpr int SMEM_ELEMS = RING_ELEMS + WIN_ELEMS;
+    static_assert(SMEM_ELEMS >= G::STAGE_ELEMS && SMEM_ELEMS >= Geom1x1<TERMS, 1>::SMEM_ELEMS, "one LDS array for every phase");
+    static_assert((RING_ELEMS * 2) % 16 == 0, "the windows start 16-byte aligned");
+};
+
+template <int TERMS>
+__global__ __launch_bounds__(256, 2) void conv1x1_band_kernel(const woft_conv_params pa, const woft_conv_params pb,
+                                                              const woft_lookup_band_params bp, const int split) {
+    using GB = GeomBand<TERMS>;
+    using G = Geom1x1<TERMS, 2>;
+    constexpr int NP = G::NP, TM = G::TM, TN = 2, A_PLANE = G::A_PLANE, A_ELEMS = G::A_ELEMS, WCOLS = G::WCOLS;
+    constexpr int R = GB::R, NW = GB::NW, WS = GB::WS, RS = GB::RS, PLD = GB::PLD, NT = 256, NB = 4, NCHUNK = 11;
+    constexpr int STEP_ELEMS = NP * 2 * 64 * 8;
+    __shared__ __attribute__((aligned(16))) __bf16 smem[GB::SMEM_ELEMS];
+    __shared__ int s_ox[GB::LEVELS][64], s_oy[GB::LEVELS][64];
+    __shared__ float s_fx[GB::LEVELS][64], s_fy[GB::LEVELS][64];
+
+    if ((int)blockIdx.x >= split) {
+        int m_tile, n_tile;
+        woft::tile_of_block((int)blockIdx.x - split, m_tiles_1x1(pb), pb.cout_pad / 128, m_tile, n_tile);
+        tile_1x1<TERMS, 1, true, 4, 4>(pb, m_tile, n_tile, smem);
+        return;
+    }
+    const woft_lookup_otf_params& p = bp.otf;
+    __bf16* const ring = smem;
+    float* const Wl = (float*)(smem + GB::RING_ELEMS);
+
+    const int tid = threadIdx.x;
+    const int lane = tid & 63;
+    const int wave = __builtin_amdgcn_readfirstlane(tid >> 6);
+    const int r32 = lane & 31, hh = lane >> 5;
+    const int tiles_x = (p.wf + 7) / 8;
+    int tile;
+    {
+        const int q = split / 8, rr = split % 8, xcd = blockIdx.x % 8, idx = blockIdx.x / 8;
+        tile = (xcd < rr ? xcd * (q + 1) : rr * (q + 1) + (xcd - rr) * q) + idx;
+    }
+    const int px0 = (tile % tiles_x) * 8, py0 = (tile / tiles_x) * 8;
+
+    const __bf16* wstream[TN];
+#pragma unroll
+    for (int j = 0; j < TN; ++j) wstream[j] = (const __bf16*)pa.wgt_frag + (int64_t)(wave * TN + j) * NCHUNK * STEP_ELEMS + lane * 8;
+    bf16x8 bq[NB][TN][NP];
+    auto fetch_b = [&](int step, auto slot_tag) {
+        constexpr int slot = decltype(slot_tag)::value;
+        const int s = step < 2 * NCHUNK ? step : 2 * NCHUNK - 1;
+        const int off = (s >> 1) * STEP_ELEMS + (s & 1) * 512;
+#pragma unroll
+        for (int j = 0; j < TN; ++j)
+#pragma unroll
+            for (int pl = 0; pl < NP; ++pl) bq[slot][j][pl] = *(const bf16x8*)(wstream[j] + off + pl * 1024);
+    };
+    [&]<int... S>(std::integer_sequence<int, S...>) {
+        (fetch_b(S, std::integral_constant<int, S>{}), ...);
+    }(std::make_integer_sequence<int, NB - 1>{});
+
+    int ok = 1;
+    {
+        const int y = py0 + (lane >> 3), x = px0 + (lane & 7);
+        const bool cvalid = tid < 64 && y < p.hf && x < p.wf;
+        if (cvalid) {
+            const int64_t i = (int64_t)y * p.wf + x;
+            const float cx = p.coords[i * 2], cy = p.coords[i * 2 + 1];
+#pragma unroll
+            for (int l = 0; l < GB::LEVELS; ++l) {
+                const float sc = 1.0f / (float)(1 << l);
+                const float xs = cx * sc, ys = cy * sc;
+                float flx = floorf(xs), fly = floorf(ys);
+                s_fx[l][tid] = xs - flx;
+                s_fy[l][tid] = ys - fly;
+                flx = fminf(fmaxf(flx, -1.0e6f), 1.0e6f);
+                fly = fminf(fmaxf(fly, -1.0e6f), 1.0e6f);
+                const int m = WOFT_BAND_M(l);
+                const int ox = (int)flx - (x >> l) + m, oy = (int)fly - (y >> l) + m;
+                ok &= (ox >= 0 && ox <= 2 * m && oy >= 0 && oy <= 2 * m) ? 1 : 0;
+                s_ox[l][tid] = ox;
+                s_oy[l][tid] = oy;
+            }
+        } else if (tid < 64) {
+#pragma unroll
+            for (int l = 0; l < GB::LEVELS; ++l) {
+                s_fx[l][tid] = s_fy[l][tid] = 0.f;
+                s_ox[l][tid] = s_oy[l][tid] = 0;
+            }
+        }
+    }
+    const bool hit = __builtin_amdgcn_readfirstlane(__syncthreads_and(ok)) != 0;
+
+    constexpr int ROWS = 16 + 14 + 12 + 12;
+    f32x4 pc[GB::HR];
+    auto load_half = [&](auto l_tag, auto h_tag) __attribute__((always_inline)) {
+        constexpr int l = decltype(l_tag)::value, half = decltype(h_tag)::value;
+        constexpr int NR = half == 0 ? 6 : 5, R0 = half == 0 ? 0 : 5;
+        constexpr int roff = l == 0 ? 0 : (l == 1 ? 16 : (l == 2 ? 30 : 42));
+        static_assert(64 * NR * 4 == NR * NT, "NR pieces per thread");
+#pragma unroll
+        for (int k = 0; k < NR; ++k) {
+            const int it = tid + k * NT;
+            const int pix = it / (4 * NR), rem = it - pix * (4 * NR);
+            const int gy = py0 + (pix >> 3), gx = px0 + (pix & 7);
+            pc[k] = f32x4{0.f, 0.f, 0.f, 0.f};
+            if (gy < p.hf && gx < p.wf) {
+                const int ox = s_ox[l][pix];
+                pc[k] = *(const f32x4*)(bp.band + (((int64_t)gy * p.wf + gx) * ROWS + roff + ox + R0) * WOFT_BAND_LD + rem * 4);
+            }
+        }
+    };
+    auto store_half = [&](auto h_tag) __attribute__((always_inline)) {
+        constexpr int half = decltype(h_tag)::value;
+        constexpr int NR = half == 0 ? 6 : 5;
+#pragma unroll
+        for (int k = 0; k < NR; ++k) {
+            const int it = tid + k * NT;
+            const int pix = it / (4 * NR), rem = it - pix * (4 * NR);
+            *(f32x4*)(Wl + pix * PLD + (rem >> 2) * RS + (rem & 3) * 4) = pc[k];
+        }
+    };
+    auto sample = [&](auto l_tag, int pix, int c, int lrow) __attribute__((always_inline)) {
+        constexpr int l = decltype(l_tag)::value;
+        const int gy = py0 + (pix >> 3), gx = px0 + (pix & 7);
+        if (gy >= p.hf || gx >= p.wf) return;
+        const float fx = s_fx[l][pix], fy = s_fy[l][pix];
+        const float* cq = Wl + pix * PLD + lrow * RS + s_oy[l][pix];
+        float h[WS];
+#pragma unroll
+        for (int j = 0; j < WS; ++j) h[j] = cq[j] * (1.f - fx) + cq[RS + j] * fx;
+        float o[12];
+#pragma unroll
+        for (int j = 0; j < NW; ++j) o[j] = h[j] * (1.f - fy) + h[j + 1] * fy;
+        o[9] = o[10] = o[11] = 0.f;
+        const int ch0 = l * GB::N2 + c * NW;
+#pragma unroll
+        for (int g = 0; g < 3; ++g) {
+            const f32x4 val = {o[4 * g], o[4 * g + 1], o[4 * g + 2], o[4 * g + 3]};
+            const bf16x4 hi = cvt16<TERMS>(val);
+            bf16x4 lo = hi;
+            if (NP == 2) lo = __builtin_convertvector(val - widen_bf16x4(hi), bf16x4);
+#pragma unroll
+            for (int e = 0; e < 4; ++e) {
+                if (4 * g + e >= NW) continue;
+                const int ch = ch0 + 4 * g + e;
+                __bf16* a = ring + ((ch >> 5) & (GB::RING - 1)) * A_ELEMS + pix * LDB + (ch & 31);
+                a[0] = hi[e];
+                if (NP == 2) a[A_PLANE] = lo[e];
+            }
+        }
+    };
+    const int row = tid >> 2, v = tid & 3;
+    const int64_t mrow = BlockRows{py0, px0, p.hf, p.wf}(row);
+    auto fill_chunk = [&](int chunk) __attribute__((always_inline)) {
+        const f32x4 zero = {0.f, 0.f, 0.f, 0.f};
+        f32x4 rh[2] = {zero, zero};
+        if (mrow >= 0) {
+            const uint32_t off = (uint32_t)mrow * (uint32_t)pa.cs0 + (uint32_t)(chunk * BK + 8 * v);
+            rh[0] = *(const f32x4*)(pa.in0 + off);
+            rh[1] = *(const f32x4*)(pa.in0 + off + 4);
+        }
+        bf16x4 hi[2], lo[2];
+#pragma unroll
+        for (int e = 0; e < 2; ++e) {
+            hi[e] = cvt16<TERMS>(rh[e]);
+            if (NP == 2) lo[e] = __builtin_convertvector(rh[e] - widen_bf16x4(hi[e]), bf16x4);
+        }
+        __bf16* As = ring + (chunk & (GB::RING - 1)) * A_ELEMS;
+        *(bf16x8*)(As + row * LDB + 8 * v) = __builtin_shufflevector(hi[0], hi[1], 0, 1, 2, 3, 4, 5, 6, 7);
+        if (NP == 2) *(bf16x8*)(As + A_PLANE + row * LDB + 8 * v) = __builtin_shufflevector(lo[0], lo[1], 0, 1, 2, 3, 4, 5, 6, 7);
+    };
+
+    f32x16 acc[TM][TN];
+#pragma unroll
+    for (int i = 0; i < TM; ++i)
+#pragma unroll
+        for (int j = 0; j < TN; ++j)
+#pragma unroll
+            for (int r = 0; r < 16; ++r) acc[i][j][r] = 0.f;
+    const int a_off = r32 * LDB + hh * 8;
+    auto run_chunk = [&](auto c_tag) __attribute__((always_inline)) {
+        constexpr int c = decltype(c_tag)::value;
+        const __bf16* As = ring + (c & (GB::RING - 1)) * A_ELEMS;
+        bf16x8 aq[2][TM][NP];
+#pragma unroll
+        for (int s2 = 0; s2 < 2; ++s2)
+#pragma unroll
+            for (int i = 0; i < TM; ++i)
+#pragma unroll
+                for (int pl = 0; pl < NP; ++pl) aq[s2][i][pl] = *(const bf16x8*)(As + a_off + i * 32 * LDB + pl * A_PLANE + s2 * 16);
+        [&]<int... S2>(std::integer_sequence<int, S2...>) {
+            ([&] {
+                constexpr int s2 = S2, slot = (2 * c + s2) % NB;
+                fetch_b(2 * c + s2 + NB - 1, std::integral_constant<int, (2 * c + s2 + NB - 1) % NB>{});
+                __builtin_amdgcn_sched_barrier(0);
+                if (NP == 2) {
+#pragma unroll
+                    for (int j = 0; j < TN; ++j)
+#pragma unroll
+                        for (int i = 0; i < TM; ++i) acc[i][j] = mma16<TERMS>(aq[s2][i][NP - 1], bq[slot][j][0], acc[i][j]);
+#pragma unroll
+                    for (int j = 0; j < TN; ++j)
+#pragma unroll
+                        for (int i = 0; i < TM; ++i) acc[i][j] = mma16<TERMS>(aq[s2][i][0], bq[slot][j][NP - 1], acc[i][j]);
+                }
+#pragma unroll
+                for (int j = 0; j < TN; ++j)
+#pragma unroll
+                    for (int i = 0; i < TM; ++i) acc[i][j] = mma16<TERMS>(aq[s2][i][0], bq[slot][j][0], acc[i][j]);
+                __builtin_amdgcn_sched_barrier(0);
+            }(), ...);
+        }(std::make_integer_sequence<int, 2>{});
+    };
+
+    if (hit) load_half(std::integral_constant<int, 0>{}, std::integral_constant<int, 0>{});
+    auto level = [&](auto l_tag) __attribute__((always_inline)) {
+        constexpr int l = decltype(l_tag)::value;
+        constexpr int c_first = l == 0 ? 0 : (l == 1 ? 2 : (l == 2 ? 5 : 7));
+        constexpr int c_last = l == 0 ? 1 : (l == 1 ? 4 : (l == 2 ? 6 : 10));
+        static_assert(c_last == (l == 3 ? NCHUNK - 1 : ((l + 1) * GB::N2) / BK - 1) && c_last - c_first < GB::RING, "ring of four chunk tiles");
+        if (hit) {
+            store_half(std::integral_constant<int, 0>{});
+            __syncthreads();
+            load_half(l_tag, std::integral_constant<int, 1>{});
+            if (l == 3) {
+                __bf16* As = ring + ((NCHUNK - 1) & (GB::RING - 1)) * A_ELEMS + row * LDB;
+                const bf16x4 z4 = __builtin_bit_cast(bf16x4, (uint64_t)0);
+#pragma unroll
+                for (int pl = 0; pl < NP; ++pl) {
+                    if (v == 0) *(bf16x4*)(As + pl * A_PLANE + 4) = z4;
+                    else *(bf16x8*)(As + pl * A_PLANE + 8 * v) = __builtin_shufflevector(z4, z4, 0, 1, 2, 3, 4, 5, 6, 7);
+                }
+            }
+            for (int it = tid; it < 64 * 5; it += NT) {
+                const int pix = it / 5, c = it - pix * 5;
+                sample(l_tag, pix, c, c);
+            }
+            __syncthreads();
+            store_half(std::integral_constant<int, 1>{});
+            __syncthreads();
+            if constexpr (l + 1 < GB::LEVELS) load_half(std::integral_constant<int, l + 1>{}, std::integral_constant<int, 0>{});
+            sample(l_tag, tid >> 2, 5 + (tid & 3), tid & 3);
+        } else {
+            __syncthreads();
+#pragma unroll
+            for (int c = c_first; c <= c_last; ++c) fill_chunk(c);
+        }
+        __syncthreads();
+        [&]<int... C>(std::integer_sequence<int, C...>) {
+            (run_chunk(std::integral_constant<int, c_first + C>{}), ...);
+        }(std::make_integer_sequence<int, c_last - c_first + 1>{});
+    };
+    level(std::integral_constant<int, 0>{});
+    level(std::integral_constant<int, 1>{});
+    level(std::integral_constant<int, 2>{});
+    level(std::integral_constant<int, 3>{});
+    __syncthreads();
+    woft::conv_epilogue_t<TM, TN, G::BM, WCOLS, G::ST>(pa, acc, (float*)smem + wave * G::ST * woft::STAGE_FLOATS,
+                                                        BlockRows{py0, px0, p.hf, p.wf}, 0, 0, wave, lane, tile);
+}
+
+}
+
+extern "C" int woft_conv1x1_band(const woft_conv_params* c1, const woft_conv_params* f1, const woft_lookup_band_params* bp,
+                                 void* stream) {
+    if (c1 == nullptr || bp == nullptr || bp->band == nullptr) return WOFT_EINVAL;
+    const woft_lookup_otf_params& o = bp->otf;
+    if (o.radius != 4 || o.k != 256 || o.levels != 4 || (o.terms != 1 && o.terms != 3) || o.coords == nullptr || o.out == nullptr ||
+        o.hf <= 0 || o.wf <= 0 || o.need != nullptr || o.ablate != 0)
+        return WOFT_EINVAL;
+    if ((o.roi_y0 | o.roi_x0 | o.roi_h | o.roi_w | o.smp_y0 | o.smp_x0 | o.smp_h | o.smp_w) != 0) return WOFT_EINVAL;
+    for (const woft_conv_params* q : {c1, f1}) {
+        if (q == nullptr) continue;
+        if (woft_conv_check(*q) != WOFT_OK) return WOFT_EINVAL;
+        const woft_conv_params& p = *q;
+        if (p.halo != 16 || p.precision < 1 || p.precision > 3 || p.precision != c1->precision) return WOFT_EINVAL;
+        if (p.stride != 1 || p.ho != p.h || p.wo != p.w || p.taps_x != 1) return WOFT_EINVAL;
+        if (p.wgt_frag == nullptr || p.stat_sum != nullptr || p.in_norm != 0 || p.wh0_lookup != nullptr) return WOFT_EINVAL;
+        if (p.epi == WOFT_EPI_FLOWHEAD || p.epi == WOFT_EPI_WH_MEAN || p.epi == WOFT_EPI_CTX) return WOFT_EINVAL;
+        if ((p.roi_y0 | p.roi_x0 | p.roi_h | p.roi_w) != 0) return WOFT_EINVAL;
+        const int64_t cs_max = (p.in1 != nullptr && p.cs1 > p.cs0) ? p.cs1 : p.cs0;
+        if ((int64_t)p.n_img * p.h * p.w * cs_max >= (1ll << 31)) return WOFT_EINVAL;
+    }
+    if (c1->flat || c1->taps_y != 1 || c1->pad_y != 0 || c1->pad_x != 0 || c1->tile_n != 256 || c1->cin_pad != 352 ||
+        c1->cout_pad != 256 || c1->in1 != nullptr || c1->n_img != 1 || c1->h != o.hf || c1->w != o.wf)
+        return WOFT_EINVAL;
+    if (c1->in0 != o.out || c1->cs0 != o.ldo || o.ldo < 352) return WOFT_EINVAL;
+    if (f1 != nullptr && (!f1->flat || f1->cin_pad != 32 || f1->tile_n != 128 || 2 * f1->pad_y + 1 != f1->taps_y ||
+                          f1->cout_pad % 128 != 0))
+        return WOFT_EINVAL;
+    const int split = ((o.hf + 7) / 8) * ((o.wf + 7) / 8);
+    const int64_t extra = f1 != nullptr ? (int64_t)m_tiles_1x1(*f1) * (f1->cout_pad / 128) : 0;
+    dim3 grid((unsigned)(split + extra));
+    hipStream_t s = (hipStream_t)stream;
+    const woft_conv_params& pb = f1 != nullptr ? *f1 : *c1;
+    switch (c1->precision) {
+        case 1: woft_launch(0, conv1x1_band_kernel<3>, grid, dim3(256), 0, s, *c1, pb, *bp, split); break;
+        case 2: woft_launch(0, conv1x1_band_kernel<1>, grid, dim3(256), 0, s, *c1, pb, *bp, split); break;
+        default: woft_launch(0, conv1x1_band_kernel<16>, grid, dim3(256), 0, s, *c1, pb, *bp, split); break;
+    }
+    return woft_launch_status();
+}
diff --git a/woft_amd/csrc/conv_1x1_tile.h b/woft_amd/csrc/conv_1x1_tile.h
--- /dev/null
+++ b/woft_amd/csrc/conv_1x1_tile.h
@@ -0,0 +1,203 @@
+#pragma once
+#include "conv_common.h"
+
+namespace {
+
+using woft::BK;
+
+template <int TERMS, int TN>
+struct Geom1x1 {
+    static constexpr int NP = (TERMS == 3) ? 2 : 1;
+    static constexpr int BM = 64, TM = 2;
+    static constexpr int WCOLS = 32 * TN, BN = 4 * WCOLS;
+    static constexpr int A_PLANE = BM * LDB, A_ELEMS = NP * A_PLANE;
+    static constexpr int ST = 2;
+    static constexpr int STAGE_ELEMS = 2 * 4 * ST * woft::STAGE_FLOATS;
+    static constexpr int SMEM_ELEMS = (2 * A_ELEMS > STAGE_ELEMS) ? 2 * A_ELEMS : STAGE_ELEMS;
+};
+
+template <int TERMS, int TN, bool FLAT, int DEPTH, int NB>
+__device__ __forceinline__ void tile_1x1(const woft_conv_params& p, const int m_tile, const int n_tile, __bf16* smem) {
+    using G = Geom1x1<TERMS, TN>;
+    constexpr int NP = G::NP, TM = G::TM, A_PLANE = G::A_PLANE, A_ELEMS = G::A_ELEMS, WCOLS = G::WCOLS, BN = G::BN;
+    static_assert(DEPTH % 2 == 0 && (2 * DEPTH) % NB == 0 && NB >= 2, "static ring slots");
+    constexpr int STEP_ELEMS = NP * 2 * 64 * 8;
+
+    const int tid = threadIdx.x;
+    const int lane = tid & 63;
+    const int wave = __builtin_amdgcn_readfirstlane(tid >> 6);
+    const int r32 = lane & 31, hh = lane >> 5;
+    const int row = tid >> 2, v = tid & 3;
+
+    int64_t M = (int64_t)p.n_img * p.ho * p.wo;
+    int64_t m0 = (int64_t)m_tile * G::BM;
+    if ((p.roi_y0 | p.roi_x0 | p.roi_h | p.roi_w) != 0) {
+        const int runs = (p.roi_w + G::BM - 1) / G::BM;
+        const int line = m_tile / runs, run = m_tile - line * runs;
+        const int img = line / p.roi_h, ry = line - img * p.roi_h;
+        m0 = ((int64_t)img * p.ho + p.roi_y0 + ry) * p.wo + p.roi_x0 + run * G::BM;
+        const int left = p.roi_w - run * G::BM;
+        M = m0 + (left < G::BM ? left : G::BM);
+    }
+    const int n0 = n_tile * BN;
+    const int nchunk = FLAT ? p.taps_y : p.cin_pad / BK;
+
+    const int abl = (p.out_w <= -12350 && p.out_w > -12358) ? -12350 - p.out_w : 0;
+    const bool rok = m0 + row < M;
+    const uint32_t pix = rok ? (uint32_t)(m0 + row) : 0u;
+    int oy = 0, img_row0 = 0;
+    uint32_t run0 = 0;
+    bool okx[2] = {true, true};
+    if constexpr (FLAT) {
+        const int hw = p.ho * p.wo;
+        const int img = (int)(pix / (uint32_t)hw), rem = (int)(pix - (uint32_t)img * (uint32_t)hw);
+        oy = rem / p.wo;
+        const int ox = rem - oy * p.wo;
+        img_row0 = img * p.h;
+#pragma unroll
+        for (int e = 0; e < 2; ++e) {
+            const int ixp = ox - p.pad_x + (8 * v + 4 * e) / p.cs0;
+            okx[e] = rok && ixp >= 0 && ixp < p.w;
+        }
+        run0 = (uint32_t)((ox - p.pad_x) * p.cs0 + 8 * v);
+    }
+    f32x4 rh[DEPTH][2];
+    auto load_a = [&](int chunk, auto slot_tag) {
+        constexpr int slot = decltype(slot_tag)::value;
+        if ((abl & 1) && chunk >= DEPTH) return;
+        const int ck = chunk < nchunk ? chunk : nchunk - 1;
+        if constexpr (FLAT) {
+            int iy = oy + ck - p.pad_y;
+            iy = iy < 0 ? 0 : (iy >= p.h ? p.h - 1 : iy);
+            const uint32_t rowoff = (uint32_t)(img_row0 + iy) * (uint32_t)(p.w * p.cs0);
+#pragma unroll
+            for (int e = 0; e < 2; ++e) rh[slot][e] = *(const f32x4*)(p.in0 + (okx[e] ? rowoff + run0 + 4 * e : 0u));
+        } else {
+            const int c0 = ck * BK;
+            const bool second = (p.in1 != nullptr) && (c0 >= p.c_split);
+            const float* base = second ? p.in1 : p.in0;
+            const uint32_t cs = (uint32_t)(second ? p.cs1 : p.cs0);
+            const uint32_t coff = (uint32_t)(second ? c0 - p.c_split : c0);
+            rh[slot][0] = *(const f32x4*)(base + (pix * cs + coff + 8 * v));
+            rh[slot][1] = *(const f32x4*)(base + (pix * cs + coff + 8 * v + 4));
+        }
+    };
+    auto store_a = [&](int chunk, __bf16* As, auto slot_tag) {
+        constexpr int slot = decltype(slot_tag)::value;
+        const f32x4 zero = {0.f, 0.f, 0.f, 0.f};
+        bool oky = true;
+        if constexpr (FLAT) {
+            const int iy = oy + chunk - p.pad_y;
+            oky = iy >= 0 && iy < p.h;
+        }
+        bf16x4 hi[2], lo[2];
+#pragma unroll
+        for (int e = 0; e < 2; ++e) {
+            const f32x4 val = (FLAT ? (okx[e] && oky) : rok) ? rh[slot][e] : zero;
+            hi[e] = cvt16<TERMS>(val);
+            if (NP == 2) lo[e] = __builtin_convertvector(val - widen_bf16x4(hi[e]), bf16x4);
+        }
+        *(bf16x8*)(As + row * LDB + 8 * v) = __builtin_shufflevector(hi[0], hi[1], 0, 1, 2, 3, 4, 5, 6, 7);
+        if (NP == 2) *(bf16x8*)(As + A_PLANE + row * LDB + 8 * v) = __builtin_shufflevector(lo[0], lo[1], 0, 1, 2, 3, 4, 5, 6, 7);
+    };
+
+    const __bf16* wstream[TN];
+#pragma unroll
+    for (int j = 0; j < TN; ++j) wstream[j] = (const __bf16*)p.wgt_frag + (int64_t)(n0 / 32 + wave * TN + j) * nchunk * STEP_ELEMS + lane * 8;
+    bf16x8 bq[NB][TN][NP];
+    auto fetch_b = [&](int step, auto slot_tag) {
+        constexpr int slot = decltype(slot_tag)::value;
+        if ((abl & 2) && step >= NB - 1) return;
+        const int s = step < 2 * nchunk ? step : 2 * nchunk - 1;
+        const int off = (s >> 1) * STEP_ELEMS + (s & 1) * 512;
+#pragma unroll
+        for (int j = 0; j < TN; ++j)
+#pragma unroll
+            for (int pl = 0; pl < NP; ++pl) bq[slot][j][pl] = *(const bf16x8*)(wstream[j] + off + pl * 1024);
+    };
+
+    f32x16 acc[TM][TN];
+#pragma unroll
+    for (int i = 0; i < TM; ++i)
+#pragma unroll
+        for (int j = 0; j < TN; ++j)
+#pragma unroll
+            for (int r = 0; r < 16; ++r) acc[i][j][r] = 0.f;
+    const int a_off = r32 * LDB + hh * 8;
+
+    [&]<int... D>(std::integer_sequence<int, D...>) {
+        (load_a(D, std::integral_constant<int, D>{}), ...);
+    }(std::make_integer_sequence<int, DEPTH>{});
+    [&]<int... S>(std::integer_sequence<int, S...>) {
+        (fetch_b(S, std::integral_constant<int, S>{}), ...);
+    }(std::make_integer_sequence<int, NB - 1>{});
+    store_a(0, smem, std::integral_constant<int, 0>{});
+    __syncthreads();
+
+    auto run_chunk = [&](int c, auto d_tag) {
+        constexpr int D = decltype(d_tag)::value;
+        const __bf16* As = smem + (D & 1) * A_ELEMS;
+        bf16x8 aq[2][TM][NP];
+        auto read_a = [&](auto s2_tag) {
+            constexpr int s2 = decltype(s2_tag)::value;
+#pragma unroll
+            for (int i = 0; i < TM; ++i)
+#pragma unroll
+                for (int pl = 0; pl < NP; ++pl) aq[s2][i][pl] = *(const bf16x8*)(As + a_off + i * 32 * LDB + pl * A_PLANE + s2 * 16);
+        };
+        read_a(std::integral_constant<int, 0>{});
+        read_a(std::integral_constant<int, 1>{});
+        [&]<int... S2>(std::integer_sequence<int, S2...>) {
+            ([&] {
+                constexpr int s2 = S2, slot = (2 * D + s2) % NB;
+                fetch_b(2 * c + s2 + NB - 1, std::integral_constant<int, (2 * D + s2 + NB - 1) % NB>{});
+                __builtin_amdgcn_sched_barrier(0);
+                if (NP == 2) {
+#pragma unroll
+                    for (int j = 0; j < TN; ++j)
+#pragma unroll
+                        for (int i = 0; i < TM; ++i) acc[i][j] = mma16<TERMS>(aq[s2][i][NP - 1], bq[slot][j][0], acc[i][j]);
+#pragma unroll
+                    for (int j = 0; j < TN; ++j)
+#pragma unroll
+                        for (int i = 0; i < TM; ++i) acc[i][j] = mma16<TERMS>(aq[s2][i][0], bq[slot][j][NP - 1], acc[i][j]);
+                }
+#pragma unroll
+                for (int j = 0; j < TN; ++j)
+#pragma unroll
+                    for (int i = 0; i < TM; ++i) acc[i][j] = mma16<TERMS>(aq[s2][i][0], bq[slot][j][0], acc[i][j]);
+                if constexpr (s2 == 0) {
+                    store_a(c + 1, smem + ((D + 1) & 1) * A_ELEMS, std::integral_constant<int, (D + 1) % DEPTH>{});
+                    load_a(c + DEPTH, std::integral_constant<int, D>{});
+                }
+                __builtin_amdgcn_sched_barrier(0);
+            }(), ...);
+        }(std::make_integer_sequence<int, 2>{});
+        __syncthreads();
+    };
+    for (int c0 = 0; c0 < nchunk; c0 += DEPTH) {
+        [&]<int... D>(std::integer_sequence<int, D...>) {
+            ((c0 + D < nchunk ? run_chunk(c0 + D, std::integral_constant<int, D>{}) : (void)0), ...);
+        }(std::make_integer_sequence<int, DEPTH>{});
+    }
+    if (abl & 4) {
+        float t = 0.f;
+#pragma unroll
+        for (int i = 0; i < TM; ++i)
+#pragma unroll
+            for (int j = 0; j < TN; ++j)
+#pragma unroll
+                for (int r = 0; r < 16; ++r) t += acc[i][j][r];
+        if (t == 12345.678f) p.out[0] = t;
+        return;
+    }
+    woft::conv_epilogue_t<TM, TN, G::BM, WCOLS, G::ST>(p, acc, (float*)smem + wave * G::ST * woft::STAGE_FLOATS,
+                                                        woft::LinearRows{m0, M}, n0, 0, wave, lane, m_tile);
+}
+
+__host__ __device__ __forceinline__ int m_tiles_1x1(const woft_conv_params& p) {
+    if ((p.roi_y0 | p.roi_x0 | p.roi_h | p.roi_w) != 0) return p.n_img * p.roi_h * ((p.roi_w + 63) / 64);
+    return (int)(((int64_t)p.n_img * p.ho * p.wo + 63) / 64);
+}
+
+}
diff --git a/woft_amd/csrc/lookup_band.hip b/woft_amd/csrc/lookup_band.hip
--- a/woft_amd/csrc/lookup_band.hip
+++ b/woft_amd/csrc/lookup_band.hip
@@ -103,6 +103,7 @@
         if (tid == 0) atomicAdd(bp.miss_count, 1);
         return;
     }
+    if (bp.defer_samples != 0) return;
     const int rows = band_row_off(R, p.levels);
     f32x4 pc[NLD];
     auto load_level = [&](int l) __attribute__((always_inline)) {
diff --git a/woft_amd/engine.py b/woft_amd/engine.py
--- a/woft_amd/engine.py
+++ b/woft_amd/engine.py
@@ -15,6 +15,7 @@
 PYRAMID_ONE_LAUNCH = os.environ.get("WOFT_PYRAMID", "1") != "0"
 FOLD_GATHER = os.environ.get("WOFT_FOLD_GATHER", "1") != "0"
 CORR_BAND = os.environ.get("WOFT_CORR_BAND", "1") != "0"
+FUSE_C1 = os.environ.get("WOFT_FUSE_C1", "1") != "0"
 BAND_MIN_LOOKUPS = 6
 
 
@@ -132,7 +133,7 @@
 
 class RaftEngine:
     def __init__(self, state_dict, small=False, weighted=True, precision="fp32", corr="volume", volume_storage=None,
-                 mask_head=False, corr_band="auto"):
+                 mask_head=False, corr_band="auto", fuse_c1=True):
         if precision not in ops.PRECISION:
             raise ValueError(f"precision must be one of {sorted(ops.PRECISION)}")
         if corr not in ("volume", "otf"):
@@ -143,6 +144,7 @@
         if corr_band not in ("auto", True, False):
             raise ValueError("corr_band must be 'auto', True or False")
         self.corr_band = corr_band
+        self.fuse_c1 = bool(fuse_c1)
         self.volume_storage = volume_storage or ("bf16" if precision == "bf16" else "fp32")
         if self.volume_storage not in ("fp32", "bf16") or (self.volume_storage == "bf16" and precision == "fp32"):
             raise ValueError("volume_storage: 'fp32', or 'bf16' with the split-bf16 precisions (their GEMM packs it)")
@@ -281,6 +283,7 @@
         self._graphs = {}
         self._band = None
         self._band_params = {}
+        self._fuse_c1 = False
         self.mk = self.mask = self.prog_iter_last = self.folded = self.fh_part = None
         self.x8 = self.x32 = self.wmean = self.wlow = self.cs_ws = self.cs_tot = self.wh6_b = self._wh6_pad = None
         self.a1 = self.a2 = self.wh0_t = self.wh_last = None
@@ -708,7 +711,11 @@
 
     def run(self, prog):
         ev = self.conv_events
-        for kind, a, tag in prog:
+        fused = False
+        for k, (kind, a, tag) in enumerate(prog):
+            if fused:
+                fused = False
+                continue
             if kind == "conv":
                 ops.run_conv(a) if ev is None else _timed(ev.get(tag), ops.run_conv, a)
             elif kind == "conv2":
@@ -730,7 +737,11 @@
             elif kind == "cgemm":
                 ops.corr_gemm_bf16(*a)
             elif kind == "lookup":
-                self._lookup(a)
+                fused = k + 1 < len(prog) and self._c1_on_band(a, prog[k + 1])
+                if fused:
+                    self._lookup_c1_band(a, prog[k + 1])
+                else:
+                    self._lookup(a)
             elif kind == "copy":
                 a[1].copy_(a[0])
             elif kind == "fh_gather":
@@ -788,6 +799,33 @@
         bp = self._band_variant(params)
         ops.run_lookup_band(bp)
         ops.run_lookup_otf(bp._fallback)
+
+    def _c1_on_band(self, params, nxt):
+        if not (self._fuse_c1 and self.band_valid) or nxt.tag not in ("convc1+convf1", "convc1"):
+            return False
+        sp = self.eng.spec
+        c1 = nxt.arg[0] if nxt.kind == "conv2" else nxt.arg
+        rect = lambda q: (q.roi_y0 | q.roi_x0 | q.roi_h | q.roi_w) != 0
+        if params.need or rect(params) or (params.smp_y0 | params.smp_x0 | params.smp_h | params.smp_w) != 0 or rect(c1):
+            return False
+        return ((sp.radius, sp.fdim, sp.levels) == (4, 256, 4) and Kernel(c1.halo) is Kernel.GEMM_1X1
+                and c1.precision in (1, 2, 3) and (c1.cin_pad, c1.cout_pad) == (352, 256)
+                and c1.in0 == params.out and c1.cs0 == params.ldo)
+
+    def _lookup_c1_band(self, params, nxt):
+        bp = self._band_variant(params)
+
+        def lookup():
+            bp.defer_samples = 1
+            try:
+                ops.run_lookup_band(bp)
+            finally:
+                bp.defer_samples = 0
+            ops.run_lookup_otf(bp._fallback)
+        _timed(self.lookup_events, lookup)
+        c1, f1 = nxt.arg if nxt.kind == "conv2" else (nxt.arg, None)
+        ev = self.conv_events
+        _timed(None if ev is None else ev.get(nxt.tag), ops.run_conv1x1_band, c1, f1, bp)
 
     @property
     def band_miss_blocks(self):
@@ -908,6 +946,7 @@
     def _flow(self, iters, crop, h, w, flow_up, dst, wout, do_sigmoid, trace, defer_wh, mout, mask_sigmoid, has_init, skip_wh,
               target_restored, region):
         e, sp = self.eng, self.eng.spec
+        self._fuse_c1 = FUSE_C1 and e.fuse_c1 and trace is None
         self._target_changed(self.target_owner)
         if not target_restored:
             self.run(self.prog_f_dst)
diff --git a/woft_amd/flow_provider.py b/woft_amd/flow_provider.py
--- a/woft_amd/flow_provider.py
+++ b/woft_amd/flow_provider.py
@@ -143,9 +143,11 @@
         self.corr = os.environ.get("WOFT_CORR") or getattr(self.C, "corr", None) or "otf"
         v = getattr(self.C, "corr_band", None)
         self.corr_band = "auto" if (v is None or isinstance(v, type(self.C))) else (v if v == "auto" else bool(v))
+        v = getattr(self.C, "fuse_c1", None)
+        self.fuse_c1 = True if (v is None or isinstance(v, type(self.C))) else bool(v)
         self.engine = RaftEngine(state_dict, small=small, weighted=weighted, precision=self.precision, corr=self.corr,
                                  volume_storage=getattr(self.C, "volume_storage", None), mask_head=self.masked,
-                                 corr_band=self.corr_band)
+                                 corr_band=self.corr_band, fuse_c1=self.fuse_c1)
         self._wh_loaded = {k: v for k, v in state_dict.items() if k.startswith("weight_head.net.")}
         self._wh_params = None
         v = getattr(self.C, "flow_region", None)
diff --git a/woft_amd/ops.py b/woft_amd/ops.py
--- a/woft_amd/ops.py
+++ b/woft_amd/ops.py
@@ -450,6 +450,11 @@
     check(_lib.load().woft_corr_lookup_band(C.byref(p), stream_ptr()), "woft_corr_lookup_band")
 
 
+def run_conv1x1_band(c1, f1, bp):
+    check(_lib.load().woft_conv1x1_band(C.byref(c1), C.byref(f1) if f1 is not None else None, C.byref(bp), stream_ptr()),
+          "woft_conv1x1_band")
+
+
 def split_bf16_lines(x, out):
     check(_lib.load().woft_split_bf16_lines(ptr(x), x.numel(), ptr(out), stream_ptr()), "woft_split_bf16_lines")
 
```

Result: faster. 124.8, median of 6 (+1.6%).
